# Pranav-Jain/Neural-Monte-Carlo-Fluid-Simulation

Measured on AMD Instinct MI355X. Metric: WoS walk-steps/sec + pressure-projection wall-time per step, 2D karman 64k pts, higher is better.
Workload: dtype f32

## Files before the change

include/wos.h:

```cpp
#ifndef WOS_H
#define WOS_H

#include <stddef.h>
#include <stdint.h>

#ifdef __cplusplus
extern "C" {
#endif

#define WOS_ABI_VERSION 10

enum {
    WOS_OK = 0,
    WOS_E_INVALID = -1,
    WOS_E_IO = -2,
    WOS_E_DEVICE = -3,
    WOS_E_CAPACITY = -4,
    WOS_E_NOMEM = -5
};

#define WOS_PTRS_DEVICE 0x1u
#define WOS_ASYNC       0x2u

typedef struct wos_mesh {
    int32_t dim;
    int32_t n_vertices;
    int32_t n_prims;
    float *vertices;
    int32_t *prims;
} wos_mesh;

int wos_load_obj(const char *path, int32_t dim, int32_t flip_orientation,
                 int32_t normalize, wos_mesh *out);
void wos_mesh_free(wos_mesh *mesh);

typedef struct wos_scene_desc {
    int32_t dim;
    const float *vertices;
    const int32_t *prims;
    int32_t n_vertices, n_prims;
    const float *dvertices;
    const int32_t *dprims;
    int32_t n_dvertices, n_dprims;
    float dirichlet_value;
    float absorption;
    int32_t is_watertight;
    int32_t is_double_sided;
    const float *source;
    int32_t source_dims[3];
    int32_t source_on_device;
    const float *dirichlet_image;
    int32_t dirichlet_image_dims[2];
    float dirichlet_image_box[4];
    int32_t dirichlet_image_on_device;
    const float *neumann_image;
    int32_t neumann_image_dims[2];
    float neumann_image_box[4];
    int32_t neumann_image_on_device;
} wos_scene_desc;

typedef struct wos_scene wos_scene;

int wos_scene_create(const wos_scene_desc *desc, int32_t device, wos_scene **out);
int wos_scene_destroy(wos_scene *scene);

int wos_scene_set_source(wos_scene *scene, const float *source, const int32_t *dims,
                         int32_t on_device, void *stream);

#define WOS_MAX_CHANNELS 4
int wos_scene_set_source_channels(wos_scene *scene, const float *source, int32_t n_channels,
                                  const int32_t *dims, const float *dirichlet_values,
                                  int32_t on_device, void *stream);
int32_t wos_scene_channels(const wos_scene *scene);

int wos_release_caches(int32_t device);

int64_t wos_set_max_batch_tasks(int64_t max_tasks);

typedef struct wos_scene_info {
    int32_t dim, n_prims, n_silhouettes, n_dprims, device;
    float bbox_min[3], bbox_max[3];
} wos_scene_info;
int wos_scene_get_info(const wos_scene *scene, wos_scene_info *info);

enum { WOS_QUERY_NEUMANN = 0, WOS_QUERY_DIRICHLET = 1 };
int wos_scene_query(wos_scene *scene, int32_t which, float boundary_distance_mask,
                    const float *pts, int64_t n,
                    float *dist, float *signed_dist, float *closest , int32_t *state,
                    void *stream, uint32_t flags);

typedef struct wos_solver_params {
    int32_t n_walks;
    int32_t max_walk_length;
    int32_t steps_before_tikhonov;
    int32_t steps_before_maximal_spheres;
    float epsilon_shell;
    float min_star_radius;
    float silhouette_precision;
    float russian_roulette_threshold;
    float boundary_distance_mask;
    int32_t disable_gradient_control_variates;
    int32_t disable_gradient_antithetic_variates;
    int32_t use_cosine_sampling;
    int32_t ignore_dirichlet;
    int32_t ignore_neumann;
    int32_t ignore_source;
    uint64_t seed;
    int32_t robust_float;
    uint32_t schedule;
} wos_solver_params;

#define WOS_SCHED_GEOM_GLOBAL   0x1u
#define WOS_SCHED_FULL_NEUMANN  0x2u
#define WOS_SCHED_NO_STAR_GRID  0x4u
#define WOS_SCHED_NO_DIR_GRID   0x8u
#define WOS_SCHED_NO_TAIL_SPREAD 0x10u
#define WOS_SCHED_NO_GRID_SPREAD 0x20u

void wos_default_params(wos_solver_params *p);

typedef struct wos_stats {
    uint64_t walk_steps;
    uint64_t wasted_steps;
    uint64_t walks_recorded;
    uint64_t walks_escaped;
    uint64_t walks_max_length;
    uint64_t walks_rr;
    uint64_t walks_dirichlet;
    uint64_t points_estimated;
    uint64_t rejection_iters;
    double kernel_ms;
    double first_ball_ms;
    double walk_ms;
    double fold_ms;
    uint64_t walk_launches;
    int32_t first_ball_blocks_per_cu;
    int32_t walk_blocks_per_cu;
    int32_t walk_lds_bytes;
    int32_t star_grid;
    int32_t geom_global;
    int32_t dir_grid;
    uint64_t ticket;
} wos_stats;

int wos_solve(wos_scene *scene, const wos_solver_params *params,
              const float *pts, int64_t n, int64_t index_base, int64_t index_stride,
              float *p, float *grad, int32_t *n_est, int32_t *steps,
              wos_stats *stats, void *stream, uint32_t flags);

int wos_solve_var(wos_scene *scene, const wos_solver_params *params,
                  const float *pts, int64_t n, int64_t index_base, int64_t index_stride,
                  float *p, float *grad, float *p_var, float *grad_var, int32_t *n_est, int32_t *steps,
                  wos_stats *stats, void *stream, uint32_t flags);

int wos_solve_channels(wos_scene *scene, const wos_solver_params *params,
                       const float *pts, int64_t n, int64_t index_base, int64_t index_stride,
                       int32_t n_channels, float *p, float *grad, float *p_var, float *grad_var,
                       int32_t *n_est, int32_t *steps, wos_stats *stats, void *stream, uint32_t flags);

typedef struct wos_bvc_params {
    int32_t n_walks_solution;
    int32_t n_walks_gradient;
    int32_t boundary_cache_size;
    int32_t domain_cache_size;
    int32_t grid_res;
    int32_t use_finite_differences;
    float normal_offset;
    float radius_clamp;
    float kernel_regularization;
    float grid_box[4];
} wos_bvc_params;

void wos_default_bvc_params(wos_bvc_params *p);

int wos_bvc(wos_scene *scene, const wos_solver_params *params, const wos_bvc_params *bvc,
            float *solution, float *grad, float *samples, int64_t samples_capacity, int64_t *counts,
            wos_stats *stats);

int wos_solve_stats(wos_scene *scene, uint64_t ticket, wos_stats *stats);

typedef struct wos_tape wos_tape;
typedef struct wos_tape_info {
    int32_t dim, n_walks, source_dims[3], device;
    int64_t n_points, n_tasks, n_entries, max_entries_per_walk, bytes;
    int32_t replay_chunk_entries;
} wos_tape_info;
int wos_tape_record(wos_scene *scene, const wos_solver_params *params, const float *pts, int64_t n,
                    int64_t index_base, int64_t index_stride, int64_t max_bytes,
                    wos_tape **out, wos_stats *stats, void *stream, uint32_t flags);
int wos_tape_solve(wos_tape *tape, wos_scene *scene, int32_t n_channels,
                   float *p, float *grad, float *p_var, float *grad_var,
                   int32_t *n_est, int32_t *steps, wos_stats *stats, void *stream, uint32_t flags);
int wos_tape_get_info(const wos_tape *tape, wos_tape_info *info);
int wos_tape_destroy(wos_tape *tape);

typedef enum wos_tape_field {
    WOS_TAPE_CODE = 0, WOS_TAPE_CNT = 1, WOS_TAPE_SLOT = 2, WOS_TAPE_CELL0 = 3, WOS_TAPE_GNORM = 4,
    WOS_TAPE_THR_END = 5, WOS_TAPE_TERM = 6, WOS_TAPE_TNEU = 7, WOS_TAPE_BDIR = 8, WOS_TAPE_SDIR = 9,
    WOS_TAPE_E_CELL = 10, WOS_TAPE_E_THR = 11, WOS_TAPE_E_NRM = 12, WOS_TAPE_PSTATE = 13,
    WOS_TAPE_SEGMENT_POINTS = 14
// ... 100 lines not shown
```

neural-monte-carlo-fluid-simulation_amd/csrc/wos_capi.h:

```cpp
#pragma once
#include <hip/hip_runtime.h>

#include <algorithm>
#include <atomic>
#include <cmath>
#include <condition_variable>
#include <cstdlib>
#include <cstring>
#include <list>
#include <memory>
#include <mutex>
#include <string>
#include <vector>

#include "../../include/wos.h"
#include "wos_bvc.h"
#include "wos_detmath.h"
#include "wos_host_scene.h"
#include "wos_launch.h"
#include "wos_siren.h"

namespace wos::capi {

extern thread_local std::string g_err;

inline int fail(int code, const std::string& msg) {
  g_err = msg;
  return code;
}

#define HIP_TRY(expr)                                                                         \
  do {                                                                                        \
    hipError_t _e = (expr);                                                                   \
    if (_e != hipSuccess) return fail(WOS_E_DEVICE, std::string(#expr ": ") + hipGetErrorString(_e)); \
  } while (0)

#define WOS_TRY(expr)                  \
  do {                                 \
    int _rc = (expr);                  \
    if (_rc != WOS_OK) return _rc;     \
  } while (0)

template <typename T>
hipError_t upload(T** dst, const std::vector<T>& src) {
  *dst = nullptr;
  if (src.empty()) return hipSuccess;
  hipError_t e = hipMalloc((void**)dst, src.size() * sizeof(T));
  if (e != hipSuccess) { *dst = nullptr; return e; }
  e = hipMemcpy(*dst, src.data(), src.size() * sizeof(T), hipMemcpyHostToDevice);
  if (e != hipSuccess) {
    hipFree(*dst);
    *dst = nullptr;
  }
  return e;
}

struct DevBufs {
  std::vector<void*> p;
  ~DevBufs() { for (void* q : p) hipFree(q); }
  template <typename T>
  hipError_t get(T** out, size_t n) {
    *out = nullptr;
    void* q = nullptr;
    hipError_t e = hipMalloc(&q, std::max<size_t>(1, n) * sizeof(T));
    if (e == hipSuccess) { p.push_back(q); *out = (T*)q; }
    return e;
  }
};

struct RunShape {
  int32_t bpc_fb = 0, bpc_walk = 0, walk_lds = 0, star_grid = 0, geom_global = 0, dir_grid = 0;
};

struct StatSlot {
  uint64_t ticket = 0;
  unsigned long long* h_cnt = nullptr;
  hipEvent_t ev0 = nullptr, ev1 = nullptr, done = nullptr;
  std::vector<hipEvent_t> bev;
  int64_t n_batches = 0;
  RunShape shape;
};
constexpr int kStatSlots = 16;

struct TaskWs {
  float* tasks = nullptr;
  int64_t task_cap = 0;
  int32_t* pstate = nullptr;
  int64_t pstate_cap = 0;
  unsigned long long* counters = nullptr;
  hipStream_t stream = nullptr;
  hipEvent_t done = nullptr;
};
constexpr int kSideWs = 2;

struct DevCtx {
  std::mutex mu;
  bool ready = false;
  int num_cus = 0;
  float* d_pts = nullptr;
  float* d_p = nullptr;
  float* d_g = nullptr;
  int32_t* d_nest = nullptr;
  int32_t* d_steps = nullptr;
  size_t ws_points = 0;
  float* d_pvar = nullptr;
  float* d_gvar = nullptr;
  size_t ws_var_points = 0;
  uint64_t* d_jump = nullptr;
  int n_jump = 0;
  float* d_tasks = nullptr;
  int64_t task_cap = 0;
  int32_t* d_pstate = nullptr;
  int64_t pstate_cap = 0;
  unsigned long long* d_counters = nullptr;
  StatSlot slot[kStatSlots];
  uint64_t next_ticket = 1;
  hipEvent_t done = nullptr;
  hipStream_t last_stream = nullptr;
  bool inflight = false;
  float* d_rejtab = nullptr;
  int stat_waiters = 0;
  std::condition_variable no_waiters;
  TaskWs side[kSideWs];
  hipStream_t bvc_dir = nullptr;
  hipEvent_t bvc_dir_done = nullptr;
};

constexpr int kMaxDevices = 64;
extern DevCtx g_ctx[kMaxDevices];
extern std::atomic<int64_t> g_max_batch_tasks;

int ctx_ready(DevCtx& c, int device);
hipError_t ctx_order(DevCtx& c, hipStream_t st);
int ctx_mark(DevCtx& c, hipStream_t st);

int ensure_workspace(DevCtx& c, int dim, size_t npts);
int ensure_tasks_in(float*& d_tasks, int64_t& task_cap, int32_t*& d_pstate, int64_t& pstate_cap, int dim,
                    int64_t tasks, int64_t points, int channels = 1);
int ensure_tasks(DevCtx& c, int dim, int64_t tasks, int64_t points, int channels = 1);
wos::DevTasks task_view_in(float* d_tasks, int32_t* d_pstate, int64_t pstate_cap, int dim, int64_t T, int32_t wpp,
                           int channels = 1);
wos::DevTasks task_view(DevCtx& c, int dim, int64_t T, int32_t wpp, int channels = 1);
int ensure_jump(DevCtx& c, int k_needed);
const std::vector<float>& rejection_tables();

int slot_open(DevCtx& c, hipStream_t st, int64_t n_events, int64_t n_batches, const RunShape& shape, StatSlot** out);
int slot_close(StatSlot& q, const unsigned long long* d_cnt, hipStream_t st);
int slot_finish(DevCtx& c, StatSlot& q, hipStream_t st, bool async, wos_stats* stats);

void stats_from(const unsigned long long* cnt, const RunShape& shape, wos_stats* stats);
void stats_add_counters(wos_stats* into, const wos_stats& from);
int fill_stats(const StatSlot& q, wos_stats* stats);

struct SolveOut {
  float* p = nullptr;
  float* grad = nullptr;
  int32_t* n_est = nullptr;
  int32_t* steps = nullptr;
  float* p_var = nullptr;
  float* grad_var = nullptr;
};
struct OutStage {
  SolveOut dev, host;
  size_t n = 0;
  int C = 1, dim = 2;
  bool staged = false;
};
int stage_outputs(DevCtx& c, const SolveOut& caller, bool dev_ptrs, int64_t n, int C, int dim, OutStage& o);
int copy_back(const OutStage& o, hipStream_t st);

struct Geom {
  int device = 0;
  int dim = 2, double_sided = 0;
  std::vector<float> v, dv;
  std::vector<int32_t> ix, dix;
  wos::HostScene host;
  float *d_prim = nullptr, *d_paux = nullptr, *d_sil = nullptr, *d_dprim = nullptr, *d_dpaux = nullptr;
  float *d_pgroup = nullptr, *d_sgroup = nullptr, *d_dgroup = nullptr;
  float *d_ptree = nullptr, *d_stree = nullptr, *d_dtree = nullptr;
  float* d_nbox = nullptr;
  int32_t *d_nchild = nullptr, *d_nref = nullptr;
  std::mutex mu;
  struct Grid {
    float prec, min_r;
    bool ok;
    wos::StarGrid grid;
    uint32_t* d = nullptr;
  };
  std::list<Grid> grids;
  bool dgrid_built = false, dgrid_ok = false;
  wos::DirGrid dgrid;
  uint32_t* d_dgrid = nullptr;
  ~Geom();
};

int star_grid(Geom& g, float prec, float min_r, const Geom::Grid** out);
int dir_grid(Geom& g, bool* ok);
void geom_cache_drop(int device);

constexpr size_t kLdsDynamicMax = 160 * 1024 - 4096;

}

struct wos_scene {
  int device = 0;
  uint64_t serial = 0;
  std::shared_ptr<wos::capi::Geom> geom;
  wos::DevScene dev{};
  float* d_source = nullptr;
  size_t source_cap = 0;
  float* d_planar = nullptr;
  size_t planar_cap = 0;
  float g_dirichlet = 0.0f;
  float* d_dimg = nullptr;
  float* d_nimg = nullptr;
  std::mutex mu;
};

namespace wos::capi {

struct WalkLayout {
  wos::DevScene dsc;
  int geom_floats = 0;
  int geom_floats_walk = 0;
  size_t shmem_walk = 0;
};
int walk_layout(wos_scene* s, const wos_solver_params* prm, WalkLayout& L);

wos::DevParams dev_params(const wos_solver_params* prm);
int check_params(const std::string& fn, const wos_solver_params* prm);

struct SolveExtra {
  const float* ddir = nullptr;
  float* deriv = nullptr;
  bool force_estimate = false;
  int wave_prio = 0;
  float* p_var = nullptr;
  float* grad_var = nullptr;
  int channels = 1;
};

struct SolvePlan {
  wos::DevParams dp{};
  wos::DevScene dsc{}, dfb{};
  int geom_floats_walk = 0, lhs_floats = 0;
  size_t shmem_walk = 0, shmem_fb = 0, shmem_fb_run = 0;
  int64_t wpp = 0;
  wos::KernelVariant kv{};
  int grid_fb = 0, grid_walk = 0, bpc_fb = 0, bpc_walk = 0;
  RunShape shape() const {
    return {bpc_fb, bpc_walk, (int32_t)shmem_walk, dsc.sgrid != nullptr, dsc.geom_global, dsc.dgrid != nullptr};
  }
};
int solve_plan(DevCtx& c, wos_scene* s, const wos_solver_params* prm, const SolveExtra& ex, bool record, SolvePlan& P);
int solve_grids(DevCtx& c, int dim, int64_t chunk, bool record, SolvePlan& P);

struct Batches {
  int64_t chunk = 1, n_chunks = 0;
};
Batches batches(int64_t n, int64_t wpp);
int batch_head(DevCtx& c, int dim, const SolvePlan& P, int64_t k, const float* d_pts, int64_t nb,
               const wos::DevTasks& tk, hipEvent_t after_zero, hipStream_t st);
int fold_channels(int dim, const wos::DevParams& dp, const wos::DevTasks& tk, int C, int64_t nb, int64_t b0,
                  int64_t n, const SolveOut& out, hipStream_t st);

int solve_locked(wos_scene* s, const wos_solver_params* prm, const float* pts, int64_t n, int64_t index_base,
                 int64_t index_stride, float* p, float* grad, int32_t* n_est, int32_t* steps, wos_stats* stats,
                 void* stream, uint32_t flags, const SolveExtra& ex);

}
```

neural-monte-carlo-fluid-simulation_amd/csrc/wos_capi_ctx.cpp:

```cpp
#include "wos_capi.h"

namespace wos::capi {

thread_local std::string g_err;
DevCtx g_ctx[kMaxDevices];

#ifndef WOS_BATCH_LOG2
#define WOS_BATCH_LOG2 28
#endif
static_assert(WOS_BATCH_LOG2 <= 30, "task indices carry a flag in bit 31 (wos_walk_kernel hand-out)");
constexpr int64_t kDefaultBatchTasks = (int64_t)1 << WOS_BATCH_LOG2;
std::atomic<int64_t> g_max_batch_tasks{kDefaultBatchTasks};

static void ctx_free(DevCtx& c) {
  hipFree(c.d_pts); hipFree(c.d_p); hipFree(c.d_g); hipFree(c.d_nest); hipFree(c.d_steps);
  hipFree(c.d_pvar); hipFree(c.d_gvar);
  c.d_pvar = c.d_gvar = nullptr;
  c.ws_var_points = 0;
  hipFree(c.d_jump); hipFree(c.d_tasks); hipFree(c.d_pstate); hipFree(c.d_counters); hipFree(c.d_rejtab);
  c.d_rejtab = nullptr;
  for (StatSlot& q : c.slot) {
    if (q.ev0) hipEventDestroy(q.ev0);
    if (q.ev1) hipEventDestroy(q.ev1);
    if (q.done) hipEventDestroy(q.done);
    for (hipEvent_t e : q.bev) hipEventDestroy(e);
    if (q.h_cnt) hipHostFree(q.h_cnt);
    q = StatSlot{};
  }
  if (c.done) hipEventDestroy(c.done);
  if (c.bvc_dir_done) hipEventDestroy(c.bvc_dir_done);
  if (c.bvc_dir) hipStreamDestroy(c.bvc_dir);
  c.bvc_dir_done = nullptr;
  c.bvc_dir = nullptr;
  for (TaskWs& w : c.side) {
    hipFree(w.tasks); hipFree(w.pstate); hipFree(w.counters);
    if (w.done) hipEventDestroy(w.done);
    if (w.stream) hipStreamDestroy(w.stream);
    w = TaskWs{};
  }
  c.d_pts = c.d_p = c.d_g = nullptr;
  c.d_nest = c.d_steps = nullptr;
  c.ws_points = 0;
  c.d_jump = nullptr; c.n_jump = 0;
  c.d_tasks = nullptr; c.task_cap = 0;
  c.d_pstate = nullptr; c.pstate_cap = 0;
  c.d_counters = nullptr;
  c.done = nullptr;
  c.last_stream = nullptr;
  c.inflight = false;
  c.ready = false;
}

const std::vector<float>& rejection_tables() {
  static std::once_flag once;
  static std::vector<float> t(2 * wos::kRejTabBins);
  std::call_once(once, [] {
    wos::rejection_bound_table(2, t.data());
    wos::rejection_bound_table(3, t.data() + wos::kRejTabBins);
  });
  return t;
}

int ctx_ready(DevCtx& c, int device) {
  if (c.ready) return WOS_OK;
  {
    const std::vector<float>& t = rejection_tables();
    HIP_TRY(hipMalloc((void**)&c.d_rejtab, t.size() * sizeof(float)));
    HIP_TRY(hipMemcpy(c.d_rejtab, t.data(), t.size() * sizeof(float), hipMemcpyHostToDevice));
  }
  HIP_TRY(hipDeviceGetAttribute(&c.num_cus, hipDeviceAttributeMultiprocessorCount, device));
  HIP_TRY(hipMalloc((void**)&c.d_counters, wos::kMainCounterSlots * sizeof(unsigned long long)));
  for (StatSlot& q : c.slot) {
    HIP_TRY(hipHostMalloc((void**)&q.h_cnt, wos::kNumCounters * sizeof(unsigned long long)));
    HIP_TRY(hipEventCreate(&q.ev0));
    HIP_TRY(hipEventCreate(&q.ev1));
    HIP_TRY(hipEventCreateWithFlags(&q.done, hipEventDisableTiming));
  }
  HIP_TRY(hipEventCreateWithFlags(&c.done, hipEventDisableTiming));
  c.ready = true;
  return WOS_OK;
}

hipError_t ctx_order(DevCtx& c, hipStream_t st) {
  if (c.inflight && c.last_stream != st && c.done) return hipStreamWaitEvent(st, c.done, 0);
  return hipSuccess;
}

int ctx_mark(DevCtx& c, hipStream_t st) {
  HIP_TRY(hipEventRecord(c.done, st));
  c.last_stream = st;
  return WOS_OK;
}

int ensure_workspace(DevCtx& c, int dim, size_t npts) {
  if (npts <= c.ws_points) return WOS_OK;
  hipFree(c.d_pts); hipFree(c.d_p); hipFree(c.d_g); hipFree(c.d_nest); hipFree(c.d_steps);
  c.d_pts = c.d_p = c.d_g = nullptr; c.d_nest = c.d_steps = nullptr; c.ws_points = 0;
  const size_t cap = npts + npts / 4 + 1024;
  HIP_TRY(hipMalloc((void**)&c.d_pts, cap * 3 * sizeof(float)));
  HIP_TRY(hipMalloc((void**)&c.d_p, cap * sizeof(float)));
  HIP_TRY(hipMalloc((void**)&c.d_g, cap * 3 * sizeof(float)));
  HIP_TRY(hipMalloc((void**)&c.d_nest, cap * sizeof(int32_t)));
  HIP_TRY(hipMalloc((void**)&c.d_steps, cap * sizeof(int32_t)));
  (void)dim;
  c.ws_points = cap;
  return WOS_OK;
}

static int ensure_var_workspace(DevCtx& c, size_t npts) {
  if (npts <= c.ws_var_points) return WOS_OK;
  hipFree(c.d_pvar); hipFree(c.d_gvar);
  c.d_pvar = c.d_gvar = nullptr; c.ws_var_points = 0;
  const size_t cap = npts + npts / 4 + 1024;
  HIP_TRY(hipMalloc((void**)&c.d_pvar, cap * sizeof(float)));
  HIP_TRY(hipMalloc((void**)&c.d_gvar, cap * 3 * sizeof(float)));
  c.ws_var_points = cap;
  return WOS_OK;
}

int ensure_tasks_in(float*& d_tasks, int64_t& task_cap, int32_t*& d_pstate, int64_t& pstate_cap, int dim,
                    int64_t tasks, int64_t points, int channels) {
  const int tf = std::max(wos::task_floats(dim), wos::task_floats(3));
  const int tfc = std::max(wos::task_floats(dim, channels), wos::task_floats(3, channels));
  if (channels > 1) tasks = (tasks * tfc + tf - 1) / tf;
  if (tasks > task_cap) {
    hipFree(d_tasks);
    d_tasks = nullptr; task_cap = 0;
    HIP_TRY(hipMalloc((void**)&d_tasks, (size_t)tasks * tf * sizeof(float)));
    task_cap = tasks;
  }
  if (points > pstate_cap) {
    hipFree(d_pstate);
    d_pstate = nullptr; pstate_cap = 0;
    HIP_TRY(hipMalloc((void**)&d_pstate, ((size_t)7 * points + 2 * wos::kCostBuckets) * sizeof(int32_t)));
    pstate_cap = points;
  }
  return WOS_OK;
}

int ensure_tasks(DevCtx& c, int dim, int64_t tasks, int64_t points, int channels) {
  return ensure_tasks_in(c.d_tasks, c.task_cap, c.d_pstate, c.pstate_cap, dim, tasks, points, channels);
}

wos::DevTasks task_view_in(float* d_tasks, int32_t* d_pstate, int64_t pstate_cap, int dim, int64_t T, int32_t wpp,
                           int channels) {
  wos::DevTasks tk{};
  float* f = d_tasks;
  tk.pt = f; f += dim * T;
  tk.thr = f; f += T;
  tk.tsrc = f; f += channels * T;
  tk.dd = f; f += T;
  tk.first = f; f += channels * T;
  tk.bdir = f; f += dim * T;
  tk.sdir = f; f += dim * T;
  tk.total = f; f += channels * T;
  tk.code = (uint32_t*)f;
  tk.pstate = d_pstate;
  tk.perm = (uint32_t*)(d_pstate + pstate_cap);
  tk.prad = (float*)(d_pstate + 2 * pstate_cap);
  tk.hist = (uint32_t*)(d_pstate + 3 * pstate_cap);
  tk.pball = (float*)(d_pstate + 3 * pstate_cap + 2 * wos::kCostBuckets);
  tk.pball_stride = pstate_cap;
  tk.T = T;
  tk.wpp = wpp;
  return tk;
}

wos::DevTasks task_view(DevCtx& c, int dim, int64_t T, int32_t wpp, int channels) {
  return task_view_in(c.d_tasks, c.d_pstate, c.pstate_cap, dim, T, wpp, channels);
}

int ensure_jump(DevCtx& c, int k_needed) {
  if (k_needed <= c.n_jump) return WOS_OK;
  const int cap = std::max(k_needed, 4096);
  std::vector<uint64_t> t(2 * (size_t)cap);
  uint64_t A = 1u, Cc = 0u;
  for (int k = 0; k < cap; k++) {
    t[2 * k] = A; t[2 * k + 1] = Cc;
    A = A * wos::kPcgMult;
    Cc = Cc * wos::kPcgMult + wos::kPcgInc;
  }
  hipFree(c.d_jump);
  c.d_jump = nullptr; c.n_jump = 0;
  HIP_TRY(hipMalloc((void**)&c.d_jump, t.size() * sizeof(uint64_t)));
  HIP_TRY(hipMemcpy(c.d_jump, t.data(), t.size() * sizeof(uint64_t), hipMemcpyHostToDevice));
  c.n_jump = cap;
  return WOS_OK;
}

int stage_outputs(DevCtx& c, const SolveOut& caller, bool dev_ptrs, int64_t n, int C, int dim, OutStage& o) {
  o.dev = o.host = caller;
  o.n = (size_t)std::max<int64_t>(n, 0);
  o.C = C;
  o.dim = dim;
  o.staged = !dev_ptrs && n > 0;
  if (!o.staged) return WOS_OK;
  WOS_TRY(ensure_workspace(c, dim, o.n * C));
  o.dev.p = c.d_p; o.dev.grad = c.d_g;
  o.dev.n_est = caller.n_est ? c.d_nest : nullptr;
  o.dev.steps = caller.steps ? c.d_steps : nullptr;
  if (caller.p_var || caller.grad_var) {
    WOS_TRY(ensure_var_workspace(c, o.n * C));
    o.dev.p_var = caller.p_var ? c.d_pvar : nullptr;
    o.dev.grad_var = caller.grad_var ? c.d_gvar : nullptr;
  }
  return WOS_OK;
}

int copy_back(const OutStage& o, hipStream_t st) {
  if (!o.staged) return WOS_OK;
  const size_t n = o.n, nc = o.n * o.C;
  const SolveOut &h = o.host, &d = o.dev;
  HIP_TRY(hipMemcpyAsync(h.p, d.p, nc * sizeof(float), hipMemcpyDeviceToHost, st));
  HIP_TRY(hipMemcpyAsync(h.grad, d.grad, nc * o.dim * sizeof(float), hipMemcpyDeviceToHost, st));
  if (h.n_est) HIP_TRY(hipMemcpyAsync(h.n_est, d.n_est, n * sizeof(int32_t), hipMemcpyDeviceToHost, st));
  if (h.steps) HIP_TRY(hipMemcpyAsync(h.steps, d.steps, n * sizeof(int32_t), hipMemcpyDeviceToHost, st));
  if (h.p_var) HIP_TRY(hipMemcpyAsync(h.p_var, d.p_var, nc * sizeof(float), hipMemcpyDeviceToHost, st));
  if (h.grad_var)
    HIP_TRY(hipMemcpyAsync(h.grad_var, d.grad_var, nc * o.dim * sizeof(float), hipMemcpyDeviceToHost, st));
  return WOS_OK;
}

int slot_open(DevCtx& c, hipStream_t st, int64_t n_events, int64_t n_batches, const RunShape& shape, StatSlot** out) {
  const uint64_t ticket = c.next_ticket++;
  StatSlot& q = c.slot[ticket % kStatSlots];
  while ((int64_t)q.bev.size() < n_events) {
    hipEvent_t e = nullptr;
    HIP_TRY(hipEventCreate(&e));
    q.bev.push_back(e);
  }
  q.ticket = ticket;
  q.n_batches = n_batches;
  q.shape = shape;
  HIP_TRY(hipEventRecord(q.ev0, st));
  *out = &q;
  return WOS_OK;
}

int slot_close(StatSlot& q, const unsigned long long* d_cnt, hipStream_t st) {
  HIP_TRY(hipEventRecord(q.ev1, st));
  HIP_TRY(hipMemcpyAsync(q.h_cnt, d_cnt, wos::kNumCounters * sizeof(unsigned long long), hipMemcpyDeviceToHost, st));
  return WOS_OK;
}

int slot_finish(DevCtx& c, StatSlot& q, hipStream_t st, bool async, wos_stats* stats) {
  HIP_TRY(hipEventRecord(q.done, st));
  WOS_TRY(ctx_mark(c, st));
  c.inflight = true;
  if (async) {
    if (stats) {
      *stats = wos_stats{};
      stats->ticket = q.ticket;
    }
    return WOS_OK;
  }
  HIP_TRY(hipStreamSynchronize(st));
  c.inflight = false;
  return stats ? fill_stats(q, stats) : WOS_OK;
}

void stats_from(const unsigned long long* cnt, const RunShape& shape, wos_stats* stats) {
  *stats = wos_stats{};
  stats->walk_steps = cnt[0];
  stats->wasted_steps = cnt[1];
  stats->walks_recorded = cnt[2];
  stats->walks_escaped = cnt[3];
  stats->walks_max_length = cnt[4];
  stats->walks_rr = cnt[5];
  stats->walks_dirichlet = cnt[6];
  stats->points_estimated = cnt[7];
  stats->rejection_iters = cnt[8];
  stats->first_ball_blocks_per_cu = shape.bpc_fb;
  stats->walk_blocks_per_cu = shape.bpc_walk;
  stats->walk_lds_bytes = shape.walk_lds;
  stats->star_grid = shape.star_grid;
  stats->geom_global = shape.geom_global;
  stats->dir_grid = shape.dir_grid;
}

void stats_add_counters(wos_stats* into, const wos_stats& from) {
  into->walk_steps += from.walk_steps; into->wasted_steps += from.wasted_steps;
  into->walks_recorded += from.walks_recorded; into->walks_escaped += from.walks_escaped;
  into->walks_max_length += from.walks_max_length; into->walks_rr += from.walks_rr;
  into->walks_dirichlet += from.walks_dirichlet; into->points_estimated += from.points_estimated;
  into->rejection_iters += from.rejection_iters;
}

int fill_stats(const StatSlot& q, wos_stats* stats) {
  stats_from(q.h_cnt, q.shape, stats);
  float ms = 0.0f;
  HIP_TRY(hipEventElapsedTime(&ms, q.ev0, q.ev1));
  stats->kernel_ms = ms;
  stats->walk_launches = (uint64_t)q.n_batches;
  for (int64_t b = 0; b < q.n_batches; b++) {
    const hipEvent_t* ev = &q.bev[4 * b];
    float a = 0.0f, w = 0.0f, f = 0.0f;
    HIP_TRY(hipEventElapsedTime(&a, ev[0], ev[1]));
    HIP_TRY(hipEventElapsedTime(&w, ev[1], ev[2]));
    HIP_TRY(hipEventElapsedTime(&f, ev[2], ev[3]));
    stats->first_ball_ms += a; stats->walk_ms += w; stats->fold_ms += f;
  }
  stats->ticket = q.ticket;
  return WOS_OK;
}

}

using namespace wos::capi;

extern "C" {

const char* wos_last_error(void) { return g_err.c_str(); }
int32_t wos_abi_version(void) { return WOS_ABI_VERSION; }

int32_t wos_device_count(void) {
  int n = 0;
  if (hipGetDeviceCount(&n) != hipSuccess) return 0;
  return n;
}

int64_t wos_set_max_batch_tasks(int64_t max_tasks) {
  const int64_t v = max_tasks <= 0 ? kDefaultBatchTasks
                                   : std::min<int64_t>(std::max<int64_t>(max_tasks, (int64_t)1 << 16), (int64_t)1 << 30);
  return g_max_batch_tasks.exchange(v);
}

int wos_release_caches(int32_t device) {
  int ndev = 0;
  if (hipGetDeviceCount(&ndev) != hipSuccess) ndev = 0;
  for (int dv = 0; dv < std::min(ndev, kMaxDevices); dv++) {
    if (device >= 0 && dv != device) continue;
    DevCtx& c = g_ctx[dv];
    std::unique_lock<std::mutex> lk(c.mu);
    c.no_waiters.wait(lk, [&] { return c.stat_waiters == 0; });
    if (!c.ready) continue;
    HIP_TRY(hipSetDevice(dv));
    HIP_TRY(hipDeviceSynchronize());
    ctx_free(c);
  }
  geom_cache_drop(device);
  return WOS_OK;
}

int wos_solve_stats(wos_scene* s, uint64_t ticket, wos_stats* stats) {
  if (!s || !stats) return fail(WOS_E_INVALID, "wos_solve_stats: null scene/stats");
  const auto unknown = [&] {
    return fail(WOS_E_INVALID, "wos_solve_stats: unknown ticket (more than " + std::to_string(kStatSlots) +
                                   " solves were enqueued on this device after it)");
  };
  HIP_TRY(hipSetDevice(s->device));
  DevCtx& c = g_ctx[s->device];
  hipEvent_t done = nullptr;
  {
    std::lock_guard<std::mutex> lock(s->mu);
    std::lock_guard<std::mutex> lk(c.mu);
    StatSlot& q = c.slot[ticket % kStatSlots];
    if (ticket == 0 || q.ticket != ticket) return unknown();
    done = q.done;
    c.stat_waiters++;
  }
  const hipError_t e = hipEventSynchronize(done);
  std::lock_guard<std::mutex> lock(s->mu);
  std::lock_guard<std::mutex> lk(c.mu);
  if (--c.stat_waiters == 0) c.no_waiters.notify_all();
  if (e != hipSuccess) return fail(WOS_E_DEVICE, std::string("wos_solve_stats: ") + hipGetErrorString(e));
  StatSlot& q = c.slot[ticket % kStatSlots];
  if (q.ticket != ticket) return unknown();
  HIP_TRY(hipEventSynchronize(q.done));
  return fill_stats(q, stats);
}

}
```

neural-monte-carlo-fluid-simulation_amd/csrc/wos_capi_scene.cpp:

```cpp
#include "wos_capi.h"

namespace wos::capi {

Geom::~Geom() {
  hipSetDevice(device);
  hipDeviceSynchronize();
  hipFree(d_prim); hipFree(d_paux); hipFree(d_sil); hipFree(d_dprim); hipFree(d_dpaux);
  hipFree(d_pgroup); hipFree(d_sgroup); hipFree(d_dgroup);
  hipFree(d_ptree); hipFree(d_stree); hipFree(d_dtree);
  hipFree(d_nbox); hipFree(d_nchild); hipFree(d_nref);
  for (Grid& g : grids) hipFree(g.d);
  hipFree(d_dgrid);
}

static std::mutex g_geom_mu;
static std::vector<std::shared_ptr<Geom>>& g_geom_lru = *new std::vector<std::shared_ptr<Geom>>();
constexpr size_t kGeomCacheSize = 8;
static std::atomic<uint64_t> g_scene_serial{0};

template <typename T>
static bool same(const std::vector<T>& a, const T* b, int n) {
  return a.size() == (size_t)n && (n == 0 || std::memcmp(a.data(), b, (size_t)n * sizeof(T)) == 0);
}

static bool geom_matches(const Geom& g, const wos_scene_desc* d, int device) {
  const int dim = d->dim;
  return g.device == device && g.dim == dim && g.double_sided == d->is_double_sided &&
         same(g.v, d->vertices, d->n_vertices * dim) && same(g.ix, d->prims, d->n_prims * dim) &&
         same(g.dv, d->dvertices, d->n_dvertices * dim) && same(g.dix, d->dprims, d->n_dprims * dim);
}

static int geom_get(const wos_scene_desc* d, int device, std::shared_ptr<Geom>& out) {
  {
    std::lock_guard<std::mutex> lk(g_geom_mu);
    for (size_t i = 0; i < g_geom_lru.size(); i++)
      if (geom_matches(*g_geom_lru[i], d, device)) {
        out = g_geom_lru[i];
        std::rotate(g_geom_lru.begin(), g_geom_lru.begin() + i, g_geom_lru.begin() + i + 1);
        return WOS_OK;
      }
  }
  auto g = std::make_shared<Geom>();
  const int dim = d->dim;
  g->device = device;
  g->dim = dim;
  g->double_sided = d->is_double_sided;
  if (d->n_vertices > 0) g->v.assign(d->vertices, d->vertices + (size_t)d->n_vertices * dim);
  if (d->n_prims > 0) g->ix.assign(d->prims, d->prims + (size_t)d->n_prims * dim);
  if (d->n_dvertices > 0) g->dv.assign(d->dvertices, d->dvertices + (size_t)d->n_dvertices * dim);
  if (d->n_dprims > 0) g->dix.assign(d->dprims, d->dprims + (size_t)d->n_dprims * dim);
  wos::HostSceneInput in;
  in.dim = dim;
  in.vertices = d->vertices; in.prims = d->prims; in.n_vertices = d->n_vertices; in.n_prims = d->n_prims;
  in.dvertices = d->dvertices; in.dprims = d->dprims; in.n_dvertices = d->n_dvertices; in.n_dprims = d->n_dprims;
  in.is_double_sided = d->is_double_sided;
  std::string err;
  if (!wos::prepare_scene(in, g->host, err)) return fail(WOS_E_INVALID, "wos_scene_create: " + err);
  HIP_TRY(upload(&g->d_prim, g->host.prim));
  HIP_TRY(upload(&g->d_paux, g->host.paux));
  HIP_TRY(upload(&g->d_sil, g->host.sil));
  HIP_TRY(upload(&g->d_dprim, g->host.dprim));
  HIP_TRY(upload(&g->d_dpaux, g->host.dpaux));
  HIP_TRY(upload(&g->d_pgroup, g->host.pgroup));
  HIP_TRY(upload(&g->d_dgroup, g->host.dgroup));
  HIP_TRY(upload(&g->d_sgroup, g->host.sgroup));
  HIP_TRY(upload(&g->d_ptree, g->host.ptree.node));
  HIP_TRY(upload(&g->d_stree, g->host.stree.node));
  HIP_TRY(upload(&g->d_dtree, g->host.dtree.node));
  HIP_TRY(upload(&g->d_nbox, g->host.nbvh.box));
  HIP_TRY(upload(&g->d_nchild, g->host.nbvh.child));
  HIP_TRY(upload(&g->d_nref, g->host.nbvh.ref));
  {
    std::lock_guard<std::mutex> lk(g_geom_mu);
    g_geom_lru.insert(g_geom_lru.begin(), g);
    if (g_geom_lru.size() > kGeomCacheSize) g_geom_lru.pop_back();
  }
  out = g;
  return WOS_OK;
}

void geom_cache_drop(int device) {
  std::lock_guard<std::mutex> lk(g_geom_mu);
  if (device < 0) {
    g_geom_lru.clear();
  } else {
    g_geom_lru.erase(std::remove_if(g_geom_lru.begin(), g_geom_lru.end(),
                                    [&](const std::shared_ptr<Geom>& g) { return g->device == device; }),
                     g_geom_lru.end());
  }
}

constexpr size_t kStarGridBudget = 16 * 1024;

int star_grid(Geom& g, float prec, float min_r, const Geom::Grid** out) {
  std::lock_guard<std::mutex> lk(g.mu);
  for (const Geom::Grid& x : g.grids)
    if (x.prec == prec && x.min_r == min_r) { *out = &x; return WOS_OK; }
  Geom::Grid x{prec, min_r, false, {}, nullptr};
  if (wos::build_star_grid(g.host, prec, min_r, kStarGridBudget, x.grid)) {
    HIP_TRY(upload(&x.d, x.grid.words));
    x.ok = true;
  }
  g.grids.push_back(std::move(x));
  *out = &g.grids.back();
  return WOS_OK;
}

int dir_grid(Geom& g, bool* ok) {
  std::lock_guard<std::mutex> lk(g.mu);
  if (!g.dgrid_built) {
    const bool have = wos::build_dirichlet_grid(g.host, g.dgrid);
    if (have) HIP_TRY(upload(&g.d_dgrid, g.dgrid.words));
    g.dgrid_ok = have;
    g.dgrid_built = true;
  }
  *ok = g.dgrid_ok;
  return WOS_OK;
}

static void source_installed(wos_scene* s, const int32_t* dims, int n_channels, const float* dirichlet_values) {
  const int nsd = s->dev.dim == 2 ? 2 : 3;
  s->dev.source = s->d_source;
  for (int k = 0; k < 3; k++) s->dev.sdims[k] = k < nsd ? dims[k] : 1;
  s->dev.n_channels = n_channels;
  s->dev.g_dirichlet = s->g_dirichlet;
  for (int ch = 0; ch < wos::kMaxChannels; ch++)
    s->dev.g_ch[ch] = (dirichlet_values && ch < n_channels) ? dirichlet_values[ch] : s->g_dirichlet;
}

static int check_source_dims(int dim, const int32_t* dims, size_t* nsrc) {
  const int nsd = dim == 2 ? 2 : 3;
  size_t n = 1;
  for (int k = 0; k < nsd; k++) {
// ... 326 lines not shown
```

neural-monte-carlo-fluid-simulation_amd/csrc/wos_capi_solve.cpp:

```cpp
#include "wos_capi.h"

namespace wos::capi {

int walk_layout(wos_scene* s, const wos_solver_params* prm, WalkLayout& L) {
  Geom& geom = *s->geom;
  const wos::HostScene& host = geom.host;
  const int dim = host.dim;
  const int PS = dim == 2 ? wos::kPrimStride2 : wos::kPrimStride3;
  const int SS = dim == 2 ? wos::kSilStride2 : wos::kSilStride3;
  const int primAl = (host.n_prims * PS + 3) & ~3;
  const int silAl = (host.n_sil * SS + 3) & ~3;
  L.geom_floats = primAl + silAl + wos::kGroupStride * host.n_pgroups + wos::kSGroupStride * host.n_sgroups;
  wos::DevScene& dsc = L.dsc;
  dsc = s->dev;
  dsc.sgrid = nullptr;
  dsc.sgrid_words = dsc.sgrid_off_words = 0;
  if (!(prm->schedule & WOS_SCHED_NO_STAR_GRID) && host.n_sil > 0) {
    const Geom::Grid* gr = nullptr;
    WOS_TRY(star_grid(geom, prm->silhouette_precision, prm->min_star_radius, &gr));
    if (gr->ok) {
      dsc.sgrid = gr->d;
      dsc.sgrid_words = (int32_t)gr->grid.words.size();
      dsc.sgrid_off_words = gr->grid.off_words;
      for (int k = 0; k < 3; k++) {
// ... 87 lines not shown
  wos::DevScene& dsc = P.dsc;
  dsc = wl.dsc;
  P.geom_floats_walk = wl.geom_floats_walk;
  P.shmem_walk = wl.shmem_walk;
  P.lhs_floats = ((2 * dp.n_pairs * (dim - 1)) + 3) & ~3;
  P.shmem_fb = wos::kWavesPerBlockHost * wos::first_ball_wave_lds_bytes(P.lhs_floats, dp.n_pairs);
  P.shmem_fb_run = P.shmem_fb;
  wos::DevScene& dfb = P.dfb;
  dfb = s->dev;
  dfb.dgrid = dsc.dgrid;
  dfb.dgrid_off_words = dsc.dgrid_off_words;
  for (int k = 0; k < 2; k++) {
    dfb.dgrid_n[k] = dsc.dgrid_n[k];
    dfb.dgrid_min[k] = dsc.dgrid_min[k];
    dfb.dgrid_inv[k] = dsc.dgrid_inv[k];
  }
  if ((prm->schedule & WOS_SCHED_GEOM_GLOBAL) || P.shmem_walk > kLdsDynamicMax) {
    dfb.geom_global = 1;
    dsc.geom_global = 1;
    P.geom_floats_walk = 0;
    P.shmem_walk = wos::kWavesPerBlockHost * wos::walk_wave_lds_bytes(dim);
  }
  if (P.shmem_fb > kLdsDynamicMax)
    return fail(WOS_E_CAPACITY, "wos_solve: nWalks exceed the LDS budget of the first-ball kernel (" +
                                    std::to_string(P.shmem_fb) + " bytes of stratified samples per block)");
  if (P.shmem_walk > kLdsDynamicMax)
    return fail(WOS_E_CAPACITY, "wos_solve: the walk kernel's per-wave scratch exceeds the LDS budget (" +
                                    std::to_string(P.shmem_walk) + " bytes)");

  P.wpp = (int64_t)dp.n_pairs * dp.n_anti;
  {
    double diag2 = 0.0;
    for (int k = 0; k < 3; k++) diag2 += (double)host.ext[k] * host.ext[k];
    const double mu_r = std::sqrt(std::max(0.0, (double)s->dev.absorption)) * std::sqrt(diag2) * 1.01;
    dp.neumann_inert = (!dp.robust && s->dev.watertight && !s->dev.double_sided && mu_r < 80.0 && !s->dev.nimg &&
                        !(prm->schedule & WOS_SCHED_FULL_NEUMANN)) ? 1 : 0;
  }
  dp.tail_spread = (dim == 2 && !dp.robust && !dsc.geom_global && !(prm->schedule & WOS_SCHED_NO_TAIL_SPREAD)) ? 1 : 0;
#ifdef WOS_ACCT_NOSPREAD
  dp.tail_spread = 0;
#endif
  if (record) {
    dp.neumann_inert = 0;
    dp.tail_spread = 0;
    dsc.n_channels = 1;
    dfb.n_channels = 1;
  }
  P.kv = wos::kernel_variant(dim, dsc, dp, false);
  return WOS_OK;
}

int solve_grids(DevCtx& c, int dim, int64_t chunk, bool record, SolvePlan& P) {
  wos::DevParams& dp = P.dp;
  const bool gg = P.dsc.geom_global != 0;
  const auto occupancy = [&](int which, size_t shmem, int* blocks) {
    return record ? wos::occupancy_rec_blocks_per_cu(dim, gg, which, shmem, blocks)
                  : wos::occupancy_blocks_per_cu(P.kv, which, shmem, blocks);
  };
  HIP_TRY(occupancy(0, P.shmem_fb, &P.bpc_fb));
  const int jn = std::min(2 * (2 * dp.n_pairs) * (dim - 1), wos::kLhsJumpMax);
  const size_t shmem_j = P.shmem_fb + (size_t)jn * 2 * sizeof(uint64_t);
  int bpc_j = 0;
  if (jn > 0 && shmem_j <= kLdsDynamicMax) HIP_TRY(occupancy(0, shmem_j, &bpc_j));
  if (WOS_LHS_JUMP_STAGE && jn > 0 && bpc_j >= P.bpc_fb) {
    dp.lhs_jump_n = jn;
    P.shmem_fb_run = shmem_j;
  }
  const int64_t fb_waves = (chunk + wos::first_ball_points_per_wave(dp.n_pairs) - 1) / wos::first_ball_points_per_wave(dp.n_pairs);
  P.grid_fb = (int)std::min<int64_t>((fb_waves + wos::kWavesPerBlockHost - 1) / wos::kWavesPerBlockHost,
                                     (int64_t)std::max(1, P.bpc_fb) * std::max(1, c.num_cus));
  HIP_TRY(occupancy(1, P.shmem_walk, &P.bpc_walk));
  P.grid_walk = std::max(1, P.bpc_walk) * std::max(1, c.num_cus);
  return WOS_OK;
}

Batches batches(int64_t n, int64_t wpp) {
  Batches b;
  b.chunk = std::max<int64_t>(1, std::min<int64_t>(n, g_max_batch_tasks.load() / wpp));
  b.n_chunks = n > 0 ? (n + b.chunk - 1) / b.chunk : 0;
  return b;
}

int batch_head(DevCtx& c, int dim, const SolvePlan& P, int64_t k, const float* d_pts, int64_t nb,
               const wos::DevTasks& tk, hipEvent_t after_zero, hipStream_t st) {
  HIP_TRY(wos::launch_zero(k == 0 ? c.d_counters : c.d_counters + wos::kNumCounters,
                           k == 0 ? wos::kNumCounterSlots : wos::kNumCounterSlots - wos::kNumCounters,
                           tk.hist, 2 * wos::kCostBuckets, st));
  if (after_zero) HIP_TRY(hipEventRecord(after_zero, st));
  HIP_TRY(wos::launch_point_setup(dim, P.dfb, P.dp, d_pts, nb, tk, st));
  HIP_TRY(wos::launch_lpt_order(tk, nb, st));
  return WOS_OK;
}

int fold_channels(int dim, const wos::DevParams& dp, const wos::DevTasks& tk, int C, int64_t nb, int64_t b0,
                  int64_t n, const SolveOut& out, hipStream_t st) {
  for (int ch = 0; ch < C; ch++) {
    wos::DevTasks tkc = tk;
    tkc.total = tk.total + (int64_t)ch * tk.T;
    tkc.first = tk.first + (int64_t)ch * tk.T;
    const int64_t o1 = (int64_t)ch * n + b0, od = ((int64_t)ch * n + b0) * dim;
    HIP_TRY(wos::launch_fold(dim, dp, tkc, nb, out.p + o1, out.grad + od,
                             (out.n_est && ch == 0) ? out.n_est + b0 : nullptr,
                             (out.steps && ch == 0) ? out.steps + b0 : nullptr, out.p_var ? out.p_var + o1 : nullptr,
                             out.grad_var ? out.grad_var + od : nullptr, st));
  }
  return WOS_OK;
}

int solve_locked(wos_scene* s, const wos_solver_params* prm, const float* pts, int64_t n, int64_t index_base,
                 int64_t index_stride, float* p, float* grad, int32_t* n_est, int32_t* steps, wos_stats* stats,
                 void* stream, uint32_t flags, const SolveExtra& ex) {
  const int dim = s->geom->host.dim;
  hipStream_t st = (hipStream_t)stream;
  DevCtx& c = g_ctx[s->device];
  WOS_TRY(ctx_ready(c, s->device));

  SolvePlan plan;
  WOS_TRY(solve_plan(c, s, prm, ex, false, plan));
  wos::DevParams& dp = plan.dp;

  HIP_TRY(ctx_order(c, st));

  const bool dev_ptrs = (flags & WOS_PTRS_DEVICE) != 0;
  const int C = ex.channels;
  OutStage out;
  WOS_TRY(stage_outputs(c, SolveOut{p, grad, n_est, steps, ex.p_var, ex.grad_var}, dev_ptrs, n, C, dim, out));
  const float* d_pts = pts;
  if (out.staged) {
    HIP_TRY(hipMemcpyAsync(c.d_pts, pts, (size_t)n * dim * sizeof(float), hipMemcpyHostToDevice, st));
    d_pts = c.d_pts;
  }

  const int64_t wpp = plan.wpp;
  const Batches bt = batches(n, wpp);
  if (n > 0) {
    WOS_TRY(ensure_tasks(c, dim, bt.chunk * wpp, bt.chunk, C));
    WOS_TRY(solve_grids(c, dim, bt.chunk, false, plan));
  }
  StatSlot* slot = nullptr;
  WOS_TRY(slot_open(c, st, 4 * bt.n_chunks, bt.n_chunks, plan.shape(), &slot));
  StatSlot& q = *slot;
  if (bt.n_chunks == 0) HIP_TRY(wos::launch_zero(c.d_counters, wos::kMainCounterSlots, nullptr, 0, st));
  for (int64_t k = 0; k < bt.n_chunks; k++) {
    const int64_t b0 = k * bt.chunk;
    hipEvent_t* ev = &q.bev[4 * k];
    const int64_t nb = std::min(bt.chunk, n - b0);
    wos::DevTasks tk = task_view(c, dim, nb * wpp, (int32_t)wpp, C);
    tk.ddir = ex.ddir ? ex.ddir + b0 * dim : nullptr;
    tk.deriv = ex.deriv ? ex.deriv + b0 : nullptr;
    const int64_t bbase = index_base + b0 * index_stride;
    unsigned int* q_points = (unsigned int*)(c.d_counters + wos::kNumCounters);
    unsigned int* q_tasks = (unsigned int*)(c.d_counters + wos::kTaskQueueSlot0);
    const int walk_grid = (int)std::min<int64_t>(plan.grid_walk, (tk.T + 63) / 64);
    WOS_TRY(batch_head(c, dim, plan, k, d_pts + b0 * dim, nb, tk, ev[0], st));
    HIP_TRY(wos::launch_first_balls(plan.kv, plan.dfb, dp, d_pts + b0 * dim, nb, bbase, index_stride, tk,
                                    c.d_counters, q_points, plan.grid_fb, plan.shmem_fb_run, plan.lhs_floats, st));
    HIP_TRY(hipEventRecord(ev[1], st));
    HIP_TRY(wos::launch_walks(plan.kv, plan.dsc, dp, tk, bbase, index_stride, c.d_counters, q_tasks, walk_grid,
                              plan.shmem_walk, plan.geom_floats_walk, st));
    HIP_TRY(hipEventRecord(ev[2], st));
    WOS_TRY(fold_channels(dim, dp, tk, C, nb, b0, n, out.dev, st));
    HIP_TRY(hipEventRecord(ev[3], st));
  }
  WOS_TRY(slot_close(q, c.d_counters, st));
  WOS_TRY(copy_back(out, st));
  const bool async = (flags & WOS_ASYNC) && dev_ptrs;
  WOS_TRY(slot_finish(c, q, st, async, stats));
  if (!async) wos::diag_dump(dim == 2 ? "2d" : "3d");
  return WOS_OK;
}

static int solve_checked(wos_scene* s, const wos_solver_params* prm, const float* pts, int64_t n, int64_t index_base,
                         int64_t index_stride, int32_t n_channels, float* p, float* grad, float* p_var,
                         float* grad_var, int32_t* n_est, int32_t* steps, wos_stats* stats, void* stream,
                         uint32_t flags) {
  if (!s || !prm) return fail(WOS_E_INVALID, "wos_solve: null scene/params");
  if (n < 0) return fail(WOS_E_INVALID, "wos_solve: negative point count");
  if (n > 0 && (!pts || !p || !grad)) return fail(WOS_E_INVALID, "wos_solve: null point/output buffer");
  if (n >= (int64_t)0xFFFFFFF0LL) return fail(WOS_E_INVALID, "wos_solve: too many points for one call");
  WOS_TRY(check_params("wos_solve", prm));
  std::lock_guard<std::mutex> lock(s->mu);
  HIP_TRY(hipSetDevice(s->device));
  DevCtx& c = g_ctx[s->device];
  std::lock_guard<std::mutex> lk(c.mu);
  if (n_channels == 0 && s->dev.n_channels > 1)
    return fail(WOS_E_INVALID, "wos_solve: the scene holds " + std::to_string(s->dev.n_channels) +
                                   " source channels; use wos_solve_channels (or wos_scene_set_source for one)");
  if (n_channels != 0 && n_channels != s->dev.n_channels)
    return fail(WOS_E_INVALID, "wos_solve_channels: n_channels " + std::to_string(n_channels) +
                                   " differs from the scene's " + std::to_string(s->dev.n_channels));
  SolveExtra ex;
  ex.p_var = p_var;
  ex.grad_var = grad_var;
  ex.channels = s->dev.n_channels;
  return solve_locked(s, prm, pts, n, index_base, index_stride, p, grad, n_est, steps, stats, stream, flags, ex);
}

}

using namespace wos::capi;

extern "C" {

void wos_default_params(wos_solver_params* p) {
  if (!p) return;
  std::memset(p, 0, sizeof(*p));
  p->n_walks = 128;
  p->max_walk_length = 1024;
  p->steps_before_tikhonov = 1024;
  p->steps_before_maximal_spheres = 1024;
  p->epsilon_shell = 1e-3f;
  p->min_star_radius = 1e-3f;
  p->silhouette_precision = 1e-3f;
  p->russian_roulette_threshold = 0.0f;
  p->boundary_distance_mask = 0.0f;
  p->seed = 0x5EED0001ULL;
}

int wos_solve_var(wos_scene* s, const wos_solver_params* prm, const float* pts, int64_t n, int64_t index_base,
                  int64_t index_stride, float* p, float* grad, float* p_var, float* grad_var, int32_t* n_est,
                  int32_t* steps, wos_stats* stats, void* stream, uint32_t flags) {
  return solve_checked(s, prm, pts, n, index_base, index_stride, 0, p, grad, p_var, grad_var, n_est, steps, stats,
                       stream, flags);
}

int wos_solve_channels(wos_scene* s, const wos_solver_params* prm, const float* pts, int64_t n, int64_t index_base,
                       int64_t index_stride, int32_t n_channels, float* p, float* grad, float* p_var,
                       float* grad_var, int32_t* n_est, int32_t* steps, wos_stats* stats, void* stream,
                       uint32_t flags) {
  if (n_channels < 1 || n_channels > WOS_MAX_CHANNELS)
    return fail(WOS_E_INVALID, "wos_solve_channels: n_channels must be 1.." + std::to_string(WOS_MAX_CHANNELS) +
                                   ", got " + std::to_string(n_channels));
  return solve_checked(s, prm, pts, n, index_base, index_stride, n_channels, p, grad, p_var, grad_var, n_est, steps,
                       stats, stream, flags);
}

int wos_solve(wos_scene* s, const wos_solver_params* prm, const float* pts, int64_t n, int64_t index_base,
              int64_t index_stride, float* p, float* grad, int32_t* n_est, int32_t* steps, wos_stats* stats,
              void* stream, uint32_t flags) {
  return wos_solve_var(s, prm, pts, n, index_base, index_stride, p, grad, nullptr, nullptr, n_est, steps, stats,
                       stream, flags);
}
// ... 3 lines not shown
```

neural-monte-carlo-fluid-simulation_amd/csrc/wos_capi_tape.cpp:

```cpp
#include "wos_capi.h"

using namespace wos::capi;

struct TapeSeg {
  int64_t nb = 0, T = 0;
  uint64_t slots = 0;
  void* buf = nullptr;
  void* ebuf = nullptr;
  wos::DevTape tp{};
  uint32_t* code = nullptr;
  float* bdir = nullptr;
  float* sdir = nullptr;
  int32_t* pstate = nullptr;
};

struct TapeIndexSeg {
  void* buf = nullptr;
  wos::DevTapeIndex ix{};
  int64_t bytes = 0, max_row = 0;
};

struct TapeIndex {
  std::vector<TapeIndexSeg> seg;
  int64_t bytes = 0, n_terms = 0, max_row = 0;
// ... 57 lines not shown
  for (int k = 0; k < 3; k++)
    if ((s->dev.source ? s->dev.sdims[k] : 0) != tape->sdims[k])
      return fail(WOS_E_INVALID, fn + ": the scene's source dims differ from the recorded ones "
                                 "(the tape stores grid cells)");
  return WOS_OK;
}

static int tape_ensure_tasks(DevCtx& c, const wos_tape* tape, int C) {
  int64_t maxT = 0;
  for (const TapeSeg& g : tape->seg) maxT = std::max(maxT, g.T);
  return maxT > 0 ? ensure_tasks(c, tape->dim, maxT, 0, C) : WOS_OK;
}

extern "C" {

int wos_tape_record(wos_scene* s, const wos_solver_params* prm, const float* pts, int64_t n, int64_t index_base,
                    int64_t index_stride, int64_t max_bytes, wos_tape** out, wos_stats* stats, void* stream,
                    uint32_t flags) {
  if (!s || !prm || !out) return fail(WOS_E_INVALID, "wos_tape_record: null scene/params/out");
  *out = nullptr;
  if (n < 0) return fail(WOS_E_INVALID, "wos_tape_record: negative point count");
  if (n > 0 && !pts) return fail(WOS_E_INVALID, "wos_tape_record: null point buffer");
  if (n >= (int64_t)0xFFFFFFF0LL) return fail(WOS_E_INVALID, "wos_tape_record: too many points for one call");
  WOS_TRY(check_params("wos_tape_record", prm));
  if (prm->robust_float)
    return fail(WOS_E_INVALID, "wos_tape_record: robust_float walks are not recorded (reference float semantics only)");
  std::lock_guard<std::mutex> lock(s->mu);
  HIP_TRY(hipSetDevice(s->device));
  DevCtx& c = g_ctx[s->device];
  std::lock_guard<std::mutex> lk(c.mu);
  WOS_TRY(ctx_ready(c, s->device));
  const int dim = s->geom->host.dim;
  hipStream_t st = (hipStream_t)stream;
  SolvePlan plan;
  WOS_TRY(solve_plan(c, s, prm, SolveExtra{}, true, plan));
  wos::DevParams& dp = plan.dp;
  HIP_TRY(ctx_order(c, st));
  const float* d_pts = pts;
  if (!(flags & WOS_PTRS_DEVICE) && n > 0) {
    WOS_TRY(ensure_workspace(c, dim, (size_t)n));
    HIP_TRY(hipMemcpyAsync(c.d_pts, pts, (size_t)n * dim * sizeof(float), hipMemcpyHostToDevice, st));
    d_pts = c.d_pts;
  }
  const int64_t wpp = plan.wpp;
  const Batches bt = batches(n, wpp);
  DevBufs tmp;
  unsigned long long* d_cnt2 = nullptr;
  unsigned long long* d_bsum = nullptr;
  if (n > 0) {
    WOS_TRY(ensure_tasks(c, dim, bt.chunk * wpp, bt.chunk, 1));
    WOS_TRY(solve_grids(c, dim, bt.chunk, true, plan));
    HIP_TRY(tmp.get(&d_cnt2, (size_t)wos::kNumCounterSlots));
    HIP_TRY(tmp.get(&d_bsum, (size_t)wos::tape_slot_blocks(bt.chunk * wpp) + 1));
  }

  std::unique_ptr<wos_tape> tape(new wos_tape());
  tape->device = s->device;
  tape->geom = s->geom;
  tape->scene_serial = s->serial;
  tape->dim = dim;
  for (int k = 0; k < 3; k++) tape->sdims[k] = s->dev.source ? s->dev.sdims[k] : 0;
  tape->dp = dp;
  tape->dp.jump = nullptr;
  tape->dp.rej_tab = nullptr;
  tape->n = n;
  tape->wpp = wpp;
  tape->shape = plan.shape();
  HIP_TRY(hipMalloc((void**)&tape->d_cnt, (wos::kNumCounters + 2) * sizeof(unsigned long long)));
  HIP_TRY(hipMalloc((void**)&tape->d_flag, sizeof(uint32_t)));
  HIP_TRY(hipMemsetAsync(tape->d_cnt, 0, (wos::kNumCounters + 2) * sizeof(unsigned long long), st));
  HIP_TRY(hipMemsetAsync(tape->d_flag, 0, sizeof(uint32_t), st));
  tape->bytes = (int64_t)((wos::kNumCounters + 2) * sizeof(unsigned long long) + sizeof(uint32_t));
  unsigned long long* d_stat = tape->d_cnt + wos::kNumCounters;
  const auto over_cap = [&](int64_t bytes) {
    return fail(WOS_E_CAPACITY, "wos_tape_record: the tape needs more than " + std::to_string(bytes) +
                                    " bytes, max_bytes is " + std::to_string(max_bytes));
  };

  hipEvent_t ev0 = nullptr, ev1 = nullptr;
  HIP_TRY(hipEventCreate(&ev0));
  struct EvGuard { hipEvent_t& a; hipEvent_t& b; ~EvGuard() { if (a) hipEventDestroy(a); if (b) hipEventDestroy(b); } } evg{ev0, ev1};
  HIP_TRY(hipEventCreate(&ev1));
  HIP_TRY(hipEventRecord(ev0, st));
  if (bt.n_chunks == 0) HIP_TRY(wos::launch_zero(c.d_counters, wos::kMainCounterSlots, nullptr, 0, st));
  tape->seg.reserve((size_t)bt.n_chunks);
  for (int64_t k = 0; k < bt.n_chunks; k++) {
    const int64_t b0 = k * bt.chunk;
    const int64_t nb = std::min(bt.chunk, n - b0);
    tape->seg.emplace_back();
    TapeSeg& g = tape->seg.back();
    g.nb = nb;
    g.T = nb * wpp;
    const size_t tb = tape_task_bytes(dim, g.T, nb);
    if (max_bytes > 0 && tape->bytes + (int64_t)tb > max_bytes) return over_cap(tape->bytes + (int64_t)tb);
    HIP_TRY(hipMalloc(&g.buf, tb));
    tape->bytes += (int64_t)tb;
    tape_seg_views(g, dim, tape->d_flag);
    wos::DevTasks tk = task_view(c, dim, g.T, (int32_t)wpp, 1);
    wos::DevTasks tkr = tk;
    tkr.bdir = g.bdir;
    tkr.sdir = g.sdir;
    const int64_t bbase = index_base + b0 * index_stride;
    unsigned long long* qslot = c.d_counters + wos::kNumCounters;
    const int walk_grid = (int)std::min<int64_t>(plan.grid_walk, (g.T + 63) / 64);
    WOS_TRY(batch_head(c, dim, plan, k, d_pts + b0 * dim, nb, tk, nullptr, st));
    HIP_TRY(wos::launch_first_balls_rec(dim, plan.dfb, dp, d_pts + b0 * dim, nb, bbase, index_stride, tkr, g.tp,
                                        c.d_counters, (unsigned int*)qslot, plan.grid_fb, plan.shmem_fb_run,
                                        plan.lhs_floats, st));
    HIP_TRY(hipMemsetAsync(tk.tsrc, 0, (size_t)g.T * sizeof(float), st));
    HIP_TRY(wos::launch_walks(plan.kv, plan.dsc, dp, tk, bbase, index_stride, c.d_counters,
                              (unsigned int*)(c.d_counters + wos::kTaskQueueSlot0), walk_grid, plan.shmem_walk,
                              plan.geom_floats_walk, st));
    HIP_TRY(wos::launch_tape_slots(tk.code, g.T, (uint32_t*)g.tp.slot, d_bsum, st));
    unsigned long long slots = 0;
    HIP_TRY(hipMemcpyAsync(&slots, d_bsum + wos::tape_slot_blocks(g.T), sizeof(slots), hipMemcpyDeviceToHost, st));
    HIP_TRY(hipStreamSynchronize(st));
    if (slots >= (1ull << 31))
      return fail(WOS_E_CAPACITY, "wos_tape_record: a batch's walks need " + std::to_string(slots) +
                                      " entry slots (32-bit slot indices); lower wos_set_max_batch_tasks");
    g.slots = slots;
    const size_t eb = (size_t)std::max<unsigned long long>(slots, 1) * 12;
    if (max_bytes > 0 && tape->bytes + (int64_t)eb > max_bytes) return over_cap(tape->bytes + (int64_t)eb);
    HIP_TRY(hipMalloc(&g.ebuf, eb));
    tape->bytes += (int64_t)eb;
    g.tp.e_cell = (uint32_t*)g.ebuf;
    g.tp.e_thr = (float*)g.ebuf + std::max<unsigned long long>(slots, 1);
    g.tp.e_nrm = g.tp.e_thr + std::max<unsigned long long>(slots, 1);
    HIP_TRY(hipMemsetAsync(g.ebuf, 0, eb, st));
    tkr.code = g.code;
    HIP_TRY(wos::launch_zero(d_cnt2, wos::kNumCounterSlots, nullptr, 0, st));
    HIP_TRY(wos::launch_walks_rec(dim, plan.dsc.geom_global != 0, plan.dsc, dp, tkr, g.tp, bbase, index_stride, d_cnt2,
                                  (unsigned int*)(d_cnt2 + wos::kTaskQueueSlot0), walk_grid, plan.shmem_walk,
                                  plan.geom_floats_walk, st));
    HIP_TRY(hipMemcpyAsync(g.pstate, tk.pstate, (size_t)nb * sizeof(int32_t), hipMemcpyDeviceToDevice, st));
    HIP_TRY(wos::launch_tape_stats(g.code, g.tp.cnt, g.T, d_stat, st));
  }
  HIP_TRY(hipMemcpyAsync(tape->d_cnt, c.d_counters, wos::kNumCounters * sizeof(unsigned long long),
                         hipMemcpyDeviceToDevice, st));
  HIP_TRY(hipEventRecord(ev1, st));
  unsigned long long h_cnt[wos::kNumCounters + 2] = {};
  uint32_t h_flag = 0;
  HIP_TRY(hipMemcpyAsync(h_cnt, tape->d_cnt, sizeof(h_cnt), hipMemcpyDeviceToHost, st));
  HIP_TRY(hipMemcpyAsync(&h_flag, tape->d_flag, sizeof(h_flag), hipMemcpyDeviceToHost, st));
  WOS_TRY(ctx_mark(c, st));
  HIP_TRY(hipStreamSynchronize(st));
  c.inflight = false;
  if (h_flag)
    return fail(WOS_E_DEVICE, "wos_tape_record: a walk outgrew the slots sized for it; the tape is discarded");
  tape->n_entries = (int64_t)h_cnt[wos::kNumCounters];
  tape->max_entries = (int64_t)h_cnt[wos::kNumCounters + 1];
  if (stats) {
    stats_from(h_cnt, tape->shape, stats);
    float ms = 0.0f;
    HIP_TRY(hipEventElapsedTime(&ms, ev0, ev1));
    stats->kernel_ms = ms;
    stats->walk_launches = (uint64_t)(2 * bt.n_chunks);
  }
  *out = tape.release();
  return WOS_OK;
}

int wos_tape_solve(wos_tape* tape, wos_scene* s, int32_t n_channels, float* p, float* grad, float* p_var,
                   float* grad_var, int32_t* n_est, int32_t* steps, wos_stats* stats, void* stream, uint32_t flags) {
  if (!tape || !s) return fail(WOS_E_INVALID, "wos_tape_solve: null tape/scene");
  const int64_t n = tape->n;
  const int dim = tape->dim;
  if (n > 0 && (!p || !grad)) return fail(WOS_E_INVALID, "wos_tape_solve: null output buffer");
// ... 322 lines not shown
```

neural-monte-carlo-fluid-simulation_amd/csrc/wos_device.h:

```cpp

#pragma once
#include <cstdio>

#include "wos_detmath.h"
#include "wos_scene.h"

namespace wos {

#ifndef WOS_DIAG
#define WOS_DIAG 0
#endif

constexpr int kWave = 64;
constexpr int kBlock = 256;

enum { WC_DIRICHLET = 0, WC_RR = 1, WC_MAXLEN = 2, WC_ESCAPED = 3 };

enum { C_STEPS = 0, C_WASTED, C_REC, C_ESC, C_MAXL, C_RR, C_DIR, C_PTS, C_ITERS, C_NUM };

__device__ __forceinline__ void wave_sync() {
  __builtin_amdgcn_fence(__ATOMIC_SEQ_CST, "wavefront");
  __builtin_amdgcn_wave_barrier();
}

enum { D_ITERS = 0, D_LANES, D_STAR, D_RAY, D_SAMPLE, D_STEP, D_LOOP, D_RAYOVF, D_SCALLS, D_SGVISIT, D_SCAND, D_SEXACT,
       D_FB_PTS, D_FB_SETUP, D_FB_LHS, D_FB_BALLS, D_FB_TOTAL, D_FB_MAX, D_WMAXLEN, D_WAVEMAX, D_RCALLS, D_RGENS, D_RITEMS, D_RQUICK, D_RUND, D_RLANES, D_MID, D_END, D_TAIL,
       D_XITERS, D_XLANES, D_XLOOP,
       D_L_ITERS, D_L_STEP, D_L_STAR, D_L_MID, D_L_RAY, D_L_END, D_L_SAMPLE, D_L_TAIL, D_L_LOOP,
       D_L_S_CELL, D_L_S_PFX, D_L_S_WIN, D_L_S_FIN, D_L_S_BUILD, D_L_S_PRE, D_L_S_POST,
       D_FB_UPD, D_FB_SMP, D_FB_MA, D_FB_MB, D_FB_ST, D_FB_ITSUM, D_FB_ITMAX, D_NUM };
__host__ __device__ constexpr bool diag_is_max(int k) { return k == D_FB_MAX || k == D_WMAXLEN || k == D_WAVEMAX; }
static __device__ unsigned long long g_diag[D_NUM];
#if WOS_DIAG
static __shared__ unsigned long long s_diag[D_NUM];
#endif
#if WOS_DIAG
#define DIAG_T0(v) const uint64_t v = __builtin_amdgcn_s_memtime()
#define DIAG_ADD(slot, v)                                                              \
  do {                                                                                 \
    const uint64_t dt_ = __builtin_amdgcn_s_memtime() - (v);                           \
    if ((int)(threadIdx.x & 63) == __builtin_amdgcn_readfirstlane((int)(threadIdx.x & 63))) \
      atomicAdd(&s_diag[slot], (unsigned long long)dt_);                               \
  } while (0)
#define DIAG_COUNT(slot, n)                                                            \
  do {                                                                                 \
    const unsigned long long n_ = (n);                                                 \
    if ((int)(threadIdx.x & 63) == __builtin_amdgcn_readfirstlane((int)(threadIdx.x & 63))) \
      atomicAdd(&s_diag[slot], n_);                                                    \
  } while (0)
#define DIAG_ADD_LONE(slot, lslot, v, lone)                                            \
  do {                                                                                 \
    const uint64_t dt_ = __builtin_amdgcn_s_memtime() - (v);                           \
    if ((int)(threadIdx.x & 63) == __builtin_amdgcn_readfirstlane((int)(threadIdx.x & 63))) { \
      atomicAdd(&s_diag[slot], (unsigned long long)dt_);                               \
      if (lone) atomicAdd(&s_diag[lslot], (unsigned long long)dt_);                    \
    }                                                                                  \
  } while (0)
#define DIAG_LONE(v, pred) const bool v = __popcll(__ballot(pred)) <= 2
#define DIAG_ADD_IF(slot, v, cond)                                                     \
  do {                                                                                 \
    const uint64_t dt_ = __builtin_amdgcn_s_memtime() - (v);                           \
    if ((cond) && (int)(threadIdx.x & 63) == __builtin_amdgcn_readfirstlane((int)(threadIdx.x & 63))) \
      atomicAdd(&s_diag[slot], (unsigned long long)dt_);                               \
  } while (0)
#define DIAG_LANE(slot) atomicAdd(&s_diag[slot], 1ull)
#define DIAG_MAX(slot, v) atomicMax(&s_diag[slot], (unsigned long long)(v))
#else
#define DIAG_T0(v)
#define DIAG_ADD(slot, v)
#define DIAG_COUNT(slot, n)
#define DIAG_ADD_LONE(slot, lslot, v, lone)
#define DIAG_LONE(v, pred)
#define DIAG_ADD_IF(slot, v, cond)
#define DIAG_LANE(slot)
#define DIAG_MAX(slot, v)
#endif

#ifndef WOS_TIMELINE
#define WOS_TIMELINE 0
#endif
constexpr int kTlBins = 384, kTlShift = 10;
enum { TL_WAVE = 0, TL_LANE, TL_START, TL_FIN, TL_NUM };
#if WOS_TIMELINE
static __device__ unsigned long long g_tl[1 + TL_NUM * kTlBins];
#endif

template <int DIM>
__device__ __forceinline__ float dotv(const float* a, const float* b) {
  float s = a[0] * b[0] + a[1] * b[1];
  if constexpr (DIM == 3) s = s + a[2] * b[2];
  return s;
}
template <int DIM>
__device__ __forceinline__ float normv(const float* a) { return __builtin_sqrtf(dotv<DIM>(a, a)); }

__device__ __forceinline__ void cross3(float* r, const float* a, const float* b) {
  float x = a[1] * b[2] - a[2] * b[1], y = a[2] * b[0] - a[0] * b[2], z = a[0] * b[1] - a[1] * b[0];
  r[0] = x; r[1] = y; r[2] = z;
}

template <int DIM>
__device__ __forceinline__ void normalize_div(float* v) {
  float z = dotv<DIM>(v, v);
  if (z > 0.0f) { float s = __builtin_sqrtf(z); for (int k = 0; k < DIM; k++) v[k] = v[k] / s; }
}
template <int DIM>
__device__ __forceinline__ void normalize_rcp(float* v) {
  float inv = 1.0f / __builtin_sqrtf(dotv<DIM>(v, v));
  for (int k = 0; k < DIM; k++) v[k] = v[k] * inv;
}


template <int DIM>
// ... 2965 lines not shown
  const int dpN = sc.n_dprims * PS, dpAl = (dpN + 3) & ~3, dgN = sc.n_dgroups * kGroupStride;
  float* dbase = smem + primAl + silAl + pgN + sgN + sgridAl;
  G.dprim = with_sil ? dbase : sc.dprim;
  G.dgroup = with_sil ? dbase + dpAl : sc.dgroup;
  if (!copy) return G;
  for (int i = threadIdx.x; i < primN; i += kBlock) smem[i] = sc.prim[i];
  if (with_sil) {
    for (int i = threadIdx.x; i < silN; i += kBlock) smem[primAl + i] = sc.sil[i];
    for (int i = threadIdx.x; i < pgN; i += kBlock) smem[primAl + silAl + i] = sc.pgroup[i];
    for (int i = threadIdx.x; i < sgN; i += kBlock) smem[primAl + silAl + pgN + i] = sc.sgroup[i];
    if (sc.sgrid != nullptr)
      for (int i = threadIdx.x; i < sc.sgrid_words; i += kBlock) gw[i] = sc.sgrid[i];
    for (int i = threadIdx.x; i < dpN; i += kBlock) dbase[i] = sc.dprim[i];
    for (int i = threadIdx.x; i < dgN; i += kBlock) dbase[dpAl + i] = sc.dgroup[i];
  }
  return G;
}

template <int DIM, bool GG>
__device__ __forceinline__ LGeom stage_geometry(const DevScene& sc, float* smem, bool with_sil) {
  return geometry_view<DIM, GG>(sc, smem, with_sil, true);
}

struct WalkKernArgs {
  DevScene sc;
  DevParams prm;
  DevTasks tk;
};
using KernArgsPtr = const __attribute__((address_space(4))) WalkKernArgs*;
__device__ __forceinline__ KernArgsPtr kernargs_opaque() {
  KernArgsPtr q = (KernArgsPtr)__builtin_amdgcn_kernarg_segment_ptr();
  asm volatile("" : "+s"(q));
  return q;
}

__device__ __forceinline__ void flush_counter(unsigned long long* counters, int slot, uint32_t v, int lane) {
  unsigned long long s = v;
  for (int off = kWave / 2; off > 0; off >>= 1) s += __shfl_xor(s, off);
  if (lane == 0 && s) atomicAdd(&counters[slot], s);
}

enum { kPtEstimate = 1, kPtMaskP = 2, kPtMaskG = 4 };

constexpr unsigned int kPtGrab = 2;
#ifndef WOS_FB_WAVES_PER_EU
#define WOS_FB_WAVES_PER_EU 3
#endif
#ifndef WOS_FB_WAVES_PER_EU2
#define WOS_FB_WAVES_PER_EU2 4
#endif

template <int DIM>
__device__ __forceinline__ int32_t point_state(const DevScene& sc, const DevParams& prm, float nDist, float nSigned,
                                               float dDist, float dSigned, int* bucket_out, float* firstR) {
  const bool inside = !sc.watertight ? true
                      : (__builtin_fabsf(dSigned) < __builtin_fabsf(nSigned) ? dSigned < 0.0f : nSigned < 0.0f);
  const bool estimate = inside || sc.double_sided || prm.force_estimate;
  const float mask = prm.boundary_distance_mask;
  const bool maskP = __builtin_fabsf(nDist) < mask;
  const bool maskG = (!inside && !sc.double_sided) || __builtin_fabsf(nDist) < mask;
  const float bd = smin(dDist, nDist);
  int bucket = 0;
  if (estimate) {
    const float l2 = __builtin_amdgcn_logf(smax(bd, 1e-9f));
    bucket = (int)sclamp((int)(-2.0f * l2) + 8, 1, kCostBuckets - 1);
  }
  *bucket_out = bucket;
  *firstR = 0.99f * bd;
  return (estimate ? kPtEstimate : 0) | (maskP ? kPtMaskP : 0) | (maskG ? kPtMaskG : 0) | (bucket << 8);
}

#ifndef WOS_SETUP_LANES
#define WOS_SETUP_LANES 1
#endif
constexpr int kSetupLanes = WOS_SETUP_LANES;
#ifndef WOS_SETUP_LDS_FLOATS
#define WOS_SETUP_LDS_FLOATS 4096
#endif
constexpr int kSetupLdsFloats = WOS_SETUP_LDS_FLOATS;
static_assert((kSetupLanes & (kSetupLanes - 1)) == 0 && kSetupLanes <= kWave, "kSetupLanes");
template <int DIM>
__global__ __launch_bounds__(256) void wos_point_setup_kernel(const DevScene sc, const DevParams prm,
                                                             const float* __restrict__ pts, int64_t n,
                                                             const DevTasks tk) {
  __shared__ uint32_t s_hist[kCostBuckets];
  __shared__ __attribute__((aligned(16))) float s_prim[kSetupLdsFloats];
  constexpr int PS = Layout<DIM>::prim;
  const int nfl = sc.n_prims * PS, dfl = sc.n_dprims * PS;
  const bool lds_n = nfl <= kSetupLdsFloats, lds_d = nfl + dfl <= kSetupLdsFloats;
  if (lds_n)
    for (int k = threadIdx.x; k < nfl; k += blockDim.x) s_prim[k] = sc.prim[k];
  if (lds_d)
    for (int k = threadIdx.x; k < dfl; k += blockDim.x) s_prim[nfl + k] = sc.dprim[k];
  if (threadIdx.x < kCostBuckets) s_hist[threadIdx.x] = 0u;
  __syncthreads();
  const float* nprim = lds_n ? s_prim : sc.prim;
  const float* dprim = lds_d ? s_prim + nfl : sc.dprim;
  const int64_t gi = (int64_t)blockIdx.x * blockDim.x + threadIdx.x;
  const int64_t i = gi / kSetupLanes;
  const int sub = (int)(gi % kSetupLanes);
  if (i < n) {
    float x[DIM];
    for (int k = 0; k < DIM; k++) x[k] = pts[i * DIM + k];
    float nDist = kFltMax, nSigned = kFltMax;
    if (sc.n_prims > 0) {
      const Closest c = closest_lane<DIM>(nprim, sc.pgroup, sc.n_prims, sc.n_pgroups, x, sub, kSetupLanes);
      nDist = c.d;
      nSigned = signed_dist<DIM>(sc.paux, c, x);
    }
    float dDist, dSigned;
    if (sc.n_dprims > 0) {
      const Closest c = closest_lane<DIM>(dprim, sc.dgroup, sc.n_dprims, sc.n_dgroups, x, sub, kSetupLanes);
      dDist = c.d;
      dSigned = signed_dist<DIM>(sc.dpaux, c, x);
    } else {
      dDist = dSigned = bbox_far_dist<DIM>(sc, x);
    }
    int bucket;
    float firstR;
    const int32_t ps = point_state<DIM>(sc, prm, nDist, nSigned, dDist, dSigned, &bucket, &firstR);
    if (sub == 0) {
      tk.pstate[i] = ps;
      tk.prad[i] = firstR;
      if constexpr (DIM == 2) {
        if (tk.pball != nullptr && !prm.robust && (ps & kPtEstimate) && sc.absorption > 0.0f &&
            prm.steps_before_tikhonov == 0) {
          Gfn<2> g;
          g.init(true, sc.absorption);
          g.update_ball(x, firstR, false);
          tk.pball[i] = g.A0;
          tk.pball[tk.pball_stride + i] = g.A1;
          tk.pball[2 * tk.pball_stride + i] = g.B0;
          tk.pball[3 * tk.pball_stride + i] = g.B1;
        }
      }
      atomicAdd(&s_hist[bucket], 1u);
    }
  }
  __syncthreads();
  if (threadIdx.x < kCostBuckets && s_hist[threadIdx.x]) atomicAdd(&tk.hist[threadIdx.x], s_hist[threadIdx.x]);
}

template <int DIM, bool RB = false, int NC = 1>
__global__ __launch_bounds__(kBlock) __attribute__((amdgpu_waves_per_eu(DIM == 2 ? WOS_FB_WAVES_PER_EU2 : WOS_FB_WAVES_PER_EU))) void wos_first_ball_kernel(
    const DevScene sc, const DevParams prm, const float* __restrict__ pts, int64_t n, int64_t base, int64_t stride,
    const DevTasks tk, unsigned long long* __restrict__ counters, unsigned int* __restrict__ work, int lhs_floats) {
  constexpr bool REC = false;
  const DevTape* const tape = nullptr;
#include "wos_first_ball_body.inc"
}

__device__ __forceinline__ void wave_priority(int level) {
  if (level == 1) __builtin_amdgcn_s_setprio(1);
  else if (level == 2) __builtin_amdgcn_s_setprio(2);
  else if (level >= 3) __builtin_amdgcn_s_setprio(3);
}

template <int DIM, bool BSTART, bool RB, int NC, bool REC>
__device__ __forceinline__ void walk_start(const DevScene& sc, const DevParams& prm, const DevTasks& tk, int64_t t,
                                           uint32_t pidx, uint32_t w, const float* v_pt, float v_thr, const float* v_tsrc,
                                           float v_dd, int64_t base, int64_t stride, bool yuk0, WalkState<DIM, NC, REC>& st,
                                           Gfn<DIM, RB>& g, Pcg32& ws, float& ddist, uint32_t& wsteps, float& firstR) {
  for (int kk = 0; kk < DIM; kk++) { st.pt[kk] = v_pt[kk]; st.n[kk] = 0.0f; st.prevDir[kk] = 0.0f; }
  st.prevDist = 0.0f;
  st.throughput = v_thr;
  st.onNeumann = false;
  st.walkLength = 0;
  st.totalNeumann = 0.0f;
  for (int c = 0; c < NC; c++) st.totalSource[c] = v_tsrc[c];
  st.pend = false;
  if constexpr (REC) {
    st.rbase = st.tape->slot[t];
    st.rcap = st.tape->slot[t + 1] - st.rbase;
    st.rn = 0u;
  }
  ddist = v_dd;
  g.init(yuk0, sc.absorption);
  if constexpr (BSTART) {
    for (int kk = 0; kk < DIM; kk++) { st.n[kk] = tk.n0[kk * tk.T + t]; st.prevDir[kk] = st.n[kk]; }
    st.prevDist = kFltMax;
    const uint32_t fl = tk.sflags[t];
    st.onNeumann = (fl & 1u) != 0u;
    firstR = tk.r0[t];
    ws.seed(seed32(prm.seed, (uint64_t)(base + (int64_t)pidx * stride), (uint64_t)w, (fl >> 8) & 0xFFu));
    wsteps = 0;
  } else {
    ws.seed(seed32(prm.seed, (uint64_t)(base + (int64_t)pidx * stride), (uint64_t)w, 2));
    wsteps = 1;
  }
}

template <int DIM, bool GG, bool BSTART, bool RB, bool NEU = true, int NC, bool REC>
__device__ __forceinline__ int walk_iteration(const DevScene& sc, const DevParams& prm, const LGeom& G, bool active,
                                              WalkState<DIM, NC, REC>& st, Gfn<DIM, RB>& gc, Pcg32& ws, float& ddist,
                                              uint32_t& wsteps, float& firstR, StarLDS<DIM>* starL,
                                              RayLDS<DIM>* rayL, RejLDS* rejL, uint32_t* c_iters, int lane) {
  DIAG_T0(t_step);
  Gfn<DIM, RB> g;
  g.yukawa = gc.yukawa; g.lambda = sc.absorption; g.sqrtLambda = __builtin_sqrtf(sc.absorption);
  int code = -1;
  DIAG_LONE(lone, active);
  bool flip = false, query = false;
  if (active) code = walk_step_begin<DIM>(sc, prm, ddist, st, &flip, &query, BSTART ? firstR : 0.0f);
  DIAG_T0(t_star);
  const float starQ = star_radius_wave<DIM, GG>(G, sc, prm, active && code < 0 && query, st.pt, ddist, flip, starL, lane);
  if (WOS_PROBE & 8) {
    float px[DIM];
    for (int k = 0; k < DIM; k++) px[k] = probe_opaque(st.pt[k]);
    probe_sink(star_radius_wave<DIM, GG>(G, sc, prm, active && code < 0 && query, px, probe_opaque(ddist), flip, starL,
                                         lane));
  }
  DIAG_ADD_LONE(D_STAR, D_L_STAR, t_star, lone);
  const bool live = active && code < 0;
  float dir[DIM], org[DIM], starR = 0.0f;
  for (int k = 0; k < DIM; k++) { dir[k] = 1.0f; org[k] = 0.0f; }
  DIAG_T0(t_mid);
  if (live) starR = walk_step_mid<DIM>(prm, ddist, ws, g, st, &wsteps, query, starQ, dir, org, BSTART ? firstR : 0.0f);
  DIAG_ADD_LONE(D_MID, D_L_MID, t_mid, lone);
  Hit ip;
  DIAG_T0(t_ray);
  const bool hit = ray_hit_wave<DIM, GG>(G, sc, live, org, dir, starR, &ip, rayL, lane);
  if (WOS_PROBE & 16) {
    Hit ip2;
    float po[DIM];
    for (int k = 0; k < DIM; k++) po[k] = probe_opaque(org[k]);
    probe_sink(ray_hit_wave<DIM, GG>(G, sc, live, po, dir, probe_opaque(starR), &ip2, rayL, lane) ? ip2.d : 0.0f);
  }
  DIAG_ADD_LONE(D_RAY, D_L_RAY, t_ray, lone);
  DIAG_T0(t_end);
  if (live) walk_step_end<DIM, RB, NEU>(sc, prm, G, ws, g, st, starR, dir, org, hit, ip, flip);
  DIAG_ADD_LONE(D_END, D_L_END, t_end, lone);
  float sp[DIM], pdf_unused;
  for (int k = 0; k < DIM; k++) sp[k] = 0.0f;
  DIAG_T0(t_smp);
  if ((WOS_PROBE & 32) && !prm.ignore_source) {
    Gfn<DIM, RB> g2 = g;
    Pcg32 ws2 = ws;
    ws2.state = probe_opaque(ws2.state);
    float sp2[DIM], pdf2;
    uint32_t it2 = 0;
    sample_volume_wave<DIM>(prm, live, g2, dir, ws2, &pdf2, sp2, &it2, false, rejL, lane);
    probe_sink(sp2[0]);
  }
  if (!prm.ignore_source) sample_volume_wave<DIM>(prm, live, g, dir, ws, &pdf_unused, sp, c_iters, false, rejL, lane);
  DIAG_ADD_LONE(D_SAMPLE, D_L_SAMPLE, t_smp, lone);
  DIAG_T0(t_tail);
  if (live) code = walk_step_tail<DIM>(sc, G, prm, ddist, ws, g, st, dir, hit, ip, sp);
  dirichlet_dist_step<DIM>(sc, G, live && code < 0, st.pt, ddist, lane);
  if (BSTART) firstR = 0.0f;
  DIAG_ADD_LONE(D_TAIL, D_L_TAIL, t_tail, lone);
  DIAG_ADD_LONE(D_STEP, D_L_STEP, t_step, lone);
  if (live) gc.yukawa = g.yukawa;
  return code;
}

template <int DIM, int NC, bool REC>
__device__ __forceinline__ void walk_finish(const DevScene& sc, const DevParams& prm, const DevTasks& tk, int64_t t,
                                            int code, WalkState<DIM, NC, REC>& st, uint32_t wsteps, unsigned int* s_ctr) {
  flush_source<DIM>(st);
  const bool recorded = code == WC_DIRICHLET || code == WC_RR;
  if (recorded) {
    const float term = (code == WC_DIRICHLET && !prm.ignore_dirichlet) ? dirichlet_value<DIM>(sc, st.pt) : 0.0f;
    if constexpr (REC) {
      const DevTape& tp = *st.tape;
      const bool own_g = code == WC_DIRICHLET && !prm.ignore_dirichlet && sc.dimg == nullptr;
      if (st.rn > st.rcap) *tp.overflow = 1u;
      tp.cnt[t] = (st.rn < st.rcap ? st.rn : st.rcap) | (own_g ? kTapeOwnG : 0u);
      tp.thr_end[t] = st.throughput;
      tp.term[t] = term;
      tp.tneu[t] = st.totalNeumann;
    } else if constexpr (NC == 1) {
      const float tot = st.throughput * term + st.totalNeumann + st.totalSource[0];
      if (!WOS_ACCT_NOREC) tk.total[t] = tot;
    } else {
      const bool own_g = code == WC_DIRICHLET && !prm.ignore_dirichlet && sc.dimg == nullptr;
      for (int c = 0; c < NC; c++) {
        const float tot = st.throughput * (own_g ? sc.g_ch[c] : term) + st.totalNeumann + st.totalSource[c];
        if (!WOS_ACCT_NOREC && c < sc.n_channels) tk.total[(int64_t)c * tk.T + t] = tot;
      }
    }
  }
  if (!WOS_ACCT_NOREC) tk.code[t] = (wsteps << 1) | (recorded ? 1u : 0u);
  DIAG_MAX(D_WMAXLEN, wsteps);
  atomicAdd(&s_ctr[recorded ? C_STEPS : C_WASTED], wsteps);
  atomicAdd(&s_ctr[code == WC_DIRICHLET ? C_DIR : code == WC_RR ? C_RR : code == WC_ESCAPED ? C_ESC : C_MAXL], 1u);
}

__device__ __forceinline__ void flush_walk_counters(unsigned long long* counters, const unsigned int* s_ctr) {
  if (threadIdx.x < C_NUM && threadIdx.x != C_ITERS && threadIdx.x != C_PTS) {
    unsigned int v = threadIdx.x == C_REC ? s_ctr[C_RR] + s_ctr[C_DIR] : s_ctr[threadIdx.x];
    if (v) atomicAdd(&counters[threadIdx.x], (unsigned long long)v);
  }
}

#ifndef WOS_TASK_GRAB
#define WOS_TASK_GRAB 64
#endif
constexpr unsigned int kTaskGrab = WOS_TASK_GRAB;
#ifndef WOS_TASK_GRAB3
#define WOS_TASK_GRAB3 128u
#endif
#ifndef WOS_TASK_QUEUES
#define WOS_TASK_QUEUES 8
#endif
constexpr unsigned int kTaskQueues = WOS_TASK_QUEUES;
#ifndef WOS_TASK_GRAB_HEAD
#define WOS_TASK_GRAB_HEAD 16
#endif
#ifndef WOS_TASK_HEAD
#define WOS_TASK_HEAD 1
#endif
constexpr unsigned int kTaskGrabHead = WOS_TASK_GRAB_HEAD;
constexpr unsigned int kTaskHead = WOS_TASK_HEAD;
static_assert((kTaskQueues & (kTaskQueues - 1)) == 0 && kTaskQueues <= (unsigned)kMaxTaskQueues, "power of two");


constexpr int kSpreadMax = 32;
template <int DIM, int NC = 1>
constexpr int walk_pack_words() { return (3 * DIM + 6 + 4 + 2 * (NC - 1)) + 1 + 2 + 3; }
static_assert(sizeof(WalkState<2>) == 4 * (3 * 2 + 6 + 4), "WalkState<2> members");
static_assert(sizeof(WalkState<3>) == 4 * (3 * 3 + 6 + 4), "WalkState<3> members");
static_assert(sizeof(WalkState<2, kMaxChannels>) == 4 * (3 * 2 + 6 + 4 + 2 * (kMaxChannels - 1)), "WalkState<2, NC> members");
static_assert(sizeof(Gfn<2, false>) == 4 * (1 + 3 * 2 + 9) && sizeof(Gfn<3, true>) == 4 * (1 + 3 * 3 + 9), "Gfn members");
static_assert(sizeof(Pcg32) == 8, "Pcg32 state");
template <int DIM, bool RB, int NC, bool REC>
__device__ __forceinline__ void spread_put(uint32_t* mb, int slot, const WalkState<DIM, NC, REC>& st, const Gfn<DIM, RB>& g,
                                           const Pcg32& ws, float ddist, float firstR, uint32_t wsteps, uint32_t t) {
  int q = 0;
  auto put = [&](uint32_t v) {
    mb[(q++) * kSpreadMax + slot] = v;
  };
  auto putf = [&](float v) { put(__float_as_uint(v)); };
  for (int k = 0; k < DIM; k++) { putf(st.pt[k]); putf(st.n[k]); putf(st.prevDir[k]); }
  putf(st.prevDist); putf(st.throughput); put(st.onNeumann ? 1u : 0u); put((uint32_t)st.walkLength);
  putf(st.totalNeumann);
  for (int c = 0; c < NC; c++) putf(st.totalSource[c]);
  putf(st.pThr); putf(st.pNrm);
  for (int c = 0; c < NC; c++) putf(st.pTex[c]);
  put(st.pend ? 1u : 0u);
  put((uint32_t)g.yukawa);
  put((uint32_t)ws.state); put((uint32_t)(ws.state >> 32));
  (void)firstR;
  putf(ddist); put(wsteps); put(t);
}
template <int DIM, bool RB, int NC, bool REC>
__device__ __forceinline__ void spread_get(const uint32_t* mb, int slot, WalkState<DIM, NC, REC>& st, Gfn<DIM, RB>& g,
                                           Pcg32& ws, float& ddist, float& firstR, uint32_t& wsteps, int64_t& t) {
  int q = 0;
  auto get = [&]() { return mb[(q++) * kSpreadMax + slot]; };
  auto getf = [&]() { return __uint_as_float(get()); };
  for (int k = 0; k < DIM; k++) { st.pt[k] = getf(); st.n[k] = getf(); st.prevDir[k] = getf(); }
  st.prevDist = getf(); st.throughput = getf(); st.onNeumann = get() != 0u; st.walkLength = (int)get();
  st.totalNeumann = getf();
  for (int c = 0; c < NC; c++) st.totalSource[c] = getf();
  st.pThr = getf(); st.pNrm = getf();
  for (int c = 0; c < NC; c++) st.pTex[c] = getf();
  st.pend = get() != 0u;
  g.yukawa = (int)get();
  const uint32_t lo = get(), hi = get();
  ws.state = ((uint64_t)hi << 32) | lo;
  ddist = getf(); firstR = 0.0f; wsteps = get(); t = (int64_t)get();
}
struct SpreadLDS {
  uint32_t busy, idle;
  uint32_t mbox[kBlock / kWave];
// ... 250 lines not shown
```

neural-monte-carlo-fluid-simulation_amd/csrc/wos_kernel.hip:

```cpp
#include "wos_device.h"
#include <algorithm>
#include "wos_launch.h"
#include "wos_select.h"

namespace wos {

__global__ __launch_bounds__(256) void wos_lpt_scatter_kernel(const DevTasks tk, int64_t n) {
  __shared__ uint32_t cnt[kCostBuckets], base[kCostBuckets], off[kCostBuckets];
  if (threadIdx.x < kCostBuckets) {
    cnt[threadIdx.x] = 0u;
    uint32_t acc = 0;
    for (int b = kCostBuckets - 1; b > (int)threadIdx.x; b--) acc += tk.hist[b];
    off[threadIdx.x] = acc;
  }
  __syncthreads();
  const int64_t i = (int64_t)blockIdx.x * blockDim.x + threadIdx.x;
  int b = 0;
  uint32_t local = 0;
  if (i < n) {
    b = (tk.pstate[i] >> 8) & (kCostBuckets - 1);
    local = atomicAdd(&cnt[b], 1u);
  }
  __syncthreads();
  if (threadIdx.x < kCostBuckets && cnt[threadIdx.x])
    base[threadIdx.x] = off[threadIdx.x] + atomicAdd(&tk.hist[kCostBuckets + threadIdx.x], cnt[threadIdx.x]);
  __syncthreads();
  if (i < n) tk.perm[base[b] + local] = (uint32_t)i;
}

#define UNIT_FIRST_BALLS(X) X(2, false, 1) X(3, false, 1)
#define UNIT_WALKS(X)                         \
  X(2, false, false, false, true, false, 1)   \
  X(2, false, false, false, false, false, 1)  \
  X(2, true, false, false, true, false, 1)    \
  X(2, true, false, false, false, false, 1)   \
  X(2, false, false, false, true, true, 1)    \
  X(2, false, false, false, false, true, 1)   \
  X(3, false, false, false, true, false, 1)   \
  X(3, false, false, false, false, false, 1)  \
  X(3, true, false, false, true, false, 1)    \
  X(3, true, false, false, false, false, 1)
UNIT_FIRST_BALLS(WOS_FIRST_BALL_INSTANTIATE)
template __global__ void wos_point_setup_kernel<2>(const DevScene, const DevParams, const float*, int64_t,
                                                   const DevTasks);
template __global__ void wos_point_setup_kernel<3>(const DevScene, const DevParams, const float*, int64_t,
                                                   const DevTasks);
UNIT_WALKS(WOS_WALK_INSTANTIATE)
UnitKernels unit_kernels_plain(const KernelVariant& v) {
  UnitKernels k;
  UNIT_FIRST_BALLS(WOS_FIRST_BALL_SELECT)
  UNIT_WALKS(WOS_WALK_SELECT)
  return k;
}
template __global__ void wos_fold_kernel<2>(const DevParams, const DevTasks, int64_t, float*, float*, int32_t*,
                                            int32_t*);
template __global__ void wos_fold_kernel<3>(const DevParams, const DevTasks, int64_t, float*, float*, int32_t*,
                                            int32_t*);
template __global__ void wos_fold4_kernel<3>(const DevParams, const DevTasks, int64_t, float*, float*, int32_t*,
                                             int32_t*, float*, float*);
template __global__ void wos_fold4_kernel<2>(const DevParams, const DevTasks, int64_t, float*, float*, int32_t*,
                                             int32_t*, float*, float*);
template __global__ void wos_fold4_kernel<3, true>(const DevParams, const DevTasks, int64_t, float*, float*,
                                                   int32_t*, int32_t*, float*, float*);
template __global__ void wos_fold4_kernel<2, true>(const DevParams, const DevTasks, int64_t, float*, float*,
                                                   int32_t*, int32_t*, float*, float*);

__global__ void wos_math_selftest_kernel(int which, const double* x, double* out, int64_t n) {
  int64_t i = (int64_t)blockIdx.x * blockDim.x + threadIdx.x;
  if (i >= n) return;
  double v = x[i], r = 0.0;
  switch (which) {
    case 0: r = dexp(v); break;
    case 1: r = dlog(v); break;
    case 2: { double s, c; dsincos(v, &s, &c); r = s; } break;
    case 3: { double s, c; dsincos(v, &s, &c); r = c; } break;
    case 4: r = datan(v); break;
    case 5: r = __builtin_sqrt(v); break;
    case 6: r = bessi0(v); break;
    case 7: r = bessi1(v); break;
    case 8: r = bessk0(v); break;
    case 9: r = bessk1(v); break;
    case 10: r = (double)fexp((float)v); break;
    case 11: r = (double)flog((float)v); break;
    case 12: r = (double)fsin((float)v); break;
    case 13: r = (double)fcos((float)v); break;
    case 14: r = (double)fcbrt((float)v); break;
    case 15: r = (double)__builtin_sqrtf((float)v); break;
    case 16: r = (double)i0_fast((float)v); break;
    case 17: r = (double)k0_fast((float)v); break;
    case 18: { double a, b; bessel_ik<true, false>(v, &r, &a, nullptr, nullptr); (void)b; } break;
    case 19: { double a; bessel_ik<false, true>(v, nullptr, nullptr, &r, &a); } break;
    case 20: { double a; bessel_ik<true, false>(v, &a, &r, nullptr, nullptr); } break;
    case 21: { double a; bessel_ik<false, true>(v, nullptr, nullptr, &a, &r); } break;
    case 22: { double a, b, c; bessel_ik<true, true>(v, &a, &r, &b, &c); } break;
    case 23: { double a, b, c; bessel_ik<true, true>(v, &a, &b, &c, &r); } break;
    case 24: { float k, i; k0i0_fast((float)v, &k, &i); r = (double)i; } break;
    case 25: { float k, i; k0i0_fast((float)v, &k, &i); r = (double)k; } break;
    default: r = __builtin_nan("");
  }
  out[i] = r;
}


static UnitKernels kernels_of(const KernelVariant& v) {
  UnitKernels k;
  for (UnitKernels (*unit)(const KernelVariant&) : {unit_kernels_plain, unit_kernels_channels, unit_kernels_robust,
                                                    unit_kernels_channels_rb, unit_kernels_bstart}) {
    const UnitKernels u = unit(v);
    if (u.first_ball) k.first_ball = u.first_ball;
    if (u.walk) k.walk = u.walk;
  }
  return k;
}

hipError_t launch_first_balls(const KernelVariant& v, const DevScene& sc, const DevParams& prm, const float* pts,
                              int64_t n, int64_t base, int64_t stride, const DevTasks& tk,
                              unsigned long long* counters, unsigned int* work, int grid, size_t shmem, int lhs_floats,
                              hipStream_t s) {
  const FirstBallKernel kernel = kernels_of(v).first_ball;
  if (!kernel) return hipErrorInvalidValue;
  hipLaunchKernelGGL(kernel, dim3(grid), dim3(kBlock), shmem, s, sc, prm, pts, n, base, stride, tk, counters, work,
                     lhs_floats);
  return hipGetLastError();
}

hipError_t launch_point_setup(int dim, const DevScene& sc, const DevParams& prm, const float* pts, int64_t n,
                              const DevTasks& tk, hipStream_t s) {
  const int grid = (int)((n * kSetupLanes + 255) / 256);
  if (grid < 1) return hipSuccess;
  if (dim == 2) hipLaunchKernelGGL(wos_point_setup_kernel<2>, dim3(grid), dim3(256), 0, s, sc, prm, pts, n, tk);
  else hipLaunchKernelGGL(wos_point_setup_kernel<3>, dim3(grid), dim3(256), 0, s, sc, prm, pts, n, tk);
  return hipGetLastError();
}

__global__ __launch_bounds__(256) void wos_zero_kernel(unsigned long long* a, int n64, uint32_t* b, int n32) {
  const int i0 = blockIdx.x * blockDim.x + threadIdx.x, di = gridDim.x * blockDim.x;
  for (int i = i0; i < n64; i += di) a[i] = 0ull;
  for (int i = i0; i < n32; i += di) b[i] = 0u;
}

hipError_t launch_zero(unsigned long long* a, int n64, uint32_t* b, int n32, hipStream_t s) {
  const int grid = std::max(1, std::min(32, (std::max(n64, n32 / 2) + 1023) / 1024));
  hipLaunchKernelGGL(wos_zero_kernel, dim3(grid), dim3(256), 0, s, a, n64, b, n32);
  return hipGetLastError();
}

hipError_t launch_lpt_order(const DevTasks& tk, int64_t n, hipStream_t s) {
  const int grid = (int)((n + 255) / 256);
  if (grid > 0) hipLaunchKernelGGL(wos_lpt_scatter_kernel, dim3(grid), dim3(256), 0, s, tk, n);
  return hipGetLastError();
}

hipError_t launch_walks(const KernelVariant& v, const DevScene& sc, const DevParams& prm, const DevTasks& tk,
                        int64_t base, int64_t stride, unsigned long long* counters, unsigned int* tqueue, int grid,
                        size_t shmem, int geom_floats, hipStream_t s) {
  const WalkKernel kernel = kernels_of(v).walk;
  if (!kernel) return hipErrorInvalidValue;
  hipLaunchKernelGGL(kernel, dim3(grid), dim3(kBlock), shmem, s, sc, prm, tk, base, stride, counters, tqueue,
                     geom_floats);
  return hipGetLastError();
}

hipError_t launch_fold(int dim, const DevParams& prm, const DevTasks& tk, int64_t n, float* p, float* g,
                       int32_t* nest, int32_t* steps, float* p_var, float* g_var, hipStream_t s) {
  if (tk.deriv == nullptr) {
    const int g4 = (int)((n + kFold4Points - 1) / kFold4Points);
    if (g4 < 1) return hipSuccess;
    const dim3 blk(4 * kFold4Points);
    if (p_var || g_var) {
      if (dim == 3)
        hipLaunchKernelGGL((wos_fold4_kernel<3, true>), dim3(g4), blk, 0, s, prm, tk, n, p, g, nest, steps, p_var, g_var);
      else
        hipLaunchKernelGGL((wos_fold4_kernel<2, true>), dim3(g4), blk, 0, s, prm, tk, n, p, g, nest, steps, p_var, g_var);
    } else if (dim == 3) {
      hipLaunchKernelGGL((wos_fold4_kernel<3>), dim3(g4), blk, 0, s, prm, tk, n, p, g, nest, steps, nullptr, nullptr);
    } else {
      hipLaunchKernelGGL((wos_fold4_kernel<2>), dim3(g4), blk, 0, s, prm, tk, n, p, g, nest, steps, nullptr, nullptr);
    }
    return hipGetLastError();
  }
  if (p_var || g_var) return hipErrorInvalidValue;
  const int grid = (int)((n + kFoldPoints - 1) / kFoldPoints);
  if (grid < 1) return hipSuccess;
  if (dim == 2)
    hipLaunchKernelGGL(wos_fold_kernel<2>, dim3(grid), dim3(kFoldPoints), 0, s, prm, tk, n, p, g, nest, steps);
  else
    hipLaunchKernelGGL(wos_fold_kernel<3>, dim3(grid), dim3(kFoldPoints), 0, s, prm, tk, n, p, g, nest, steps);
  return hipGetLastError();
}

size_t first_ball_wave_lds_bytes(int lhs_floats, int n_pairs) {
  const int P = fb_points_per_wave(n_pairs);
  return (size_t)2 * P * lhs_floats * sizeof(float) + fb_union_bytes(P * lhs_floats, 2 * n_pairs);
}

int first_ball_points_per_wave(int n_pairs) { return fb_points_per_wave(n_pairs); }

size_t walk_wave_lds_bytes(int dim) { return dim == 2 ? walk_scratch_bytes<2>() : walk_scratch_bytes<3>(); }

hipError_t occupancy_blocks_per_cu(const KernelVariant& v, int which, size_t shmem, int* blocks) {
  const UnitKernels k = kernels_of(v);
  const void* kernel = which == 0 ? (const void*)k.first_ball : which == 1 ? (const void*)k.walk : nullptr;
  if (!kernel) return hipErrorInvalidValue;
  return hipOccupancyMaxActiveBlocksPerMultiprocessor(blocks, kernel, kBlock, shmem);
}

void diag_dump(const char* tag) {
  diag_print(tag, HIP_SYMBOL(g_diag));
#if WOS_TIMELINE
  static unsigned long long tl[1 + TL_NUM * kTlBins];
  hipMemcpyFromSymbol(tl, HIP_SYMBOL(g_tl), sizeof(tl));
  const double bt = (double)(1u << kTlShift);
  int last = 0;
  for (int b = 0; b < kTlBins; b++)
    if (tl[1 + TL_WAVE * kTlBins + b]) last = b;
  fprintf(stderr, "[timeline %s] bin_us %.2f (bin: busy waves, live lanes, lanes/busy wave, tasks handed out, walks finished)\n",
          tag, bt / 100.0);
  for (int b = 0; b <= last; b++) {
    const double w = tl[1 + TL_WAVE * kTlBins + b] / bt, l = tl[1 + TL_LANE * kTlBins + b] / bt;
    fprintf(stderr, "[timeline %s] %3d %8.1f %9.1f %6.2f %9llu %9llu\n", tag, b, w, l, w > 0 ? l / w : 0.0,
            tl[1 + TL_START * kTlBins + b], tl[1 + TL_FIN * kTlBins + b]);
  }
  static unsigned long long z[1 + TL_NUM * kTlBins];
  hipMemcpyToSymbol(HIP_SYMBOL(g_tl), z, sizeof(z));
#endif
}

void diag_print(const char* tag, const void* sym) {
#if WOS_DIAG
  unsigned long long d[D_NUM];
  hipMemcpyFromSymbol(d, sym, sizeof(d));
  fprintf(stderr, "[diag %s] iters %llu lanes/iter %.2f  cycles/iter: step %.0f star %.0f ray %.0f sample %.0f loop %.0f  ray_overflow %llu\n",
          tag, d[D_ITERS], (double)d[D_LANES] / (double)(d[D_ITERS] ? d[D_ITERS] : 1),
          (double)d[D_STEP] / d[D_ITERS], (double)d[D_STAR] / d[D_ITERS], (double)d[D_RAY] / d[D_ITERS],
          (double)d[D_SAMPLE] / d[D_ITERS], (double)d[D_LOOP] / d[D_ITERS], d[D_RAYOVF]);
  const double fp = (double)(d[D_FB_PTS] ? d[D_FB_PTS] : 1);
  fprintf(stderr, "[diag %s] first-ball: points %llu cycles/point: setup %.0f lhs %.0f balls %.0f total %.0f\n", tag,
          d[D_FB_PTS], d[D_FB_SETUP] / fp, d[D_FB_LHS] / fp, d[D_FB_BALLS] / fp, d[D_FB_TOTAL] / fp);
  fprintf(stderr, "[diag %s] first-ball parts cycles/point: ball update %.0f  sample (member a) %.0f  member a %.0f  member b %.0f  stores %.0f\n",
          tag, d[D_FB_UPD] / fp, d[D_FB_SMP] / fp, d[D_FB_MA] / fp, d[D_FB_MB] / fp, d[D_FB_ST] / fp);
  fprintf(stderr, "[diag %s] first-ball source samples: rejection iterations per point: sum over lanes %.1f, max over lanes %.1f\n",
          tag, d[D_FB_ITSUM] / fp, d[D_FB_ITMAX] / fp);
  fprintf(stderr, "[diag %s] step parts cycles/iter: mid (ball update) %.0f  end %.0f  tail %.0f\n", tag,
          (double)d[D_MID] / (d[D_ITERS] ? d[D_ITERS] : 1), (double)d[D_END] / (d[D_ITERS] ? d[D_ITERS] : 1),
          (double)d[D_TAIL] / (d[D_ITERS] ? d[D_ITERS] : 1));
  fprintf(stderr, "[diag %s] rejection: calls %llu, lanes/call %.1f, generations/call %.2f, items/call %.1f, quick-rejected %.1f%%, undecided %.3f%%\n",
          tag, d[D_RCALLS], (double)d[D_RLANES] / (d[D_RCALLS] ? d[D_RCALLS] : 1), (double)d[D_RGENS] / (d[D_RCALLS] ? d[D_RCALLS] : 1),
          (double)d[D_RITEMS] / (d[D_RCALLS] ? d[D_RCALLS] : 1), 100.0 * d[D_RQUICK] / (d[D_RITEMS] ? d[D_RITEMS] : 1),
          100.0 * d[D_RUND] / (d[D_RITEMS] ? d[D_RITEMS] : 1));
  fprintf(stderr, "[diag %s] max cycles/point (first balls) %llu, longest walk %llu steps, longest walk-kernel wave %llu cycles\n",
          tag, d[D_FB_MAX], d[D_WMAXLEN], d[D_WAVEMAX]);
  fprintf(stderr, "[diag %s] star calls %llu: groups visited/call %.2f, candidates/call %.2f, exact/call %.2f\n", tag,
          d[D_SCALLS], (double)d[D_SGVISIT] / d[D_SCALLS], (double)d[D_SCAND] / d[D_SCALLS],
          (double)d[D_SEXACT] / d[D_SCALLS]);
  fprintf(stderr, "[diag %s] after the queue ran dry: %llu iterations (%.1f%%), lanes/iter %.2f, %.1f%% of loop cycles\n",
          tag, d[D_XITERS], 100.0 * d[D_XITERS] / (d[D_ITERS] ? d[D_ITERS] : 1),
          (double)d[D_XLANES] / (d[D_XITERS] ? d[D_XITERS] : 1), 100.0 * d[D_XLOOP] / (d[D_LOOP] ? d[D_LOOP] : 1));
  const double li = (double)(d[D_L_ITERS] ? d[D_L_ITERS] : 1);
  fprintf(stderr, "[diag %s] <=2 live lanes: %llu iterations, cycles/iter: loop %.0f step %.0f star %.0f (cell %.0f prefix %.0f "
                  "window %.0f final %.0f) mid %.0f ray %.0f end %.0f sample %.0f tail %.0f\n",
          tag, d[D_L_ITERS], d[D_L_LOOP] / li, d[D_L_STEP] / li, d[D_L_STAR] / li, d[D_L_S_CELL] / li, d[D_L_S_PFX] / li,
          d[D_L_S_WIN] / li, d[D_L_S_FIN] / li, d[D_L_MID] / li, d[D_L_RAY] / li, d[D_L_END] / li, d[D_L_SAMPLE] / li,
          d[D_L_TAIL] / li);
  fprintf(stderr, "[diag %s] <=2 live lanes star detail: prologue %.0f  list build+sync %.0f  star total (in-function) %.0f\n", tag,
          d[D_L_S_PRE] / li, d[D_L_S_BUILD] / li, d[D_L_S_POST] / li);
  unsigned long long z[D_NUM] = {};
  hipMemcpyToSymbol(sym, z, sizeof(z));
#else
  (void)tag;
  (void)sym;
#endif
}

hipError_t launch_math_selftest(int which, const double* x, double* out, int64_t n, hipStream_t s) {
  int grid = (int)((n + 255) / 256);
  if (grid < 1) grid = 1;
  hipLaunchKernelGGL(wos_math_selftest_kernel, dim3(grid), dim3(256), 0, s, which, x, out, n);
  return hipGetLastError();
}

}
```

neural-monte-carlo-fluid-simulation_amd/csrc/wos_launch.h:

```cpp
#pragma once
#include <hip/hip_runtime.h>
#include "wos_scene.h"
#include "wos_variant.h"

namespace wos {
constexpr int kBlockThreads = 256;
constexpr int kWavesPerBlockHost = 4;
constexpr int kNumCounters = 9;
constexpr int kTaskQueueSlot0 = kNumCounters + 8;
constexpr int kNumCounterSlots = kTaskQueueSlot0 + kMaxTaskQueues * 8;
constexpr int kMainCounterSlots = kNumCounterSlots;

hipError_t launch_first_balls(const KernelVariant& v, const DevScene& sc, const DevParams& prm, const float* pts,
                              int64_t n, int64_t base, int64_t stride, const DevTasks& tk,
                              unsigned long long* counters, unsigned int* work, int grid, size_t shmem, int lhs_floats,
                              hipStream_t s);
hipError_t launch_point_setup(int dim, const DevScene& sc, const DevParams& prm, const float* pts, int64_t n,
                              const DevTasks& tk, hipStream_t s);
hipError_t launch_point_query(int dim, const DevScene& sc, int which, float mask, const float* pts, int64_t n,
                              float* dist, float* sdist, float* closest, int32_t* state, hipStream_t s);
hipError_t launch_zero(unsigned long long* a, int n64, uint32_t* b, int n32, hipStream_t s);
hipError_t launch_lpt_order(const DevTasks& tk, int64_t n, hipStream_t s);
hipError_t launch_walks(const KernelVariant& v, const DevScene& sc, const DevParams& prm, const DevTasks& tk,
                        int64_t base, int64_t stride, unsigned long long* counters, unsigned int* tqueue, int grid,
                        size_t shmem, int geom_floats, hipStream_t s);
hipError_t launch_fold(int dim, const DevParams& prm, const DevTasks& tk, int64_t n, float* p, float* g,
                       int32_t* nest, int32_t* steps, float* p_var, float* g_var, hipStream_t s);
size_t first_ball_wave_lds_bytes(int lhs_floats, int n_pairs);
int first_ball_points_per_wave(int n_pairs);
size_t walk_wave_lds_bytes(int dim);
hipError_t occupancy_blocks_per_cu(const KernelVariant& v, int which, size_t shmem, int* blocks);
void diag_dump(const char* tag);
void diag_dump_bstart(const char* tag);
void diag_print(const char* tag, const void* sym);
hipError_t launch_math_selftest(int which, const double* x, double* out, int64_t n, hipStream_t s);

hipError_t launch_lhs_selftest(int dim, const DevParams& prm, const long long* gidx, int n, float* out, hipStream_t s);
size_t lhs_selftest_lds_bytes(int n_pairs, int dim, int jump_n);
hipError_t launch_lhs_permute_selftest(int impl, const int* partner, const float* values, int nstrat, int sd, int slots,
                                       int count, float* out, hipStream_t s);
int lhs_permute_selftest_slots(int impl);
int lhs_permute_selftest_max_strata(int impl);
void lhs_plan(int n_pairs, int dim, int32_t* out);
hipError_t launch_rejection_selftest(int dim, const float* rej_tab, const float* R, const float* lambda, const float* x,
                                     int64_t n, int32_t* edges, float* vals, int32_t* flags, hipStream_t s);

hipError_t launch_bvc_point_info(const DevScene& sc, const float* pts, int64_t n, float* dd, float* nd,
                                 int32_t* inside, float* src, hipStream_t s);
hipError_t launch_bvc_start(const DevScene& sc, const DevParams& prm, const float* bpt, const float* bnrm,
                            const uint8_t* aligned, const float* bdd, int64_t nb, const DevTasks& tk, int on_neumann,
                            uint32_t tag, hipStream_t s);
hipError_t launch_bvc_fd(const DevScene& sc, const float* pts, const float* sol, int64_t n, float* dn, hipStream_t s);
hipError_t launch_bvc_fold(const DevTasks& tk, int64_t nb, float* sol, int32_t* nest, hipStream_t s);
hipError_t launch_bvc_splat_list(const float* edd, const float* end_, const int32_t* ein, int64_t ne, float cutoff,
                                 float mask, int double_sided, uint32_t* list, uint32_t* count, hipStream_t s);
hipError_t launch_bvc_splat(const float* recs, int r0, int r1, int first, int last, float* state,
                            const uint32_t* list, const uint32_t* count, const float* ept, int64_t ne,
                            float absorption, float radius_clamp, float reg, float* sol, float* grad, hipStream_t s);
hipError_t launch_bvc_fill(float* recs, int64_t b0, int64_t b1, const float* bsol, const float* bdn,
                           const DevScene& sc, int ignore_neumann, hipStream_t s);
hipError_t launch_first_balls_rec(int dim, const DevScene& sc, const DevParams& prm, const float* pts, int64_t n,
                                  int64_t base, int64_t stride, const DevTasks& tk, const DevTape& tape,
                                  unsigned long long* counters, unsigned int* work, int grid, size_t shmem,
                                  int lhs_floats, hipStream_t s);
hipError_t launch_walks_rec(int dim, bool geom_global, const DevScene& sc, const DevParams& prm, const DevTasks& tk,
                            const DevTape& tape, int64_t base, int64_t stride, unsigned long long* counters,
                            unsigned int* tqueue, int grid, size_t shmem, int geom_floats, hipStream_t s);
hipError_t occupancy_rec_blocks_per_cu(int dim, bool geom_global, int which, size_t shmem, int* blocks);
constexpr int64_t tape_slot_blocks(int64_t T) { return (T + 1 + 2047) / 2048; }
hipError_t launch_tape_slots(const uint32_t* code, int64_t T, uint32_t* slot, unsigned long long* bsum, hipStream_t s);
hipError_t launch_tape_stats(const uint32_t* code, const uint32_t* cnt, int64_t T, unsigned long long* out,
                             hipStream_t s);
hipError_t launch_tape_replay(const DevTape& tape, const uint32_t* code, const DevScene& sc, int ignore_source,
                              int64_t T, float* total, float* first, hipStream_t s);
hipError_t launch_tape_adjoint_fold(int dim, const DevParams& prm, const uint32_t* code, const float* bdir,
                                    const float* sdir, const int32_t* pstate, int64_t n, int64_t T, int wpp,
                                    int n_channels, const float* up_p, const float* up_g, int64_t up_stride,
                                    float* a, float* c, hipStream_t s);
hipError_t launch_tape_scatter(const DevTape& tape, const uint32_t* code, int64_t cells, int n_channels, int64_t T,
                               const float* a, const float* c, float* out, hipStream_t s);
constexpr int kTapeIndexTile = 1024;
struct DevTapeIndex {
  const uint32_t* row;
  const uint32_t* cell;
  const uint32_t* id;
  const float* w;
  float* part;
  uint32_t n_terms;
};
constexpr int64_t tape_index_tiles(int64_t n_terms) { return (n_terms + kTapeIndexTile - 1) / kTapeIndexTile; }
hipError_t launch_tape_index_enum(const DevTape& tape, const uint32_t* code, int64_t T, int64_t slots, int64_t cells,
                                  uint32_t* key, unsigned long long* val, hipStream_t s);
hipError_t tape_index_sort(void* temp, size_t* temp_bytes, const uint32_t* key_in, uint32_t* key_out,
                           const unsigned long long* val_in, unsigned long long* val_out, int64_t N, int bits,
                           hipStream_t s);
hipError_t launch_tape_index_count(const uint32_t* key, int64_t N, uint32_t* n_terms, hipStream_t s);
hipError_t launch_tape_index_finish(const uint32_t* key, const unsigned long long* val, uint32_t n_terms,
                                    int64_t cells, uint32_t* row, uint32_t* cell, uint32_t* id, float* w,
                                    hipStream_t s);
hipError_t launch_tape_rowsum(const DevTapeIndex& ix, int64_t cells, int n_channels, int64_t T, const float* a,
                              const float* c, float* out, hipStream_t s);
// ... 3 lines not shown
```

neural-monte-carlo-fluid-simulation_amd/csrc/wos_scene.h:

```cpp
#pragma once
#include <stdint.h>

namespace wos {

constexpr int kPrimStride2 = 4, kPrimStride3 = 9;
constexpr int kAuxStride2 = 6, kAuxStride3 = 21;
constexpr int kSilStride2 = 8, kSilStride3 = 16;
constexpr int kMaxChannels = 4;
constexpr int kGroup = 8, kGroupStride = 8, kSGroupStride = 16;

constexpr int kTreeLevels = 8;
constexpr int kTreeMinGroups = 64;
struct DevTree {
  const float* node;
  int32_t levels;
  int32_t n[kTreeLevels + 1];
  int32_t off[kTreeLevels + 1];
};

template <int DIM> struct Layout;
template <> struct Layout<2> {
  static constexpr int prim = kPrimStride2, aux = kAuxStride2, sil = kSilStride2;
};
template <> struct Layout<3> {
// ... 14 lines not shown
  const float* dgroup;
  int32_t n_pgroups, n_sgroups, n_dgroups;
  DevTree ptree, stree, dtree;
  const float* nbvh_box;
  const int32_t* nbvh_child;
  const int32_t* nbvh_ref;
  int32_t nbvh_branch;
  int32_t geom_global;
  int32_t sdims[3];
  float pmin[3], pmax[3], ext[3];
  float absorption;
  float g_dirichlet;
  const float* dimg;
  int32_t ddims[2];
  float dbox[4];
  const float* nimg;
  int32_t ndims[2];
  float nbox[4];
  int32_t watertight;
  int32_t double_sided;
  const uint32_t* sgrid;
  int32_t sgrid_words, sgrid_off_words;
  int32_t sgrid_n[3];
  float sgrid_min[3], sgrid_inv[3];
  const uint32_t* dgrid;
  int32_t dgrid_off_words;
  int32_t dgrid_n[2];
  float dgrid_min[2], dgrid_inv[2];
  int32_t n_channels;
  float g_ch[kMaxChannels];
};

struct DevParams {
  int32_t n_walks;
  int32_t n_pairs;
  int32_t n_anti;
  int32_t max_walk_length;
  int32_t steps_before_tikhonov;
  int32_t steps_before_maximal_spheres;
  float epsilon_shell;
  float min_star_radius;
  float silhouette_precision;
  float rr_threshold;
  float boundary_distance_mask;
  int32_t use_cv;
  int32_t use_cosine;
  int32_t ignore_dirichlet;
  int32_t ignore_neumann;
  int32_t ignore_source;
  int32_t robust;
  int32_t neumann_inert;
  int32_t force_estimate;
  int32_t tail_spread;
  int32_t wave_prio;
  uint64_t seed;
  const uint64_t* jump;
  int32_t n_jump;
  int32_t lhs_jump_n;
  const float* rej_tab;
};

constexpr int kMaxTaskQueues = 32;
constexpr unsigned int kTaskQueueStride = 16;
constexpr int kRejTabBins = 96;
constexpr int kLhsJumpMax = 512;
constexpr float kRejTabScale = 8.0f;

struct DevTasks {
  float* pt;
  float* thr;
  float* tsrc;
  float* dd;
  float* first;
  float* bdir;
  float* sdir;
  float* total;
  uint32_t* code;
  int32_t* pstate;
  uint32_t* perm;
  uint32_t* hist;
  float* prad;
  int64_t T;
  int32_t wpp;
  float* n0;
  float* r0;
  uint32_t* sflags;
  float* pball;
  int64_t pball_stride;
  const float* ddir;
  float* deriv;
};

struct DevTape {
  float* gnorm;
  uint32_t* cell0;
  const uint32_t* slot;
  uint32_t* cnt;
  float* thr_end;
  float* term;
  float* tneu;
  uint32_t* e_cell;
  float* e_thr;
  float* e_nrm;
  uint32_t* overflow;
};
constexpr uint32_t kTapeOwnG = 0x80000000u;
constexpr int kTapeChunk = 64;

constexpr int task_floats(int dim, int channels = 1) { return 3 * dim + 6 + 3 * (channels - 1); }
constexpr int kCostBuckets = 32;

}
```

neural-monte-carlo-fluid-simulation_amd/csrc/wos_walk_body.inc:

```
  extern __shared__ __attribute__((aligned(16))) float smem[];
  static_assert(!REC || (!BSTART && !RB && !SPR && NC == 1), "recording: a solve's reference-semantics walks, one channel");
  __shared__ unsigned int s_ctr[C_NUM];
  __shared__ SpreadLDS s_spread;
  const DevScene& sc = sc_arg;
  const DevParams& prm = prm_arg;
  const DevTasks& tk = tk_arg;
  static_assert(walk_pack_words<DIM, NC>() * kSpreadMax * 4 <= (int)walk_scratch_bytes<DIM>(), "mailbox fits the scratch");
  static_assert(!(BSTART && NC != 1), "boundary-start walks carry one channel");
  constexpr bool kSpread = SPR;
  const int lane = threadIdx.x & (kWave - 1);
  stage_geometry<DIM, GG>(sc, smem, true);
  stage_rej_jump(prm);
  const int wave_u = __builtin_amdgcn_readfirstlane((int)(threadIdx.x / kWave));
  char* wscratch = reinterpret_cast<char*>(smem + geom_floats) + wave_u * walk_scratch_bytes<DIM>();
  StarLDS<DIM>* starL = reinterpret_cast<StarLDS<DIM>*>(wscratch);
  RayLDS<DIM>* rayL = reinterpret_cast<RayLDS<DIM>*>(wscratch);
  RejLDS* rejL = reinterpret_cast<RejLDS*>(wscratch);
  if (threadIdx.x < C_NUM) s_ctr[threadIdx.x] = 0u;
  if (threadIdx.x == 0) { s_spread.busy = blockDim.x / kWave; s_spread.idle = 0u; }
  if (threadIdx.x < kBlock / kWave) s_spread.mbox[threadIdx.x] = 0u;
#if WOS_DIAG
  if (threadIdx.x < D_NUM) s_diag[threadIdx.x] = 0u;
#endif
  __syncthreads();

  const uint32_t T = (uint32_t)tk.T;
  const uint32_t wpp = (uint32_t)tk.wpp;
  const int wsh = (wpp & (wpp - 1u)) == 0u ? __builtin_ctz(wpp) : -1;
  auto divw = [&](uint32_t x) -> uint32_t { return wsh >= 0 ? x >> wsh : x / wpp; };
  const bool yuk0 = sc.absorption > 0.0f && prm.steps_before_tikhonov == 0;
  uint32_t c_iters = 0;
  wave_priority(prm.wave_prio);
#if WOS_TIMELINE
  uint64_t tl_t0 = 0;
  if (lane == 0) {
    const unsigned long long now = __builtin_amdgcn_s_memrealtime();
    const unsigned long long old = atomicCAS(&g_tl[0], 0ull, now);
    tl_t0 = old == 0ull ? now : old;
  }
  tl_t0 = ((uint64_t)(uint32_t)__builtin_amdgcn_readfirstlane((int)(uint32_t)(tl_t0 >> 32)) << 32) |
          (uint32_t)__builtin_amdgcn_readfirstlane((int)(uint32_t)tl_t0);
  auto tl_bin = [&](uint64_t ts) -> int {
    const uint64_t b = ts > tl_t0 ? (ts - tl_t0) >> kTlShift : 0;
    return b < (uint64_t)kTlBins ? (int)b : kTlBins - 1;
  };
#endif

  DIAG_T0(t_wave);
  constexpr uint32_t kGrabD = DIM == 3 ? WOS_TASK_GRAB3 : kTaskGrab;
  const uint32_t G_win = kGrabD < 63u * wpp ? kGrabD : 63u * wpp;
  const uint32_t G_head = kTaskGrabHead < G_win ? kTaskGrabHead : G_win;
  const uint32_t n_head = (uint32_t)__builtin_amdgcn_readfirstlane((int)(kTaskHead * gridDim.x * (blockDim.x / kWave)));
  const uint32_t NH = G_head > 0u ? ((T + G_head - 1u) / G_head < n_head ? (T + G_head - 1u) / G_head : n_head) : 0u;
  const uint64_t H = (uint64_t)NH * G_head < (uint64_t)T ? (uint64_t)NH * G_head : (uint64_t)T;
  uint32_t wq = 0, we = 0, wp0 = 0, wperm = 0;
  bool exhausted = false;
  const uint32_t qhome = blockIdx.x & (kTaskQueues - 1u);
  uint32_t qdone = 0u;
  int head = 0, S = 0;
  uint32_t s_t = 0, s_ok = 0;
  auto refill = [&](const DevTasks& tk) {
    while (S < kWave && !exhausted) {
      if (wq >= we) {
        unsigned int c = 0xFFFFFFFFu, len = 0u;
        if (lane == 0) {
          for (uint32_t k = 0; k < kTaskQueues; k++) {
            const uint32_t x = (qhome + k) & (kTaskQueues - 1u);
            if ((qdone >> x) & 1u) continue;
            const uint32_t d = atomicAdd(tqueue + x * kTaskQueueStride, 1u);
            const uint32_t nhx = NH > x ? (NH - x + kTaskQueues - 1u) / kTaskQueues : 0u;
            const uint64_t st = d < nhx ? (uint64_t)(d * kTaskQueues + x) * G_head
                                        : H + (uint64_t)((uint64_t)(d - nhx) * kTaskQueues + x) * G_win;
            if (st < (uint64_t)T) {
              c = (unsigned int)st;
              len = d < nhx ? G_head : G_win;
              break;
            }
            qdone |= 1u << x;
          }
        }
        c = (unsigned int)__builtin_amdgcn_readlane((int)c, 0);
        len = (unsigned int)__builtin_amdgcn_readlane((int)len, 0);
        qdone = (uint32_t)__builtin_amdgcn_readlane((int)qdone, 0);
        if (c == 0xFFFFFFFFu) { exhausted = true; break; }
        wq = c;
        we = (T - c) < len ? T : c + len;
        wp0 = divw(c);
        const uint32_t np = divw(we - 1) - wp0 + 1;
        wperm = (uint32_t)lane < np ? tk.perm[wp0 + lane] : 0u;
      }
      const int avail = (int)(we - wq);
      const int take = (kWave - S) < avail ? (kWave - S) : avail;
      const int pos = ((lane - head) & (kWave - 1)) - S;
      const bool mine = pos >= 0 && pos < take;
      const uint32_t q = wq + (mine ? (uint32_t)pos : 0u), qp = divw(q);
      const uint32_t pidx = (uint32_t)__shfl((int)wperm, (int)(qp - wp0));
      if (mine) {
        s_t = pidx * wpp + (q - qp * wpp);
        s_ok = tk.pstate[pidx] & kPtEstimate;
      }
      S += take;
      wq += (uint32_t)take;
    }
  };
  refill(tk);
  int64_t t = -1;
  WalkState<DIM, NC, REC> st;
  if constexpr (REC) st.tape = tape;
  Gfn<DIM, RB> g;
  Pcg32 ws;
  float ddist = 0.0f;
  uint32_t wsteps = 0;
  float firstR = 0.0f;

  for (;;) {
    DIAG_T0(t_loop);
#if WOS_TIMELINE
    const uint64_t tl_a = __builtin_amdgcn_s_memrealtime();
#endif
    KernArgsPtr ka = kernargs_opaque();
    const DevScene& sc = (const DevScene&)ka->sc;
    const DevParams& prm = (const DevParams&)ka->prm;
    const DevTasks& tk = (const DevTasks&)ka->tk;
    const LGeom G = geometry_view<DIM, GG>(sc, smem, true, false);
    {
      const uint64_t need = __ballot(t < 0);
      if (need != 0 && S > 0) {
        const int rank = (int)__builtin_amdgcn_mbcnt_hi((uint32_t)(need >> 32),
                                                         __builtin_amdgcn_mbcnt_lo((uint32_t)need, 0u));
        const int k = __popcll(need);
        const int take = k < S ? k : S;
        const int src = (head + (rank < take ? rank : 0)) & (kWave - 1);
        const uint32_t v_pk = (uint32_t)__shfl((int)(s_t | (s_ok ? 0x80000000u : 0u)), src);
        const uint32_t v_t = v_pk & 0x7FFFFFFFu;
        const uint32_t v_ok = v_pk >> 31;
        float v_pt[DIM], v_thr = 0.0f, v_tsrc[NC], v_dd = 0.0f;
        for (int c = 0; c < NC; c++) v_tsrc[c] = 0.0f;
        if (t < 0 && rank < take && v_ok) {
          for (int kk = 0; kk < DIM; kk++) v_pt[kk] = tk.pt[kk * tk.T + v_t];
          v_thr = tk.thr[v_t];
          if constexpr (REC) {
          } else if constexpr (NC == 1) {
            v_tsrc[0] = tk.tsrc[v_t];
          } else {
            for (int c = 0; c < NC; c++)
              if (c < sc.n_channels) v_tsrc[c] = tk.tsrc[(int64_t)c * tk.T + v_t];
          }
          v_dd = (BSTART || sc.n_dprims > 0) ? tk.dd[v_t] : bbox_far_dist<DIM>(sc, v_pt);
        }
        if (t < 0 && rank < take) {
          t = (int64_t)v_t;
          if (!v_ok || (BSTART && (tk.sflags[t] & 2u))) {
            tk.code[t] = 0u;
            t = -1;
          } else {
            const uint32_t pidx = divw(v_t);
            const uint32_t w = (v_t - pidx * wpp) >> (prm.n_anti - 1);
            walk_start<DIM, BSTART, RB>(sc, prm, tk, t, pidx, w, v_pt, v_thr, v_tsrc, v_dd, base, stride, yuk0, st,
                                        g, ws, ddist, wsteps, firstR);
          }
        }
        head = (head + take) & (kWave - 1);
        S -= take;
#if WOS_TIMELINE
        if (lane == 0) atomicAdd(&g_tl[1 + TL_START * kTlBins + tl_bin(tl_a)], (unsigned long long)take);
#endif
      }
    }
    if (__ballot(t >= 0) == 0) {
      if (S == 0 && exhausted) {
        if (!kSpread) break;
        if (lane == 0) {
          __hip_atomic_fetch_or(&s_spread.idle, 1u << wave_u, __ATOMIC_RELEASE, __HIP_MEMORY_SCOPE_WORKGROUP);
          __hip_atomic_fetch_sub(&s_spread.busy, 1u, __ATOMIC_RELEASE, __HIP_MEMORY_SCOPE_WORKGROUP);
        }
        uint32_t n = 0;
        for (;;) {
          n = __hip_atomic_load(&s_spread.mbox[wave_u], __ATOMIC_ACQUIRE, __HIP_MEMORY_SCOPE_WORKGROUP);
          n = (uint32_t)__builtin_amdgcn_readfirstlane((int)n);
          if (n != 0u) break;
          const uint32_t busy = (uint32_t)__builtin_amdgcn_readfirstlane(
              (int)__hip_atomic_load(&s_spread.busy, __ATOMIC_ACQUIRE, __HIP_MEMORY_SCOPE_WORKGROUP));
          if (busy == 0u) break;
          __builtin_amdgcn_s_sleep(4);
        }
        if (n == 0u) break;
        const uint32_t* mb = reinterpret_cast<const uint32_t*>(wscratch);
        if ((uint32_t)lane < n) spread_get<DIM, RB>(mb, lane, st, g, ws, ddist, firstR, wsteps, t);
        wave_sync();
        if (lane == 0) __hip_atomic_store(&s_spread.mbox[wave_u], 0u, __ATOMIC_RELAXED, __HIP_MEMORY_SCOPE_WORKGROUP);
        continue;
      }
      refill(tk);
      continue;
    }
    DIAG_COUNT(D_ITERS, 1);
    DIAG_COUNT(D_LANES, __popcll(__ballot(t >= 0)));
#if WOS_DIAG
    const bool lone_it = __popcll(__ballot(t >= 0)) <= 2;
    if (lone_it) DIAG_COUNT(D_L_ITERS, 1);
#endif
    const int code = walk_iteration<DIM, GG, BSTART, RB, NEU>(sc, prm, G, t >= 0, st, g, ws, ddist, wsteps, firstR, starL,
                                                         rayL, rejL, &c_iters, lane);
#if WOS_TIMELINE
    {
      const unsigned long long nlive = (unsigned long long)__popcll(__ballot(t >= 0));
      const unsigned long long nfin = (unsigned long long)__popcll(__ballot(t >= 0 && code >= 0));
      const unsigned long long dt = __builtin_amdgcn_s_memrealtime() - tl_a;
      if (lane == 0) {
        const int b = tl_bin(tl_a);
        atomicAdd(&g_tl[1 + TL_WAVE * kTlBins + b], dt);
        atomicAdd(&g_tl[1 + TL_LANE * kTlBins + b], dt * nlive);
        if (nfin) atomicAdd(&g_tl[1 + TL_FIN * kTlBins + b], nfin);
      }
    }
#endif
    if (t >= 0 && code >= 0) {
      walk_finish<DIM>(sc, prm, tk, t, code, st, wsteps, s_ctr);
      t = -1;
    }
    if (kSpread && exhausted && S == 0) {
      const uint64_t live = __ballot(t >= 0);
      const int k = __popcll(live);
      if (k >= 2 && __builtin_amdgcn_readfirstlane(
                        (int)__hip_atomic_load(&s_spread.idle, __ATOMIC_RELAXED, __HIP_MEMORY_SCOPE_WORKGROUP)) != 0) {
        int to = -1;
        if (lane == 0) {
          uint32_t m = __hip_atomic_load(&s_spread.idle, __ATOMIC_RELAXED, __HIP_MEMORY_SCOPE_WORKGROUP);
          while (m != 0u) {
            const uint32_t b = 1u << __builtin_ctz(m);
            const uint32_t old =
                __hip_atomic_fetch_and(&s_spread.idle, ~b, __ATOMIC_ACQ_REL, __HIP_MEMORY_SCOPE_WORKGROUP);
            if (old & b) {
              __hip_atomic_fetch_add(&s_spread.busy, 1u, __ATOMIC_RELEASE, __HIP_MEMORY_SCOPE_WORKGROUP);
              to = __builtin_ctz(b);
              break;
            }
            m = old & ~b;
          }
        }
        to = __builtin_amdgcn_readlane(to, 0);
        if (to >= 0) {
          const int kd = (k / 2) < kSpreadMax ? (k / 2) : kSpreadMax;
          const int rank = (int)__builtin_amdgcn_mbcnt_hi((uint32_t)(live >> 32),
                                                         __builtin_amdgcn_mbcnt_lo((uint32_t)live, 0u));
          const bool give = t >= 0 && rank >= k - kd;
          uint32_t* mb = reinterpret_cast<uint32_t*>(reinterpret_cast<char*>(smem + geom_floats) +
                                                     to * walk_scratch_bytes<DIM>());
          if (give) {
            spread_put<DIM, RB>(mb, rank - (k - kd), st, g, ws, ddist, firstR, wsteps, (uint32_t)t);
            t = -1;
          }
          wave_sync();
          if (lane == 0)
            __hip_atomic_store(&s_spread.mbox[to], (uint32_t)kd, __ATOMIC_RELEASE, __HIP_MEMORY_SCOPE_WORKGROUP);
        }
      }
    }
    refill(tk);
#if WOS_DIAG
    DIAG_ADD_LONE(D_LOOP, D_L_LOOP, t_loop, lone_it);
#endif
#if WOS_DIAG
    if (exhausted) {
      DIAG_COUNT(D_XITERS, 1);
      DIAG_COUNT(D_XLANES, __popcll(__ballot(t >= 0)));
      DIAG_ADD(D_XLOOP, t_loop);
    }
#endif
  }
  DIAG_MAX(D_WAVEMAX, __builtin_amdgcn_s_memtime() - t_wave);
  flush_counter(counters, C_ITERS, c_iters, lane);
  __syncthreads();
#if WOS_DIAG
  if (threadIdx.x < D_NUM) {
    if (diag_is_max(threadIdx.x)) atomicMax(&g_diag[threadIdx.x], s_diag[threadIdx.x]);
    else atomicAdd(&g_diag[threadIdx.x], s_diag[threadIdx.x]);
  }
#endif
  flush_walk_counters(counters, s_ctr);
```

neural-monte-carlo-fluid-simulation_amd/wos_amd/__init__.py:

```python
from ._lib import WosError, load as load_library
from . import siren
from .engine import WalkTape, WosScene, bvc_params, load_obj, solver_params, selftest_math, selftest_lhs, selftest_lhs_permute, selftest_lhs_permute_slots, selftest_lhs_plan, selftest_tape_rowsum, selftest_rejection, device_count, release_caches, set_max_batch_tasks

__all__ = ["WalkTape", "WosScene", "WosError", "bvc_params", "load_obj", "solver_params", "selftest_math", "selftest_lhs", "selftest_lhs_permute",
           "selftest_lhs_permute_slots", "selftest_lhs_plan", "selftest_tape_rowsum", "selftest_rejection", "device_count", "set_max_batch_tasks",
           "load_library", "release_caches", "siren"]
```

neural-monte-carlo-fluid-simulation_amd/wos_amd/_lib.py:

```python
import ctypes as C
import os

PKG_DIR = os.path.dirname(os.path.dirname(os.path.abspath(__file__)))
LIB_PATH = os.environ.get("WOS_LIB_PATH") or os.path.join(PKG_DIR, "lib", "libwos_hip.so")

ABI_VERSION = 10
WOS_OK = 0
WOS_E_CAPACITY = -4
WOS_PTRS_DEVICE = 0x1
WOS_ASYNC = 0x2
MAX_CHANNELS = 4
LHS_REG1, LHS_REG2, LHS_LDS, LHS_PACK_R1, LHS_PACK_R2, LHS_SERIAL = range(6)


class WosError(RuntimeError):
    pass


class Mesh(C.Structure):
    _fields_ = [("dim", C.c_int32), ("n_vertices", C.c_int32), ("n_prims", C.c_int32),
                ("vertices", C.POINTER(C.c_float)), ("prims", C.POINTER(C.c_int32))]


class SceneDesc(C.Structure):
    _fields_ = [
        ("dim", C.c_int32),
        ("vertices", C.POINTER(C.c_float)), ("prims", C.POINTER(C.c_int32)),
        ("n_vertices", C.c_int32), ("n_prims", C.c_int32),
        ("dvertices", C.POINTER(C.c_float)), ("dprims", C.POINTER(C.c_int32)),
        ("n_dvertices", C.c_int32), ("n_dprims", C.c_int32),
        ("dirichlet_value", C.c_float), ("absorption", C.c_float),
        ("is_watertight", C.c_int32), ("is_double_sided", C.c_int32),
        ("source", C.c_void_p), ("source_dims", C.c_int32 * 3), ("source_on_device", C.c_int32),
        ("dirichlet_image", C.c_void_p), ("dirichlet_image_dims", C.c_int32 * 2),
        ("dirichlet_image_box", C.c_float * 4), ("dirichlet_image_on_device", C.c_int32),
        ("neumann_image", C.c_void_p), ("neumann_image_dims", C.c_int32 * 2),
        ("neumann_image_box", C.c_float * 4), ("neumann_image_on_device", C.c_int32),
    ]


class SceneInfo(C.Structure):
    _fields_ = [("dim", C.c_int32), ("n_prims", C.c_int32), ("n_silhouettes", C.c_int32),
                ("n_dprims", C.c_int32), ("device", C.c_int32),
                ("bbox_min", C.c_float * 3), ("bbox_max", C.c_float * 3)]


class SolverParams(C.Structure):
    _fields_ = [
        ("n_walks", C.c_int32), ("max_walk_length", C.c_int32),
        ("steps_before_tikhonov", C.c_int32), ("steps_before_maximal_spheres", C.c_int32),
        ("epsilon_shell", C.c_float), ("min_star_radius", C.c_float),
        ("silhouette_precision", C.c_float), ("russian_roulette_threshold", C.c_float),
        ("boundary_distance_mask", C.c_float),
        ("disable_gradient_control_variates", C.c_int32),
        ("disable_gradient_antithetic_variates", C.c_int32),
        ("use_cosine_sampling", C.c_int32), ("ignore_dirichlet", C.c_int32),
        ("ignore_neumann", C.c_int32), ("ignore_source", C.c_int32),
        ("seed", C.c_uint64),
        ("robust_float", C.c_int32),
        ("schedule", C.c_uint32),
    ]


SCHED_GEOM_GLOBAL = 0x1
SCHED_FULL_NEUMANN = 0x2
SCHED_NO_STAR_GRID = 0x4
SCHED_NO_DIR_GRID = 0x8
SCHED_NO_TAIL_SPREAD = 0x10
SCHED_NO_GRID_SPREAD = 0x20


class BvcParams(C.Structure):
    _fields_ = [("n_walks_solution", C.c_int32), ("n_walks_gradient", C.c_int32),
                ("boundary_cache_size", C.c_int32), ("domain_cache_size", C.c_int32),
                ("grid_res", C.c_int32), ("use_finite_differences", C.c_int32),
                ("normal_offset", C.c_float), ("radius_clamp", C.c_float),
                ("kernel_regularization", C.c_float), ("grid_box", C.c_float * 4)]


class Stats(C.Structure):
    _fields_ = [(n, C.c_uint64) for n in (
        "walk_steps", "wasted_steps", "walks_recorded", "walks_escaped", "walks_max_length",
        "walks_rr", "walks_dirichlet", "points_estimated", "rejection_iters")] + [
        (n, C.c_double) for n in ("kernel_ms", "first_ball_ms", "walk_ms", "fold_ms")] + [("walk_launches", C.c_uint64)] + [
        (n, C.c_int32) for n in ("first_ball_blocks_per_cu", "walk_blocks_per_cu", "walk_lds_bytes", "star_grid",
                                 "geom_global", "dir_grid")] + [("ticket", C.c_uint64)]

    def as_dict(self):
        return {n: (float(getattr(self, n)) if t is C.c_double else int(getattr(self, n))) for n, t in self._fields_}


class TapeInfo(C.Structure):
    _fields_ = [("dim", C.c_int32), ("n_walks", C.c_int32), ("source_dims", C.c_int32 * 3), ("device", C.c_int32),
                ("n_points", C.c_int64), ("n_tasks", C.c_int64), ("n_entries", C.c_int64),
                ("max_entries_per_walk", C.c_int64), ("bytes", C.c_int64), ("replay_chunk_entries", C.c_int32)]


class TapeIndexInfo(C.Structure):
    _fields_ = [("built", C.c_int32), ("n_segments", C.c_int32), ("n_terms", C.c_int64), ("n_cells", C.c_int64),
                ("max_terms_per_cell", C.c_int64), ("bytes", C.c_int64), ("tile_terms", C.c_int32)]


class SirenNet(C.Structure):
    _fields_ = [("d_in", C.c_int32), ("d_out", C.c_int32), ("hidden", C.c_int32), ("n_hidden_layers", C.c_int32),
                ("omega", C.c_float), ("weights", C.POINTER(C.c_void_p)), ("biases", C.POINTER(C.c_void_p))]


class AdamParams(C.Structure):
    _fields_ = [("lr", C.c_double), ("beta1", C.c_double), ("beta2", C.c_double), ("eps", C.c_double),
                ("max_grad_norm", C.c_double)]


EXPORTS = (
    "wos_load_obj", "wos_mesh_free", "wos_scene_create", "wos_scene_destroy",
    "wos_scene_get_info", "wos_scene_set_source", "wos_release_caches", "wos_default_params", "wos_solve", "wos_solve_var",
    "wos_solve_stats", "wos_default_bvc_params", "wos_bvc",
    "wos_selftest_math", "wos_selftest_lhs", "wos_selftest_lhs_permute", "wos_selftest_lhs_plan", "wos_last_error", "wos_abi_version", "wos_device_count", "wos_set_max_batch_tasks",
    "wos_scene_set_source_channels", "wos_scene_channels", "wos_solve_channels",
    "wos_tape_record", "wos_tape_solve", "wos_tape_get_info", "wos_tape_destroy",
    "wos_tape_vjp", "wos_tape_read",
    "wos_tape_index_build", "wos_tape_index_get_info", "wos_tape_index_read", "wos_tape_vjp_indexed",
    "wos_selftest_tape_rowsum", "wos_selftest_rejection",
    "wos_scene_query",
    "wos_siren_eval", "wos_selftest_siren_layer",
    "wos_siren_vjp", "wos_selftest_siren_vjp_layer",
    "wos_siren_fit",
    "wos_adam_step", "wos_siren_fit_run",
)

QUERY_NEUMANN, QUERY_DIRICHLET = 0, 1
STATE_ESTIMATED, STATE_MASK_P, STATE_MASK_GRAD, STATE_INSIDE = 1, 2, 4, 8

TAPE_FIELDS = {"code": (0, "u4"), "cnt": (1, "u4"), "slot": (2, "u4"), "cell0": (3, "u4"), "gnorm": (4, "f4"),
               "thr_end": (5, "f4"), "term": (6, "f4"), "tneu": (7, "f4"), "bdir": (8, "f4"), "sdir": (9, "f4"),
               "cell": (10, "u4"), "thr": (11, "f4"), "nrm": (12, "f4"), "pstate": (13, "i4")}
TAPE_SEGMENT_POINTS = 14
TAPE_INDEX_FIELDS = {"row": (0, "u4"), "id": (1, "u4"), "w": (2, "f4"), "cell": (3, "u4")}

_lib = None


def load():
    global _lib
    if _lib is not None:
        return _lib
    if not os.path.exists(LIB_PATH):
        raise WosError(f"{LIB_PATH} not built: run `make -C {PKG_DIR}` or __graft_entry__.build()")
    L = C.CDLL(LIB_PATH)
    L.wos_load_obj.restype = C.c_int
    L.wos_load_obj.argtypes = [C.c_char_p, C.c_int32, C.c_int32, C.c_int32, C.POINTER(Mesh)]
    L.wos_mesh_free.restype = None
    L.wos_mesh_free.argtypes = [C.POINTER(Mesh)]
    L.wos_scene_create.restype = C.c_int
    L.wos_scene_create.argtypes = [C.POINTER(SceneDesc), C.c_int32, C.POINTER(C.c_void_p)]
    L.wos_scene_destroy.restype = C.c_int
    L.wos_scene_destroy.argtypes = [C.c_void_p]
    L.wos_scene_get_info.restype = C.c_int
    L.wos_scene_get_info.argtypes = [C.c_void_p, C.POINTER(SceneInfo)]
    L.wos_scene_set_source.restype = C.c_int
    L.wos_scene_set_source.argtypes = [C.c_void_p, C.c_void_p, C.POINTER(C.c_int32), C.c_int32, C.c_void_p]
    L.wos_scene_query.restype = C.c_int
    L.wos_scene_query.argtypes = [C.c_void_p, C.c_int32, C.c_float, C.c_void_p, C.c_int64, C.c_void_p, C.c_void_p,
                                  C.c_void_p, C.c_void_p, C.c_void_p, C.c_uint32]
    L.wos_release_caches.restype = C.c_int
    L.wos_release_caches.argtypes = [C.c_int32]
    L.wos_set_max_batch_tasks.restype = C.c_int64
    L.wos_set_max_batch_tasks.argtypes = [C.c_int64]
    L.wos_default_params.restype = None
    L.wos_default_params.argtypes = [C.POINTER(SolverParams)]
    L.wos_solve.restype = C.c_int
    L.wos_solve.argtypes = [C.c_void_p, C.POINTER(SolverParams), C.c_void_p, C.c_int64, C.c_int64,
                            C.c_int64, C.c_void_p, C.c_void_p, C.c_void_p, C.c_void_p,
                            C.POINTER(Stats), C.c_void_p, C.c_uint32]
    L.wos_solve_var.restype = C.c_int
    L.wos_solve_var.argtypes = [C.c_void_p, C.POINTER(SolverParams), C.c_void_p, C.c_int64, C.c_int64,
                                C.c_int64, C.c_void_p, C.c_void_p, C.c_void_p, C.c_void_p, C.c_void_p,
                                C.c_void_p, C.POINTER(Stats), C.c_void_p, C.c_uint32]
    L.wos_scene_set_source_channels.restype = C.c_int
    L.wos_scene_set_source_channels.argtypes = [C.c_void_p, C.c_void_p, C.c_int32, C.POINTER(C.c_int32),
                                                C.POINTER(C.c_float), C.c_int32, C.c_void_p]
    L.wos_scene_channels.restype = C.c_int32
    L.wos_scene_channels.argtypes = [C.c_void_p]
    L.wos_solve_channels.restype = C.c_int
    L.wos_solve_channels.argtypes = [C.c_void_p, C.POINTER(SolverParams), C.c_void_p, C.c_int64, C.c_int64,
                                     C.c_int64, C.c_int32, C.c_void_p, C.c_void_p, C.c_void_p, C.c_void_p,
                                     C.c_void_p, C.c_void_p, C.POINTER(Stats), C.c_void_p, C.c_uint32]
    L.wos_solve_stats.restype = C.c_int
    L.wos_solve_stats.argtypes = [C.c_void_p, C.c_uint64, C.POINTER(Stats)]
    L.wos_tape_record.restype = C.c_int
    L.wos_tape_record.argtypes = [C.c_void_p, C.POINTER(SolverParams), C.c_void_p, C.c_int64, C.c_int64, C.c_int64,
                                  C.c_int64, C.POINTER(C.c_void_p), C.POINTER(Stats), C.c_void_p, C.c_uint32]
    L.wos_tape_solve.restype = C.c_int
    L.wos_tape_solve.argtypes = [C.c_void_p, C.c_void_p, C.c_int32, C.c_void_p, C.c_void_p, C.c_void_p, C.c_void_p,
                                 C.c_void_p, C.c_void_p, C.POINTER(Stats), C.c_void_p, C.c_uint32]
    L.wos_tape_get_info.restype = C.c_int
    L.wos_tape_get_info.argtypes = [C.c_void_p, C.POINTER(TapeInfo)]
    L.wos_tape_destroy.restype = C.c_int
    L.wos_tape_destroy.argtypes = [C.c_void_p]
    L.wos_tape_vjp.restype = C.c_int
    L.wos_tape_vjp.argtypes = [C.c_void_p, C.c_void_p, C.c_int32, C.c_void_p, C.c_void_p, C.c_void_p,
                               C.POINTER(Stats), C.c_void_p, C.c_uint32]
    L.wos_tape_read.restype = C.c_int
    L.wos_tape_read.argtypes = [C.c_void_p, C.c_int32, C.c_int32, C.c_int64, C.c_int64, C.c_void_p]
    L.wos_tape_index_build.restype = C.c_int
    L.wos_tape_index_build.argtypes = [C.c_void_p, C.c_int64]
    L.wos_tape_index_get_info.restype = C.c_int
    L.wos_tape_index_get_info.argtypes = [C.c_void_p, C.POINTER(TapeIndexInfo)]
    L.wos_tape_index_read.restype = C.c_int
    L.wos_tape_index_read.argtypes = [C.c_void_p, C.c_int32, C.c_int32, C.c_int64, C.c_int64, C.c_void_p]
    L.wos_tape_vjp_indexed.restype = C.c_int
    L.wos_tape_vjp_indexed.argtypes = L.wos_tape_vjp.argtypes
    L.wos_selftest_tape_rowsum.restype = C.c_int
    L.wos_selftest_tape_rowsum.argtypes = [C.c_void_p, C.c_int64, C.c_void_p, C.c_void_p, C.c_void_p, C.c_void_p,
                                           C.c_int64, C.c_int32, C.c_void_p, C.POINTER(C.c_int32), C.c_int32]
    L.wos_siren_eval.restype = C.c_int
    L.wos_siren_eval.argtypes = [C.POINTER(SirenNet), C.c_void_p, C.c_int64, C.c_void_p, C.c_void_p, C.c_void_p,
                                 C.c_uint32, C.c_int32, C.c_void_p]
    L.wos_selftest_siren_layer.restype = C.c_int
    L.wos_selftest_siren_layer.argtypes = [C.c_int32, C.c_int32, C.c_int64, C.c_void_p, C.c_void_p, C.c_void_p,
                                           C.c_void_p, C.c_int32]
    L.wos_siren_vjp.restype = C.c_int
    L.wos_siren_vjp.argtypes = [C.POINTER(SirenNet), C.c_void_p, C.c_int64, C.c_void_p, C.c_void_p, C.c_void_p,
                                C.POINTER(C.c_void_p), C.POINTER(C.c_void_p), C.c_size_t, C.c_uint32, C.c_int32,
                                C.c_void_p]
    L.wos_siren_fit.restype = C.c_int
    L.wos_siren_fit.argtypes = [C.POINTER(SirenNet), C.c_void_p, C.c_int64, C.c_void_p, C.c_void_p, C.c_void_p,
                                C.POINTER(C.c_void_p), C.POINTER(C.c_void_p), C.c_size_t, C.c_uint32, C.c_int32,
                                C.c_void_p]
    L.wos_adam_step.restype = C.c_int
    L.wos_adam_step.argtypes = [C.c_int32, C.POINTER(C.c_int64), C.POINTER(C.c_void_p), C.POINTER(C.c_void_p),
                                C.c_void_p, C.c_void_p, C.c_int64, C.POINTER(AdamParams), C.c_void_p, C.c_uint32,
                                C.c_int32, C.c_void_p]
    L.wos_siren_fit_run.restype = C.c_int
    L.wos_siren_fit_run.argtypes = [C.POINTER(SirenNet), C.c_void_p, C.c_void_p, C.c_void_p, C.c_int64, C.c_void_p,
                                    C.c_int64, C.c_int64, C.c_void_p, C.c_void_p, C.c_int64, C.POINTER(AdamParams),
                                    C.c_float, C.c_int32, C.c_void_p, C.c_void_p, C.c_size_t, C.c_uint32, C.c_int32,
                                    C.c_void_p]
    L.wos_selftest_siren_vjp_layer.restype = C.c_int
    L.wos_selftest_siren_vjp_layer.argtypes = [C.c_int32, C.c_int32, C.c_int64, C.c_void_p, C.c_void_p, C.c_void_p,
                                               C.c_void_p, C.c_void_p, C.c_int32]
    L.wos_default_bvc_params.restype = None
    L.wos_default_bvc_params.argtypes = [C.POINTER(BvcParams)]
    L.wos_bvc.restype = C.c_int
    L.wos_bvc.argtypes = [C.c_void_p, C.POINTER(SolverParams), C.POINTER(BvcParams), C.c_void_p, C.c_void_p,
                          C.c_void_p, C.c_int64, C.c_void_p, C.POINTER(Stats)]
    L.wos_selftest_math.restype = C.c_int
    L.wos_selftest_math.argtypes = [C.c_int32, C.c_void_p, C.c_void_p, C.c_int64, C.c_int32]
    L.wos_selftest_lhs.restype = C.c_int
    L.wos_selftest_lhs.argtypes = [C.c_uint64, C.c_void_p, C.c_int64, C.c_int32, C.c_int32, C.c_int32, C.c_void_p,
                                   C.c_int32]
# ... 23 lines not shown
```

neural-monte-carlo-fluid-simulation_amd/wos_amd/engine.py:

```python
import ctypes as C
import os

import numpy as np

from . import _lib
from ._lib import BvcParams, SceneDesc, SceneInfo, SolverParams, Stats, WosError, check

_DEFAULT_SEED = 0x5EED0001


def load_obj(path, dim, flip_orientation=False, normalize=False):
    L = _lib.load()
    m = _lib.Mesh()
    check(L.wos_load_obj(os.fsencode(path), dim, int(flip_orientation), int(normalize), C.byref(m)),
          f"wos_load_obj({path})")
    try:
        v = np.ctypeslib.as_array(m.vertices, shape=(m.n_vertices * dim,)).copy().reshape(-1, dim)
        ix = np.ctypeslib.as_array(m.prims, shape=(m.n_prims * dim,)).copy().reshape(-1, dim)
    finally:
        L.wos_mesh_free(C.byref(m))
    return v.astype(np.float32), ix.astype(np.int32)


def _get_opt(d, key, default, typ):
# ... 519 lines not shown
                raise WosError(f"WalkTape.vjp: {name} must have shape {shp}, got {tuple(u.shape)}")
        if sc.source_shape is None:
            raise WosError("WalkTape.vjp: the scene has no source grid")
        on_dev = any(_is_torch(u) and u.is_cuda for u in (grad_p, grad_grad))
        st = Stats()
        if on_dev:
            import torch
            dev = next(u.device for u in (grad_p, grad_grad) if _is_torch(u) and u.is_cuda)
            up = [None if u is None else torch.as_tensor(u).detach().to(dev, torch.float32).contiguous()
                  for u in (grad_p, grad_grad)]
            out = torch.empty(sc.source_shape, dtype=torch.float32, device=dev)
            cur = torch.cuda.current_stream(dev)
            if stream is None:
                s = cur.cuda_stream
            else:
                ts = stream if isinstance(stream, torch.cuda.Stream) else torch.cuda.ExternalStream(int(stream),
                                                                                                    device=dev)
                s = ts.cuda_stream
                ts.wait_stream(cur)
            ptr = lambda t: t.data_ptr() if t is not None else None
            flags = _lib.WOS_PTRS_DEVICE
        else:
            up = [None if u is None else np.ascontiguousarray(u.detach().cpu().numpy() if _is_torch(u) else u,
                                                              dtype=np.float32) for u in (grad_p, grad_grad)]
            out = np.empty(sc.source_shape, np.float32)
            ptr = lambda a: a.ctypes.data if a is not None else None
            s, flags = stream, 0
        if deterministic:
            self.build_index()
        fn = "wos_tape_vjp_indexed" if deterministic else "wos_tape_vjp"
        check(getattr(L, fn)(self._h, sc._h, nch, ptr(up[0]), ptr(up[1]), ptr(out), C.byref(st), s, flags), fn)
        self.last_vjp_stats = st.as_dict()
        return out

    def read(self, field, segment=0):
        L = _lib.load()
        if field not in _lib.TAPE_FIELDS:
            raise WosError(f"WalkTape.read: unknown field {field!r} (one of {', '.join(_lib.TAPE_FIELDS)})")
        fid, dtype = _lib.TAPE_FIELDS[field]
        npts = np.zeros(1, np.int64)
        check(L.wos_tape_read(self._h, segment, _lib.TAPE_SEGMENT_POINTS, 0, 1, npts.ctypes.data), "wos_tape_read")
        info = self.info
        T = int(npts[0]) * (info["n_tasks"] // max(1, info["n_points"]))
        dim = info["dim"]
        if field in ("cell", "thr", "nrm"):
            last = np.zeros(1, np.uint32)
            check(L.wos_tape_read(self._h, segment, _lib.TAPE_FIELDS["slot"][0], T, 1, last.ctypes.data), "wos_tape_read")
            shape = (int(last[0]),)
        else:
            shape = {"slot": (T + 1,), "bdir": (dim, T), "sdir": (dim, T), "pstate": (int(npts[0]),)}.get(field, (T,))
        out = np.empty(shape, dtype)
        check(L.wos_tape_read(self._h, segment, fid, 0, out.size, out.ctypes.data), "wos_tape_read")
        return out

    @property
    def segments(self):
        L = _lib.load()
        out, npts = [], np.zeros(1, np.int64)
        while sum(out) < self._n:
            check(L.wos_tape_read(self._h, len(out), _lib.TAPE_SEGMENT_POINTS, 0, 1, npts.ctypes.data), "wos_tape_read")
            out.append(int(npts[0]))
        return out

    def close(self):
        if getattr(self, "_h", None):
            _lib.load().wos_tape_destroy(self._h)
            self._h = None

    def __del__(self):
        try:
            self.close()
        except Exception:
            pass


def release_caches(device=-1):
    check(_lib.load().wos_release_caches(int(device)), "wos_release_caches")


def set_max_batch_tasks(n):
    return int(_lib.load().wos_set_max_batch_tasks(int(n)))


def selftest_math(which, x, device=0):
    x = np.ascontiguousarray(x, dtype=np.float64)
    out = np.empty_like(x)
    check(_lib.load().wos_selftest_math(which, x.ctypes.data, out.ctypes.data, x.size, device),
          "wos_selftest_math")
    return out


def selftest_rejection(dim, R, lam, x, device=0):
    R = np.ascontiguousarray(R, dtype=np.float32).reshape(-1)
    lam = np.ascontiguousarray(lam, dtype=np.float32).reshape(-1)
    x = np.ascontiguousarray(x, dtype=np.float32).reshape(-1)
    if not (R.size == lam.size == x.size):
        raise WosError("R, lam and x must have one length")
    edges = np.empty((R.size, 6), np.int32)
    vals = np.empty((R.size, 3), np.float32)
    flags = np.empty(R.size, np.int32)
    check(_lib.load().wos_selftest_rejection(int(dim), R.ctypes.data, lam.ctypes.data, x.ctypes.data, R.size,
                                             edges.ctypes.data, vals.ctypes.data, flags.ctypes.data, device),
          "wos_selftest_rejection")
    return edges, vals, flags


def selftest_lhs(key, gidx, n_pairs, dim, jump_lds=True, device=0):
    gidx = np.ascontiguousarray(gidx, dtype=np.int64).reshape(-1)
    out = np.empty((gidx.size, 2 * int(n_pairs), int(dim) - 1), np.float32)
    check(_lib.load().wos_selftest_lhs(int(key), gidx.ctypes.data, gidx.size, int(n_pairs), int(dim),
                                       int(bool(jump_lds)), out.ctypes.data, device), "wos_selftest_lhs")
    return out


def selftest_lhs_permute_slots(impl):
    return 2 if impl == _lib.LHS_PACK_R1 else 1


def selftest_lhs_permute(impl, partner, values, slots=1, device=0):
    partner = np.ascontiguousarray(partner, dtype=np.int32)
    values = np.ascontiguousarray(values, dtype=np.float32)
    cap = selftest_lhs_permute_slots(impl)
    if partner.ndim != 4 or values.ndim != 4 or partner.shape[1] != cap or \
            values.shape != (partner.shape[0], cap, partner.shape[3], partner.shape[2]):
        raise WosError(f"partner must be [count, {cap}, sd, nstrat] and values [count, {cap}, nstrat, sd]")
    count, _, sd, nstrat = partner.shape
    out = np.empty_like(values)
    check(_lib.load().wos_selftest_lhs_permute(int(impl), partner.ctypes.data, values.ctypes.data, nstrat, sd,
                                               int(slots), count, out.ctypes.data, device),
          "wos_selftest_lhs_permute")
    return out


def selftest_lhs_plan(n_pairs, dim):
    out = np.zeros(9, np.int32)
    check(_lib.load().wos_selftest_lhs_plan(int(n_pairs), int(dim), out.ctypes.data), "wos_selftest_lhs_plan")
    keys = ("points_per_wave", "one_pass", "shuffle", "pair_passes", "jump_mixed", "wave_lds_bytes", "lds_budget",
            "point_grab", "shuffle_chunks")
    return {k: int(v) for k, v in zip(keys, out)}


def selftest_tape_rowsum(row, id, w, a, c, device=0):
    row = np.ascontiguousarray(row, dtype=np.uint32)
    id = np.ascontiguousarray(id, dtype=np.uint32)
    w = np.ascontiguousarray(w, dtype=np.float32)
    a = np.ascontiguousarray(a, dtype=np.float32)
    c = np.ascontiguousarray(c, dtype=np.float32)
    if a.shape != c.shape or a.ndim not in (1, 2) or id.shape != w.shape or row.ndim != 1 or row.size < 2:
        raise WosError("selftest_tape_rowsum: row [n_rows + 1], id / w [n_terms], a / c [C, T] or [T]")
    nch = 1 if a.ndim == 1 else a.shape[0]
    if id.size != int(row[-1]):
        raise WosError(f"selftest_tape_rowsum: {id.size} terms, row[-1] = {int(row[-1])}")
    out = np.empty((nch, row.size - 1), np.float32)
    tile = C.c_int32(0)
    check(_lib.load().wos_selftest_tape_rowsum(row.ctypes.data, row.size - 1, id.ctypes.data, w.ctypes.data,
                                               a.ctypes.data, c.ctypes.data, a.shape[-1], nch, out.ctypes.data,
                                               C.byref(tile), device), "wos_selftest_tape_rowsum")
    return (out[0] if a.ndim == 1 else out), int(tile.value)


def device_count():
    return int(_lib.load().wos_device_count())
```

Before: 6.214 billion.

## Schedule long walks first using length hints recorded from an identical prior solve

Adds a length-hint mechanism for 2D single-chunk solves. During a solve, the walk kernel records which tasks ran long into a bitmap and list, keyed by a hash of every parameter, the geometry content, the seed and the point indexing. If the next solve has an identical key, a build kernel turns those hints into an express list. Some waves claim these long tasks first, at raised wave priority, to shorten the tail of the walk phase. The benefit only appears when consecutive calls are bit-identical (same seed and points), and the change adds extra kernels, atomics and bookkeeping to every hinted solve.

Measured after the change: 7.103 billion (median of 6 runs). 1.14x the previous value.

```diff
diff --git a/include/wos.h b/include/wos.h
--- a/include/wos.h
+++ b/include/wos.h
@@ -77,6 +77,11 @@
 
 int64_t wos_set_max_batch_tasks(int64_t max_tasks);
 
+void wos_set_length_hints(int32_t hint_min, int32_t express_min, int32_t express_per_wave, int32_t capacity,
+                          int32_t priority);
+int wos_length_hint_stats(int32_t device, int64_t *out);
+int32_t wos_selftest_hint_key(int32_t field);
+
 typedef struct wos_scene_info {
     int32_t dim, n_prims, n_silhouettes, n_dprims, device;
     float bbox_min[3], bbox_max[3];
@@ -116,6 +121,7 @@
 #define WOS_SCHED_NO_DIR_GRID   0x8u
 #define WOS_SCHED_NO_TAIL_SPREAD 0x10u
 #define WOS_SCHED_NO_GRID_SPREAD 0x20u
+#define WOS_SCHED_NO_LENGTH_HINTS (0x40u)
 
 void wos_default_params(wos_solver_params *p);
 
diff --git a/neural-monte-carlo-fluid-simulation_amd/csrc/wos_capi.h b/neural-monte-carlo-fluid-simulation_amd/csrc/wos_capi.h
--- a/neural-monte-carlo-fluid-simulation_amd/csrc/wos_capi.h
+++ b/neural-monte-carlo-fluid-simulation_amd/csrc/wos_capi.h
@@ -92,6 +92,22 @@
   hipEvent_t done = nullptr;
 };
 constexpr int kSideWs = 2;
+
+struct HintKey {
+  int32_t dim = 0, wpp = 0, n_walks = 0, n_anti = 0;
+  int64_t n = 0, index_base = 0, index_stride = 0;
+  uint64_t seed = 0, geometry = 0;
+  int32_t max_walk_length = 0, steps_before_tikhonov = 0, steps_before_maximal_spheres = 0;
+  int32_t use_cosine = 0, ignore_dirichlet = 0, ignore_neumann = 0, ignore_source = 0, force_estimate = 0;
+  int32_t watertight = 0, double_sided = 0;
+  float epsilon_shell = 0, min_star_radius = 0, silhouette_precision = 0, rr_threshold = 0, absorption = 0;
+  bool operator==(const HintKey& o) const;
+};
+struct HintTuning {
+  int32_t hint_min, express_min, express_per_wave, capacity, priority;
+};
+extern std::mutex g_hint_mu;
+extern HintTuning g_hint_tuning;
 
 struct DevCtx {
   std::mutex mu;
@@ -121,6 +137,13 @@
   float* d_rejtab = nullptr;
   int stat_waiters = 0;
   std::condition_variable no_waiters;
+  void* d_hint_list = nullptr;
+  uint32_t* d_hint_express = nullptr;
+  uint32_t* d_hint_bits = nullptr;
+  int64_t hint_bits_tasks = 0;
+  HintKey hint_key;
+  bool hint_key_valid = false;
+  bool hint_last = false;
   TaskWs side[kSideWs];
   hipStream_t bvc_dir = nullptr;
   hipEvent_t bvc_dir_done = nullptr;
@@ -142,6 +165,7 @@
                            int channels = 1);
 wos::DevTasks task_view(DevCtx& c, int dim, int64_t T, int32_t wpp, int channels = 1);
 int ensure_jump(DevCtx& c, int k_needed);
+int ensure_hints(DevCtx& c, int64_t tasks, uint32_t** hc);
 const std::vector<float>& rejection_tables();
 
 int slot_open(DevCtx& c, hipStream_t st, int64_t n_events, int64_t n_batches, const RunShape& shape, StatSlot** out);
@@ -173,6 +197,7 @@
   int device = 0;
   int dim = 2, double_sided = 0;
   std::vector<float> v, dv;
+  uint64_t content_id = 0;
   std::vector<int32_t> ix, dix;
   wos::HostScene host;
   float *d_prim = nullptr, *d_paux = nullptr, *d_sil = nullptr, *d_dprim = nullptr, *d_dpaux = nullptr;
@@ -260,7 +285,7 @@
 };
 Batches batches(int64_t n, int64_t wpp);
 int batch_head(DevCtx& c, int dim, const SolvePlan& P, int64_t k, const float* d_pts, int64_t nb,
-               const wos::DevTasks& tk, hipEvent_t after_zero, hipStream_t st);
+               const wos::DevTasks& tk, hipEvent_t after_zero, hipStream_t st, unsigned long long* cksum = nullptr);
 int fold_channels(int dim, const wos::DevParams& dp, const wos::DevTasks& tk, int C, int64_t nb, int64_t b0,
                   int64_t n, const SolveOut& out, hipStream_t st);
 
diff --git a/neural-monte-carlo-fluid-simulation_amd/csrc/wos_capi_ctx.cpp b/neural-monte-carlo-fluid-simulation_amd/csrc/wos_capi_ctx.cpp
--- a/neural-monte-carlo-fluid-simulation_amd/csrc/wos_capi_ctx.cpp
+++ b/neural-monte-carlo-fluid-simulation_amd/csrc/wos_capi_ctx.cpp
@@ -11,6 +11,21 @@
 static_assert(WOS_BATCH_LOG2 <= 30, "task indices carry a flag in bit 31 (wos_walk_kernel hand-out)");
 constexpr int64_t kDefaultBatchTasks = (int64_t)1 << WOS_BATCH_LOG2;
 std::atomic<int64_t> g_max_batch_tasks{kDefaultBatchTasks};
+
+constexpr HintTuning kDefaultHintTuning = {24, 40, 4, (int32_t)wos::kHintListMax, 0};
+std::mutex g_hint_mu;
+HintTuning g_hint_tuning = kDefaultHintTuning;
+
+bool HintKey::operator==(const HintKey& o) const {
+  return dim == o.dim && wpp == o.wpp && n_walks == o.n_walks && n_anti == o.n_anti && n == o.n &&
+         index_base == o.index_base && index_stride == o.index_stride && seed == o.seed && geometry == o.geometry &&
+         max_walk_length == o.max_walk_length && steps_before_tikhonov == o.steps_before_tikhonov &&
+         steps_before_maximal_spheres == o.steps_before_maximal_spheres && use_cosine == o.use_cosine &&
+         ignore_dirichlet == o.ignore_dirichlet && ignore_neumann == o.ignore_neumann &&
+         ignore_source == o.ignore_source && force_estimate == o.force_estimate && watertight == o.watertight &&
+         double_sided == o.double_sided && epsilon_shell == o.epsilon_shell && min_star_radius == o.min_star_radius &&
+         silhouette_precision == o.silhouette_precision && rr_threshold == o.rr_threshold && absorption == o.absorption;
+}
 
 static void ctx_free(DevCtx& c) {
   hipFree(c.d_pts); hipFree(c.d_p); hipFree(c.d_g); hipFree(c.d_nest); hipFree(c.d_steps);
@@ -19,6 +34,11 @@
   c.ws_var_points = 0;
   hipFree(c.d_jump); hipFree(c.d_tasks); hipFree(c.d_pstate); hipFree(c.d_counters); hipFree(c.d_rejtab);
   c.d_rejtab = nullptr;
+  hipFree(c.d_hint_list); hipFree(c.d_hint_express); hipFree(c.d_hint_bits);
+  c.d_hint_list = nullptr; c.d_hint_express = nullptr; c.d_hint_bits = nullptr;
+  c.hint_bits_tasks = 0;
+  c.hint_key_valid = false;
+  c.hint_last = false;
   for (StatSlot& q : c.slot) {
     if (q.ev0) hipEventDestroy(q.ev0);
     if (q.ev1) hipEventDestroy(q.ev1);
@@ -70,6 +90,7 @@
   }
   HIP_TRY(hipDeviceGetAttribute(&c.num_cus, hipDeviceAttributeMultiprocessorCount, device));
   HIP_TRY(hipMalloc((void**)&c.d_counters, wos::kMainCounterSlots * sizeof(unsigned long long)));
+  HIP_TRY(hipMemset(c.d_counters, 0, wos::kMainCounterSlots * sizeof(unsigned long long)));
   for (StatSlot& q : c.slot) {
     HIP_TRY(hipHostMalloc((void**)&q.h_cnt, wos::kNumCounters * sizeof(unsigned long long)));
     HIP_TRY(hipEventCreate(&q.ev0));
@@ -170,6 +191,29 @@
   return task_view_in(c.d_tasks, c.d_pstate, c.pstate_cap, dim, T, wpp, channels);
 }
 
+int ensure_hints(DevCtx& c, int64_t tasks, uint32_t** hc_out) {
+  uint32_t* const hc = (uint32_t*)(c.d_counters + wos::kNumCounterSlots);
+  *hc_out = hc;
+  if (c.d_hint_list && tasks <= c.hint_bits_tasks) return WOS_OK;
+  hipFree(c.d_hint_list); hipFree(c.d_hint_express); hipFree(c.d_hint_bits);
+  c.d_hint_list = nullptr; c.d_hint_express = nullptr; c.d_hint_bits = nullptr;
+  c.hint_bits_tasks = 0;
+  c.hint_key_valid = false;
+  const size_t words = (size_t)((tasks + 31) / 32);
+  HIP_TRY(hipMalloc(&c.d_hint_list, (size_t)wos::kHintListMax * 2 * sizeof(uint32_t)));
+  HIP_TRY(hipMalloc((void**)&c.d_hint_express, (size_t)wos::kHintListMax * sizeof(uint32_t)));
+  HIP_TRY(hipMalloc((void**)&c.d_hint_bits, words * sizeof(uint32_t)));
+  HIP_TRY(hipMemset(c.d_hint_bits, 0, words * sizeof(uint32_t)));
+  uint32_t h[wos::H_WORDS] = {};
+  const auto put = [&](int at, const void* p) { std::memcpy(h + at, &p, sizeof(p)); };
+  put(wos::H_LIST, c.d_hint_list);
+  put(wos::H_EXPRESS, c.d_hint_express);
+  put(wos::H_BITS, c.d_hint_bits);
+  HIP_TRY(hipMemcpy(hc, h, sizeof(h), hipMemcpyHostToDevice));
+  c.hint_bits_tasks = tasks;
+  return WOS_OK;
+}
+
 int ensure_jump(DevCtx& c, int k_needed) {
   if (k_needed <= c.n_jump) return WOS_OK;
   const int cap = std::max(k_needed, 4096);
@@ -325,6 +369,53 @@
   return g_max_batch_tasks.exchange(v);
 }
 
+void wos_set_length_hints(int32_t hint_min, int32_t express_min, int32_t express_per_wave, int32_t capacity,
+                          int32_t priority) {
+  std::lock_guard<std::mutex> lk(g_hint_mu);
+  const HintTuning& d = kDefaultHintTuning;
+  HintTuning& t = g_hint_tuning;
+  t.hint_min = hint_min < 0 ? d.hint_min : std::min(std::max(hint_min, 1), (int32_t)wos::kHintMinMask);
+  t.express_min = express_min < 0 ? d.express_min : std::max(express_min, 1);
+  t.express_per_wave = express_per_wave < 0 ? d.express_per_wave : std::min(std::max(express_per_wave, 1), 64);
+  t.capacity = capacity < 0 ? d.capacity : std::min(std::max(capacity, 1), (int32_t)wos::kHintListMax);
+  t.priority = priority < 0 ? d.priority : std::min(priority, 3);
+}
+
+int32_t wos_selftest_hint_key(int32_t field) {
+  HintKey a, b;
+  int k = 0;
+  bool hit = false;
+  const auto bump = [&](auto& v) {
+    if (k++ == field) { v = v + 1; hit = true; }
+  };
+  bump(b.dim); bump(b.wpp); bump(b.n_walks); bump(b.n_anti); bump(b.n); bump(b.index_base); bump(b.index_stride);
+  bump(b.seed); bump(b.geometry); bump(b.max_walk_length); bump(b.steps_before_tikhonov);
+  bump(b.steps_before_maximal_spheres); bump(b.use_cosine); bump(b.ignore_dirichlet); bump(b.ignore_neumann);
+  bump(b.ignore_source); bump(b.force_estimate); bump(b.watertight); bump(b.double_sided); bump(b.epsilon_shell);
+  bump(b.min_star_radius); bump(b.silhouette_precision); bump(b.rr_threshold); bump(b.absorption);
+  static_assert(sizeof(HintKey) == 4 * 4 + 3 * 8 + 2 * 8 + 10 * 4 + 5 * 4 + 4, "a new HintKey field: compare it, bump it here");
+  if (field < 0 || !hit) return -1;
+  return a == b ? 0 : 1;
+}
+
+int wos_length_hint_stats(int32_t device, int64_t* out) {
+  if (!out) return fail(WOS_E_INVALID, "wos_length_hint_stats: null output");
+  for (int k = 0; k < 4; k++) out[k] = 0;
+  if (device < 0 || device >= kMaxDevices) return fail(WOS_E_INVALID, "wos_length_hint_stats: no such device");
+  DevCtx& c = g_ctx[device];
+  std::lock_guard<std::mutex> lk(c.mu);
+  if (!c.ready || !c.hint_last || !c.d_hint_list) return WOS_OK;
+  HIP_TRY(hipSetDevice(device));
+  if (c.inflight) HIP_TRY(hipEventSynchronize(c.done));
+  uint32_t h[wos::H_WORDS];
+  HIP_TRY(hipMemcpy(h, c.d_counters + wos::kNumCounterSlots, sizeof(h), hipMemcpyDeviceToHost));
+  out[0] = h[wos::H_CLAIMED];
+  out[1] = h[wos::H_NLIST] > h[wos::H_CAP] ? h[wos::H_NLIST] - h[wos::H_CAP] : 0;
+  out[2] = std::min(h[wos::H_NLIST], h[wos::H_CAP]);
+  out[3] = h[wos::H_NEXPRESS];
+  return WOS_OK;
+}
+
 int wos_release_caches(int32_t device) {
   int ndev = 0;
   if (hipGetDeviceCount(&ndev) != hipSuccess) ndev = 0;
diff --git a/neural-monte-carlo-fluid-simulation_amd/csrc/wos_capi_scene.cpp b/neural-monte-carlo-fluid-simulation_amd/csrc/wos_capi_scene.cpp
--- a/neural-monte-carlo-fluid-simulation_amd/csrc/wos_capi_scene.cpp
+++ b/neural-monte-carlo-fluid-simulation_amd/csrc/wos_capi_scene.cpp
@@ -49,6 +49,20 @@
   if (d->n_prims > 0) g->ix.assign(d->prims, d->prims + (size_t)d->n_prims * dim);
   if (d->n_dvertices > 0) g->dv.assign(d->dvertices, d->dvertices + (size_t)d->n_dvertices * dim);
   if (d->n_dprims > 0) g->dix.assign(d->dprims, d->dprims + (size_t)d->n_dprims * dim);
+  {
+    uint64_t h = 0xCBF29CE484222325ull;
+    const auto mix = [&](const void* p, size_t bytes) {
+      const unsigned char* b = (const unsigned char*)p;
+      for (size_t i = 0; i < bytes; i++) h = (h ^ b[i]) * 0x100000001B3ull;
+    };
+    const int32_t head[2] = {dim, d->is_double_sided};
+    mix(head, sizeof(head));
+    mix(g->v.data(), g->v.size() * sizeof(float));
+    mix(g->ix.data(), g->ix.size() * sizeof(int32_t));
+    mix(g->dv.data(), g->dv.size() * sizeof(float));
+    mix(g->dix.data(), g->dix.size() * sizeof(int32_t));
+    g->content_id = h;
+  }
   wos::HostSceneInput in;
   in.dim = dim;
   in.vertices = d->vertices; in.prims = d->prims; in.n_vertices = d->n_vertices; in.n_prims = d->n_prims;
diff --git a/neural-monte-carlo-fluid-simulation_amd/csrc/wos_capi_solve.cpp b/neural-monte-carlo-fluid-simulation_amd/csrc/wos_capi_solve.cpp
--- a/neural-monte-carlo-fluid-simulation_amd/csrc/wos_capi_solve.cpp
+++ b/neural-monte-carlo-fluid-simulation_amd/csrc/wos_capi_solve.cpp
@@ -193,12 +193,12 @@
 }
 
 int batch_head(DevCtx& c, int dim, const SolvePlan& P, int64_t k, const float* d_pts, int64_t nb,
-               const wos::DevTasks& tk, hipEvent_t after_zero, hipStream_t st) {
+               const wos::DevTasks& tk, hipEvent_t after_zero, hipStream_t st, unsigned long long* cksum) {
   HIP_TRY(wos::launch_zero(k == 0 ? c.d_counters : c.d_counters + wos::kNumCounters,
                            k == 0 ? wos::kNumCounterSlots : wos::kNumCounterSlots - wos::kNumCounters,
                            tk.hist, 2 * wos::kCostBuckets, st));
   if (after_zero) HIP_TRY(hipEventRecord(after_zero, st));
-  HIP_TRY(wos::launch_point_setup(dim, P.dfb, P.dp, d_pts, nb, tk, st));
+  HIP_TRY(wos::launch_point_setup(dim, P.dfb, P.dp, d_pts, nb, tk, st, cksum));
   HIP_TRY(wos::launch_lpt_order(tk, nb, st));
   return WOS_OK;
 }
@@ -248,10 +248,42 @@
     WOS_TRY(ensure_tasks(c, dim, bt.chunk * wpp, bt.chunk, C));
     WOS_TRY(solve_grids(c, dim, bt.chunk, false, plan));
   }
+  const bool hinted = dim == 2 && !dp.robust && dp.neumann_inert && C == 1 && bt.n_chunks == 1 && !ex.ddir &&
+                      !ex.deriv && !(prm->schedule & WOS_SCHED_NO_LENGTH_HINTS);
+  uint32_t* hc = nullptr;
+  uint32_t hint_word = 0;
+  bool hint_use = false;
+  HintTuning ht{};
+  HintKey hint_key;
+  if (hinted) {
+    {
+      std::lock_guard<std::mutex> lk(g_hint_mu);
+      ht = g_hint_tuning;
+    }
+    WOS_TRY(ensure_hints(c, bt.chunk * wpp, &hc));
+    HintKey& key = hint_key;
+    key.dim = dim; key.wpp = (int32_t)wpp; key.n_walks = dp.n_walks; key.n_anti = dp.n_anti;
+    key.n = n; key.index_base = index_base; key.index_stride = index_stride;
+    key.seed = dp.seed; key.geometry = s->geom->content_id;
+    key.max_walk_length = dp.max_walk_length; key.steps_before_tikhonov = dp.steps_before_tikhonov;
+    key.steps_before_maximal_spheres = dp.steps_before_maximal_spheres;
+    key.use_cosine = dp.use_cosine; key.ignore_dirichlet = dp.ignore_dirichlet;
+    key.ignore_neumann = dp.ignore_neumann; key.ignore_source = dp.ignore_source;
+    key.force_estimate = dp.force_estimate;
+    key.watertight = s->dev.watertight; key.double_sided = s->dev.double_sided;
+    key.epsilon_shell = dp.epsilon_shell; key.min_star_radius = dp.min_star_radius;
+    key.silhouette_precision = dp.silhouette_precision; key.rr_threshold = dp.rr_threshold;
+    key.absorption = s->dev.absorption;
+    hint_use = c.hint_key_valid && key == c.hint_key;
+    c.hint_key_valid = false;
+    hint_word = wos::kHintCollect | (hint_use ? wos::kHintUse : 0u) | ((uint32_t)ht.priority << wos::kHintPrioShift) |
+                ((uint32_t)ht.hint_min << wos::kHintMinShift);
+  }
+  if (n > 0) c.hint_last = hinted;
   StatSlot* slot = nullptr;
   WOS_TRY(slot_open(c, st, 4 * bt.n_chunks, bt.n_chunks, plan.shape(), &slot));
   StatSlot& q = *slot;
-  if (bt.n_chunks == 0) HIP_TRY(wos::launch_zero(c.d_counters, wos::kMainCounterSlots, nullptr, 0, st));
+  if (bt.n_chunks == 0) HIP_TRY(wos::launch_zero(c.d_counters, wos::kNumCounterSlots, nullptr, 0, st));
   for (int64_t k = 0; k < bt.n_chunks; k++) {
     const int64_t b0 = k * bt.chunk;
     hipEvent_t* ev = &q.bev[4 * k];
@@ -263,12 +295,22 @@
     unsigned int* q_points = (unsigned int*)(c.d_counters + wos::kNumCounters);
     unsigned int* q_tasks = (unsigned int*)(c.d_counters + wos::kTaskQueueSlot0);
     const int walk_grid = (int)std::min<int64_t>(plan.grid_walk, (tk.T + 63) / 64);
-    WOS_TRY(batch_head(c, dim, plan, k, d_pts + b0 * dim, nb, tk, ev[0], st));
+    tk.hint = hint_word;
+    WOS_TRY(batch_head(c, dim, plan, k, d_pts + b0 * dim, nb, tk, ev[0], st,
+                       hinted ? (unsigned long long*)(hc + wos::H_CK_CUR) : nullptr));
+    if (hinted)
+      HIP_TRY(wos::launch_hint_build(hc, hint_use ? 1 : 0, (uint32_t)ht.express_min, (uint32_t)ht.express_per_wave,
+                                     (uint32_t)ht.capacity, (uint32_t)walk_grid * (uint32_t)ht.express_per_wave, tk,
+                                     st));
     HIP_TRY(wos::launch_first_balls(plan.kv, plan.dfb, dp, d_pts + b0 * dim, nb, bbase, index_stride, tk,
                                     c.d_counters, q_points, plan.grid_fb, plan.shmem_fb_run, plan.lhs_floats, st));
     HIP_TRY(hipEventRecord(ev[1], st));
     HIP_TRY(wos::launch_walks(plan.kv, plan.dsc, dp, tk, bbase, index_stride, c.d_counters, q_tasks, walk_grid,
                               plan.shmem_walk, plan.geom_floats_walk, st));
+    if (hinted) {
+      c.hint_key = hint_key;
+      c.hint_key_valid = true;
+    }
     HIP_TRY(hipEventRecord(ev[2], st));
     WOS_TRY(fold_channels(dim, dp, tk, C, nb, b0, n, out.dev, st));
     HIP_TRY(hipEventRecord(ev[3], st));
diff --git a/neural-monte-carlo-fluid-simulation_amd/csrc/wos_capi_tape.cpp b/neural-monte-carlo-fluid-simulation_amd/csrc/wos_capi_tape.cpp
--- a/neural-monte-carlo-fluid-simulation_amd/csrc/wos_capi_tape.cpp
+++ b/neural-monte-carlo-fluid-simulation_amd/csrc/wos_capi_tape.cpp
@@ -163,7 +163,7 @@
   struct EvGuard { hipEvent_t& a; hipEvent_t& b; ~EvGuard() { if (a) hipEventDestroy(a); if (b) hipEventDestroy(b); } } evg{ev0, ev1};
   HIP_TRY(hipEventCreate(&ev1));
   HIP_TRY(hipEventRecord(ev0, st));
-  if (bt.n_chunks == 0) HIP_TRY(wos::launch_zero(c.d_counters, wos::kMainCounterSlots, nullptr, 0, st));
+  if (bt.n_chunks == 0) HIP_TRY(wos::launch_zero(c.d_counters, wos::kNumCounterSlots, nullptr, 0, st));
   tape->seg.reserve((size_t)bt.n_chunks);
   for (int64_t k = 0; k < bt.n_chunks; k++) {
     const int64_t b0 = k * bt.chunk;
diff --git a/neural-monte-carlo-fluid-simulation_amd/csrc/wos_device.h b/neural-monte-carlo-fluid-simulation_amd/csrc/wos_device.h
--- a/neural-monte-carlo-fluid-simulation_amd/csrc/wos_device.h
+++ b/neural-monte-carlo-fluid-simulation_amd/csrc/wos_device.h
@@ -28,7 +28,11 @@
        D_XITERS, D_XLANES, D_XLOOP,
        D_L_ITERS, D_L_STEP, D_L_STAR, D_L_MID, D_L_RAY, D_L_END, D_L_SAMPLE, D_L_TAIL, D_L_LOOP,
        D_L_S_CELL, D_L_S_PFX, D_L_S_WIN, D_L_S_FIN, D_L_S_BUILD, D_L_S_PRE, D_L_S_POST,
-       D_FB_UPD, D_FB_SMP, D_FB_MA, D_FB_MB, D_FB_ST, D_FB_ITSUM, D_FB_ITMAX, D_NUM };
+       D_FB_UPD, D_FB_SMP, D_FB_MA, D_FB_MB, D_FB_ST, D_FB_ITSUM, D_FB_ITMAX,
+#if WOS_DIAG
+       D_E_ITERS, D_E_LANES, D_E_LOOP,
+#endif
+       D_NUM };
 __host__ __device__ constexpr bool diag_is_max(int k) { return k == D_FB_MAX || k == D_WMAXLEN || k == D_WAVEMAX; }
 static __device__ unsigned long long g_diag[D_NUM];
 #if WOS_DIAG
@@ -3160,8 +3164,10 @@
 template <int DIM>
 __global__ __launch_bounds__(256) void wos_point_setup_kernel(const DevScene sc, const DevParams prm,
                                                              const float* __restrict__ pts, int64_t n,
-                                                             const DevTasks tk) {
+                                                             const DevTasks tk, unsigned long long* cksum) {
   __shared__ uint32_t s_hist[kCostBuckets];
+  __shared__ unsigned long long s_ck;
+  if (threadIdx.x == 0) s_ck = 0ull;
   __shared__ __attribute__((aligned(16))) float s_prim[kSetupLdsFloats];
   constexpr int PS = Layout<DIM>::prim;
   const int nfl = sc.n_prims * PS, dfl = sc.n_dprims * PS;
@@ -3213,10 +3219,21 @@
         }
       }
       atomicAdd(&s_hist[bucket], 1u);
+      if (DIM == 2 && cksum != nullptr) {
+        unsigned long long h = (unsigned long long)i * 0x9E3779B97F4A7C15ull;
+        for (int k = 0; k < DIM; k++) {
+          h ^= (unsigned long long)__float_as_uint(x[k]) << (k & 1 ? 32 : 0);
+          h = (h ^ (h >> 30)) * 0xBF58476D1CE4E5B9ull;
+          h = (h ^ (h >> 27)) * 0x94D049BB133111EBull;
+          h ^= h >> 31;
+        }
+        atomicAdd(&s_ck, h);
+      }
     }
   }
   __syncthreads();
   if (threadIdx.x < kCostBuckets && s_hist[threadIdx.x]) atomicAdd(&tk.hist[threadIdx.x], s_hist[threadIdx.x]);
+  if (DIM == 2 && cksum != nullptr && threadIdx.x == 0) atomicAdd(cksum, s_ck);
 }
 
 template <int DIM, bool RB = false, int NC = 1>
@@ -3232,6 +3249,11 @@
   if (level == 1) __builtin_amdgcn_s_setprio(1);
   else if (level == 2) __builtin_amdgcn_s_setprio(2);
   else if (level >= 3) __builtin_amdgcn_s_setprio(3);
+}
+
+__device__ __forceinline__ void wave_priority_set(int level) {
+  if (level <= 0) __builtin_amdgcn_s_setprio(0);
+  else wave_priority(level);
 }
 
 template <int DIM, bool BSTART, bool RB, int NC, bool REC>
@@ -3332,9 +3354,10 @@
   return code;
 }
 
-template <int DIM, int NC, bool REC>
+template <bool HINT = false, int DIM, int NC, bool REC>
 __device__ __forceinline__ void walk_finish(const DevScene& sc, const DevParams& prm, const DevTasks& tk, int64_t t,
-                                            int code, WalkState<DIM, NC, REC>& st, uint32_t wsteps, unsigned int* s_ctr) {
+                                            int code, WalkState<DIM, NC, REC>& st, uint32_t wsteps, unsigned int* s_ctr,
+                                            unsigned int* hc = nullptr) {
   flush_source<DIM>(st);
   const bool recorded = code == WC_DIRICHLET || code == WC_RR;
   if (recorded) {
@@ -3359,6 +3382,15 @@
     }
   }
   if (!WOS_ACCT_NOREC) tk.code[t] = (wsteps << 1) | (recorded ? 1u : 0u);
+  if constexpr (HINT) {
+    if ((tk.hint & kHintCollect) && wsteps >= ((tk.hint >> kHintMinShift) & kHintMinMask)) {
+      const uint32_t cap = hc[H_CAP];
+      uint32_t i = __hip_atomic_load(&hc[H_NLIST], __ATOMIC_RELAXED, __HIP_MEMORY_SCOPE_AGENT);
+      if (i < cap) i = atomicAdd(&hc[H_NLIST], 1u);
+      else atomicAdd(&s_ctr[C_PTS], 1u);
+      if (i < cap) (*reinterpret_cast<uint2* const*>(hc + H_LIST))[i] = make_uint2((uint32_t)t, wsteps);
+    }
+  }
   DIAG_MAX(D_WMAXLEN, wsteps);
   atomicAdd(&s_ctr[recorded ? C_STEPS : C_WASTED], wsteps);
   atomicAdd(&s_ctr[code == WC_DIRICHLET ? C_DIR : code == WC_RR ? C_RR : code == WC_ESCAPED ? C_ESC : C_MAXL], 1u);
diff --git a/neural-monte-carlo-fluid-simulation_amd/csrc/wos_kernel.hip b/neural-monte-carlo-fluid-simulation_amd/csrc/wos_kernel.hip
--- a/neural-monte-carlo-fluid-simulation_amd/csrc/wos_kernel.hip
+++ b/neural-monte-carlo-fluid-simulation_amd/csrc/wos_kernel.hip
@@ -42,9 +42,9 @@
   X(3, true, false, false, false, false, 1)
 UNIT_FIRST_BALLS(WOS_FIRST_BALL_INSTANTIATE)
 template __global__ void wos_point_setup_kernel<2>(const DevScene, const DevParams, const float*, int64_t,
-                                                   const DevTasks);
+                                                   const DevTasks, unsigned long long*);
 template __global__ void wos_point_setup_kernel<3>(const DevScene, const DevParams, const float*, int64_t,
-                                                   const DevTasks);
+                                                   const DevTasks, unsigned long long*);
 UNIT_WALKS(WOS_WALK_INSTANTIATE)
 UnitKernels unit_kernels_plain(const KernelVariant& v) {
   UnitKernels k;
@@ -125,11 +125,89 @@
 }
 
 hipError_t launch_point_setup(int dim, const DevScene& sc, const DevParams& prm, const float* pts, int64_t n,
-                              const DevTasks& tk, hipStream_t s) {
+                              const DevTasks& tk, hipStream_t s, unsigned long long* cksum) {
   const int grid = (int)((n * kSetupLanes + 255) / 256);
   if (grid < 1) return hipSuccess;
-  if (dim == 2) hipLaunchKernelGGL(wos_point_setup_kernel<2>, dim3(grid), dim3(256), 0, s, sc, prm, pts, n, tk);
-  else hipLaunchKernelGGL(wos_point_setup_kernel<3>, dim3(grid), dim3(256), 0, s, sc, prm, pts, n, tk);
+  if (dim == 2) hipLaunchKernelGGL(wos_point_setup_kernel<2>, dim3(grid), dim3(256), 0, s, sc, prm, pts, n, tk, cksum);
+  else hipLaunchKernelGGL(wos_point_setup_kernel<3>, dim3(grid), dim3(256), 0, s, sc, prm, pts, n, tk, cksum);
+  return hipGetLastError();
+}
+
+constexpr int kHintBins = 1024;
+__global__ __launch_bounds__(kHintBins) void wos_hint_build_kernel(uint32_t* __restrict__ hc, int use,
+                                                                   uint32_t express_min, uint32_t epw, uint32_t cap,
+                                                                   uint32_t max_express, const DevTasks tk) {
+  __shared__ uint32_t s_bin[kHintBins], s_wave[kHintBins / kWave];
+  const int tid = threadIdx.x;
+  uint32_t* const express = *reinterpret_cast<uint32_t* const*>(hc + H_EXPRESS);
+  uint32_t* const bits = *reinterpret_cast<uint32_t* const*>(hc + H_BITS);
+  const uint2* const list = *reinterpret_cast<const uint2* const*>(hc + H_LIST);
+  const unsigned long long ck_cur = *reinterpret_cast<const unsigned long long*>(hc + H_CK_CUR);
+  const unsigned long long ck_list = *reinterpret_cast<const unsigned long long*>(hc + H_CK_LIST);
+  const uint32_t n_old = hc[H_NEXPRESS];
+  const uint32_t n = hc[H_NLIST] < hc[H_CAP] ? hc[H_NLIST] : hc[H_CAP];
+  const bool ok = use != 0 && ck_cur == ck_list && hc[H_NLIST] <= hc[H_CAP];
+  const uint32_t T = (uint32_t)tk.T, wpp = (uint32_t)tk.wpp;
+  for (uint32_t i = tid; i < n_old; i += kHintBins) {
+    const uint32_t t = express[i];
+    atomicAnd(&bits[t >> 5], ~(1u << (t & 31u)));
+  }
+  s_bin[tid] = 0u;
+  __syncthreads();
+  const auto bin_of = [&](const uint2 e) -> int {
+    if (e.y < express_min || e.x >= T || !(tk.pstate[e.x / wpp] & kPtEstimate)) return -1;
+    return kHintBins - 1 - (int)(e.y < (uint32_t)kHintBins - 1u ? e.y : (uint32_t)kHintBins - 1u);
+  };
+  if (ok)
+    for (uint32_t i = tid; i < n; i += kHintBins) {
+      const int b = bin_of(list[i]);
+      if (b >= 0) atomicAdd(&s_bin[b], 1u);
+    }
+  __syncthreads();
+  const int lane = tid & (kWave - 1), wv = tid / kWave;
+  const uint32_t mine = s_bin[tid];
+  uint32_t inc = mine;
+  for (int off = 1; off < kWave; off <<= 1) {
+    const uint32_t v = (uint32_t)__shfl_up((int)inc, off);
+    if (lane >= off) inc += v;
+  }
+  if (lane == kWave - 1) s_wave[wv] = inc;
+  __syncthreads();
+  uint32_t before = 0, total = 0;
+  for (int w = 0; w < kHintBins / kWave; w++) {
+    if (w < wv) before += s_wave[w];
+    total += s_wave[w];
+  }
+  s_bin[tid] = before + inc - mine;
+  __syncthreads();
+  if (ok)
+    for (uint32_t i = tid; i < n; i += kHintBins) {
+      const uint2 e = list[i];
+      const int b = bin_of(e);
+      if (b < 0) continue;
+      const uint32_t pos = atomicAdd(&s_bin[b], 1u);
+      if (pos >= max_express) continue;
+      express[pos] = e.x;
+      atomicOr(&bits[e.x >> 5], 1u << (e.x & 31u));
+      atomicOr(&tk.pstate[e.x / wpp], kPtExpress);
+    }
+  __syncthreads();
+  if (tid == 0) {
+    hc[H_NEXPRESS] = ok ? (total < max_express ? total : max_express) : 0u;
+    hc[H_EPW] = epw;
+    hc[H_CAP] = cap;
+    hc[H_CLAIMED] = 0u;
+    hc[H_NLIST] = 0u;
+    hc[H_XCLAIM] = 0u;
+    *reinterpret_cast<unsigned long long*>(hc + H_CK_LIST) = ck_cur;
+    *reinterpret_cast<unsigned long long*>(hc + H_CK_CUR) = 0ull;
+  }
+}
+
+hipError_t launch_hint_build(uint32_t* hc, int use, uint32_t express_min, uint32_t express_per_wave, uint32_t cap,
+                             uint32_t max_express, const DevTasks& tk, hipStream_t s) {
+  hipLaunchKernelGGL(wos_hint_build_kernel, dim3(1), dim3(kHintBins), 0, s, hc, use, express_min, express_per_wave, cap,
+                     max_express, tk);
   return hipGetLastError();
 }
 
@@ -256,6 +334,8 @@
   fprintf(stderr, "[diag %s] after the queue ran dry: %llu iterations (%.1f%%), lanes/iter %.2f, %.1f%% of loop cycles\n",
           tag, d[D_XITERS], 100.0 * d[D_XITERS] / (d[D_ITERS] ? d[D_ITERS] : 1),
           (double)d[D_XLANES] / (d[D_XITERS] ? d[D_XITERS] : 1), 100.0 * d[D_XLOOP] / (d[D_LOOP] ? d[D_LOOP] : 1));
+  fprintf(stderr, "[diag %s] express waves: %llu iterations, lanes/iter %.2f, cycles/iter (loop) %.0f\n", tag, d[D_E_ITERS],
+          (double)d[D_E_LANES] / (d[D_E_ITERS] ? d[D_E_ITERS] : 1), (double)d[D_E_LOOP] / (d[D_E_ITERS] ? d[D_E_ITERS] : 1));
   const double li = (double)(d[D_L_ITERS] ? d[D_L_ITERS] : 1);
   fprintf(stderr, "[diag %s] <=2 live lanes: %llu iterations, cycles/iter: loop %.0f step %.0f star %.0f (cell %.0f prefix %.0f "
                   "window %.0f final %.0f) mid %.0f ray %.0f end %.0f sample %.0f tail %.0f\n",
diff --git a/neural-monte-carlo-fluid-simulation_amd/csrc/wos_launch.h b/neural-monte-carlo-fluid-simulation_amd/csrc/wos_launch.h
--- a/neural-monte-carlo-fluid-simulation_amd/csrc/wos_launch.h
+++ b/neural-monte-carlo-fluid-simulation_amd/csrc/wos_launch.h
@@ -9,14 +9,17 @@
 constexpr int kNumCounters = 9;
 constexpr int kTaskQueueSlot0 = kNumCounters + 8;
 constexpr int kNumCounterSlots = kTaskQueueSlot0 + kMaxTaskQueues * 8;
-constexpr int kMainCounterSlots = kNumCounterSlots;
+constexpr int kMainCounterSlots = kNumCounterSlots + H_WORDS / 2;
+static_assert(2 * (kNumCounterSlots - kTaskQueueSlot0) == kHintBlockWord, "the control block follows the task queues");
 
 hipError_t launch_first_balls(const KernelVariant& v, const DevScene& sc, const DevParams& prm, const float* pts,
                               int64_t n, int64_t base, int64_t stride, const DevTasks& tk,
                               unsigned long long* counters, unsigned int* work, int grid, size_t shmem, int lhs_floats,
                               hipStream_t s);
 hipError_t launch_point_setup(int dim, const DevScene& sc, const DevParams& prm, const float* pts, int64_t n,
-                              const DevTasks& tk, hipStream_t s);
+                              const DevTasks& tk, hipStream_t s, unsigned long long* cksum = nullptr);
+hipError_t launch_hint_build(uint32_t* hc, int use, uint32_t express_min, uint32_t express_per_wave, uint32_t cap,
+                             uint32_t max_express, const DevTasks& tk, hipStream_t s);
 hipError_t launch_point_query(int dim, const DevScene& sc, int which, float mask, const float* pts, int64_t n,
                               float* dist, float* sdist, float* closest, int32_t* state, hipStream_t s);
 hipError_t launch_zero(unsigned long long* a, int n64, uint32_t* b, int n32, hipStream_t s);
diff --git a/neural-monte-carlo-fluid-simulation_amd/csrc/wos_scene.h b/neural-monte-carlo-fluid-simulation_amd/csrc/wos_scene.h
--- a/neural-monte-carlo-fluid-simulation_amd/csrc/wos_scene.h
+++ b/neural-monte-carlo-fluid-simulation_amd/csrc/wos_scene.h
@@ -120,6 +120,7 @@
   float* prad;
   int64_t T;
   int32_t wpp;
+  uint32_t hint;
   float* n0;
   float* r0;
   uint32_t* sflags;
@@ -127,6 +128,27 @@
   int64_t pball_stride;
   const float* ddir;
   float* deriv;
+};
+
+constexpr uint32_t kHintCollect = 1u, kHintUse = 2u;
+constexpr int kHintPrioShift = 2, kHintMinShift = 8;
+constexpr uint32_t kHintMinMask = 0xFFFFu;
+constexpr int32_t kPtExpress = 1 << 16;
+constexpr uint32_t kHintListMax = 1u << 16;
+constexpr int kHintBlockWord = kMaxTaskQueues * (int)kTaskQueueStride;
+enum {
+  H_NLIST = 0,
+  H_XCLAIM = 16,
+  H_NEXPRESS = 32,
+  H_EPW,
+  H_CAP,
+  H_CLAIMED,
+  H_CK_CUR = 48,
+  H_CK_LIST = 50,
+  H_LIST = 52,
+  H_EXPRESS = 54,
+  H_BITS = 56,
+  H_WORDS = 64
 };
 
 struct DevTape {
diff --git a/neural-monte-carlo-fluid-simulation_amd/csrc/wos_walk_body.inc b/neural-monte-carlo-fluid-simulation_amd/csrc/wos_walk_body.inc
--- a/neural-monte-carlo-fluid-simulation_amd/csrc/wos_walk_body.inc
+++ b/neural-monte-carlo-fluid-simulation_amd/csrc/wos_walk_body.inc
@@ -8,6 +8,7 @@
   static_assert(walk_pack_words<DIM, NC>() * kSpreadMax * 4 <= (int)walk_scratch_bytes<DIM>(), "mailbox fits the scratch");
   static_assert(!(BSTART && NC != 1), "boundary-start walks carry one channel");
   constexpr bool kSpread = SPR;
+  constexpr bool HINT = DIM == 2 && !BSTART && !RB && !REC && NC == 1 && !NEU;
   const int lane = threadIdx.x & (kWave - 1);
   stage_geometry<DIM, GG>(sc, smem, true);
   stage_rej_jump(prm);
@@ -59,8 +60,35 @@
   uint32_t qdone = 0u;
   int head = 0, S = 0;
   uint32_t s_t = 0, s_ok = 0;
+  unsigned int* const hc = tqueue + kHintBlockWord;
+  bool xhold = false;
+  auto claim_express = [&]() -> bool {
+    if constexpr (HINT) {
+      uint32_t i0 = 0, n = 0;
+      if (lane == 0) {
+        const uint32_t nx = hc[H_NEXPRESS], epw = hc[H_EPW];
+        if (__hip_atomic_load(&hc[H_XCLAIM], __ATOMIC_RELAXED, __HIP_MEMORY_SCOPE_AGENT) < nx) {
+          i0 = atomicAdd(&hc[H_XCLAIM], epw);
+          n = i0 < nx ? (nx - i0 < epw ? nx - i0 : epw) : 0u;
+          if (n) atomicAdd(&hc[H_CLAIMED], n);
+        }
+      }
+      i0 = (uint32_t)__builtin_amdgcn_readlane((int)i0, 0);
+      n = (uint32_t)__builtin_amdgcn_readlane((int)n, 0);
+      if (n == 0u) return false;
+      const uint32_t pos = (uint32_t)((lane - head) & (kWave - 1));
+      if (pos < n) {
+        s_t = (*reinterpret_cast<const uint32_t* const*>(hc + H_EXPRESS))[i0 + pos];
+        s_ok = kPtEstimate;
+      }
+      S = (int)n;
+      return true;
+    } else {
+      return false;
+    }
+  };
   auto refill = [&](const DevTasks& tk) {
-    while (S < kWave && !exhausted) {
+    while (S < kWave && !exhausted && !(HINT && xhold)) {
       if (wq >= we) {
         unsigned int c = 0xFFFFFFFFu, len = 0u;
         if (lane == 0) {
@@ -97,12 +125,23 @@
       const uint32_t pidx = (uint32_t)__shfl((int)wperm, (int)(qp - wp0));
       if (mine) {
         s_t = pidx * wpp + (q - qp * wpp);
-        s_ok = tk.pstate[pidx] & kPtEstimate;
+        if constexpr (HINT) {
+          const uint32_t ps = (uint32_t)tk.pstate[pidx];
+          s_ok = (ps & kPtEstimate) | ((ps & (uint32_t)kPtExpress) ? 2u : 0u);
+        } else {
+          s_ok = tk.pstate[pidx] & kPtEstimate;
+        }
       }
       S += take;
       wq += (uint32_t)take;
     }
   };
+  if constexpr (HINT) {
+    if ((tk.hint & kHintUse) && (uint32_t)wave_u == (blockIdx.x & (kBlock / kWave - 1u)) && hc[H_NEXPRESS] > 0u) {
+      xhold = claim_express();
+      if (xhold) wave_priority((int)((tk.hint >> kHintPrioShift) & 3u));
+    }
+  }
   refill(tk);
   int64_t t = -1;
   WalkState<DIM, NC, REC> st;
@@ -131,9 +170,16 @@
         const int k = __popcll(need);
         const int take = k < S ? k : S;
         const int src = (head + (rank < take ? rank : 0)) & (kWave - 1);
-        const uint32_t v_pk = (uint32_t)__shfl((int)(s_t | (s_ok ? 0x80000000u : 0u)), src);
-        const uint32_t v_t = v_pk & 0x7FFFFFFFu;
-        const uint32_t v_ok = v_pk >> 31;
+        const uint32_t v_pk =
+            (uint32_t)__shfl((int)(HINT ? s_t | (s_ok << 30) : s_t | (s_ok ? 0x80000000u : 0u)), src);
+        const uint32_t v_t = v_pk & (HINT ? 0x3FFFFFFFu : 0x7FFFFFFFu);
+        const uint32_t v_ok = HINT ? (v_pk >> 30) & 1u : v_pk >> 31;
+        bool v_own = false;
+        if constexpr (HINT) {
+          if (t < 0 && rank < take && (v_pk >> 31))
+            v_own = ((*reinterpret_cast<const uint32_t* const*>(hc + H_BITS))[v_t >> 5] >> (v_t & 31u)) & 1u;
+          if (v_own) t = 0;
+        }
         float v_pt[DIM], v_thr = 0.0f, v_tsrc[NC], v_dd = 0.0f;
         for (int c = 0; c < NC; c++) v_tsrc[c] = 0.0f;
         if (t < 0 && rank < take && v_ok) {
@@ -160,6 +206,9 @@
                                         g, ws, ddist, wsteps, firstR);
           }
         }
+        if constexpr (HINT) {
+          if (v_own) t = -1;
+        }
         head = (head + take) & (kWave - 1);
         S -= take;
 #if WOS_TIMELINE
@@ -168,6 +217,11 @@
       }
     }
     if (__ballot(t >= 0) == 0) {
+      if (HINT && xhold && S == 0) {
+        xhold = claim_express();
+        if (xhold) continue;
+        wave_priority_set(prm.wave_prio);
+      }
       if (S == 0 && exhausted) {
         if (!kSpread) break;
         if (lane == 0) {
@@ -216,10 +270,12 @@
     }
 #endif
     if (t >= 0 && code >= 0) {
-      walk_finish<DIM>(sc, prm, tk, t, code, st, wsteps, s_ctr);
+      walk_finish<HINT>(sc, prm, tk, t, code, st, wsteps, s_ctr, hc);
       t = -1;
     }
-    if (kSpread && exhausted && S == 0) {
+    bool dry = exhausted;
+    if constexpr (HINT) dry = dry || xhold;
+    if (kSpread && dry && S == 0) {
       const uint64_t live = __ballot(t >= 0);
       const int k = __popcll(live);
       if (k >= 2 && __builtin_amdgcn_readfirstlane(
@@ -262,6 +318,11 @@
     DIAG_ADD_LONE(D_LOOP, D_L_LOOP, t_loop, lone_it);
 #endif
 #if WOS_DIAG
+    if (HINT && xhold && !exhausted) {
+      DIAG_COUNT(D_E_ITERS, 1);
+      DIAG_COUNT(D_E_LANES, __popcll(__ballot(t >= 0)));
+      DIAG_ADD(D_E_LOOP, t_loop);
+    }
     if (exhausted) {
       DIAG_COUNT(D_XITERS, 1);
       DIAG_COUNT(D_XLANES, __popcll(__ballot(t >= 0)));
@@ -278,4 +339,7 @@
     else atomicAdd(&g_diag[threadIdx.x], s_diag[threadIdx.x]);
   }
 #endif
+  if constexpr (HINT) {
+    if (threadIdx.x == 0 && s_ctr[C_PTS]) atomicAdd(&hc[H_NLIST], s_ctr[C_PTS]);
+  }
   flush_walk_counters(counters, s_ctr);
diff --git a/neural-monte-carlo-fluid-simulation_amd/wos_amd/__init__.py b/neural-monte-carlo-fluid-simulation_amd/wos_amd/__init__.py
--- a/neural-monte-carlo-fluid-simulation_amd/wos_amd/__init__.py
+++ b/neural-monte-carlo-fluid-simulation_amd/wos_amd/__init__.py
@@ -1,7 +1,7 @@
 from ._lib import WosError, load as load_library
 from . import siren
-from .engine import WalkTape, WosScene, bvc_params, load_obj, solver_params, selftest_math, selftest_lhs, selftest_lhs_permute, selftest_lhs_permute_slots, selftest_lhs_plan, selftest_tape_rowsum, selftest_rejection, device_count, release_caches, set_max_batch_tasks
+from .engine import WalkTape, WosScene, bvc_params, load_obj, solver_params, selftest_math, selftest_lhs, selftest_lhs_permute, selftest_lhs_permute_slots, selftest_lhs_plan, selftest_tape_rowsum, selftest_rejection, device_count, release_caches, set_max_batch_tasks, set_length_hints, length_hint_stats, selftest_hint_key
 
 __all__ = ["WalkTape", "WosScene", "WosError", "bvc_params", "load_obj", "solver_params", "selftest_math", "selftest_lhs", "selftest_lhs_permute",
            "selftest_lhs_permute_slots", "selftest_lhs_plan", "selftest_tape_rowsum", "selftest_rejection", "device_count", "set_max_batch_tasks",
-           "load_library", "release_caches", "siren"]
+           "load_library", "release_caches", "siren", "set_length_hints", "length_hint_stats", "selftest_hint_key"]
diff --git a/neural-monte-carlo-fluid-simulation_amd/wos_amd/_lib.py b/neural-monte-carlo-fluid-simulation_amd/wos_amd/_lib.py
--- a/neural-monte-carlo-fluid-simulation_amd/wos_amd/_lib.py
+++ b/neural-monte-carlo-fluid-simulation_amd/wos_amd/_lib.py
@@ -68,6 +68,7 @@
 SCHED_NO_DIR_GRID = 0x8
 SCHED_NO_TAIL_SPREAD = 0x10
 SCHED_NO_GRID_SPREAD = 0x20
+SCHED_NO_LENGTH_HINTS = 0x40
 
 
 class BvcParams(C.Structure):
@@ -126,6 +127,7 @@
     "wos_siren_vjp", "wos_selftest_siren_vjp_layer",
     "wos_siren_fit",
     "wos_adam_step", "wos_siren_fit_run",
+    "wos_set_length_hints", "wos_length_hint_stats", "wos_selftest_hint_key",
 )
 
 QUERY_NEUMANN, QUERY_DIRICHLET = 0, 1
@@ -166,6 +168,13 @@
     L.wos_release_caches.argtypes = [C.c_int32]
     L.wos_set_max_batch_tasks.restype = C.c_int64
     L.wos_set_max_batch_tasks.argtypes = [C.c_int64]
+    if hasattr(L, "wos_set_length_hints"):
+        L.wos_set_length_hints.restype = None
+        L.wos_set_length_hints.argtypes = [C.c_int32] * 5
+        L.wos_length_hint_stats.restype = C.c_int
+        L.wos_length_hint_stats.argtypes = [C.c_int32, C.POINTER(C.c_int64)]
+        L.wos_selftest_hint_key.restype = C.c_int32
+        L.wos_selftest_hint_key.argtypes = [C.c_int32]
     L.wos_default_params.restype = None
     L.wos_default_params.argtypes = [C.POINTER(SolverParams)]
     L.wos_solve.restype = C.c_int
diff --git a/neural-monte-carlo-fluid-simulation_amd/wos_amd/engine.py b/neural-monte-carlo-fluid-simulation_amd/wos_amd/engine.py
--- a/neural-monte-carlo-fluid-simulation_amd/wos_amd/engine.py
+++ b/neural-monte-carlo-fluid-simulation_amd/wos_amd/engine.py
@@ -625,6 +625,26 @@
     return int(_lib.load().wos_set_max_batch_tasks(int(n)))
 
 
+def set_length_hints(hint_min=-1, express_min=-1, express_per_wave=-1, capacity=-1, priority=-1):
+    _lib.load().wos_set_length_hints(int(hint_min), int(express_min), int(express_per_wave), int(capacity),
+                                     int(priority))
+
+
+def length_hint_stats(device=0):
+    out = (C.c_int64 * 4)()
+    check(_lib.load().wos_length_hint_stats(int(device), out), "wos_length_hint_stats")
+    return {"claimed": int(out[0]), "overflow": int(out[1]), "listed": int(out[2]), "express": int(out[3])}
+
+
+def selftest_hint_key():
+    res = []
+    while True:
+        r = int(_lib.load().wos_selftest_hint_key(len(res)))
+        if r < 0:
+            return res
+        res.append(bool(r))
+
+
 def selftest_math(which, x, device=0):
     x = np.ascontiguousarray(x, dtype=np.float64)
     out = np.empty_like(x)
```
